# hila-chefer/Transformer-Explainability

Hardware: AMD Instinct MI355X
Metric: relevance maps/sec (ViT-B/16 224^2, batch 64 per GPU, generate_LRP transformer_attribution) (higher is better)
Workload: dtype f32 (3xbf16 split operands, 6 products, fp32 accumulate)

## Files before the change

### include/te_relprop.h

```cpp
#ifndef TE_RELPROP_H
#define TE_RELPROP_H

#include <stddef.h>
#include <stdint.h>

#ifdef __cplusplus
extern "C" {
#endif

typedef void* te_stream_t;
typedef uint16_t te_bf16_t;

enum {
  TE_OK = 0,
  TE_ERR_INVALID_ARG = -1,
  TE_ERR_WORKSPACE = -2,
  TE_ERR_UNSUPPORTED = -3,
  TE_ERR_NO_DEVICE = -4
};

enum { TE_VARIANT_OURS = 0, TE_VARIANT_LRP = 1, TE_IMPL_SIMPLE = 0x100 };

enum { TE_ROLLOUT_NORMALISE = 1, TE_ROLLOUT_CLS_FIXUP = 2, TE_ROLLOUT_ROW0 = 4 };

int te_version(void);
const char* te_status_string(int status);
int te_device_check(void);
const char* te_build_id(void);

size_t te_linear_relprop_workspace_bytes(int64_t T, int64_t in_f, int64_t out_f, int variant);
int te_linear_relprop_f32(const float* R, const float* X, const float* W, float* out,
                          int64_t T, int64_t in_f, int64_t out_f, float alpha, int variant,
                          void* ws, size_t ws_bytes, te_stream_t stream);

int te_linear_zpass_f32(const float* R, const float* X, const float* W, float* S,
                        int64_t T, int64_t in_f, int64_t out_f, te_stream_t stream);
int te_linear_cpass_f32(const float* S, const float* X, const float* W, float* out,
                        int64_t T, int64_t in_f, int64_t out_f, te_stream_t stream);

int te_linear_zpass_fwd_f32(const float* R, const float* X, const float* W, const float* Y, const float* bias,
                            float* S, int64_t T, int64_t in_f, int64_t out_f, te_stream_t stream);
int te_linear_relprop_fwd_f32(const float* R, const float* X, const float* W, const float* Y, const float* bias,
                              float* out, int64_t T, int64_t in_f, int64_t out_f,
                              void* ws, size_t ws_bytes, te_stream_t stream);

int te_linear_zpass_fwd_scaled_f32(const float* R, const float* r_scale, int64_t r_scale_stride,
                                   int64_t rows_per_sample, const float* X, const float* W, const float* Y,
                                   const float* bias, float* S, int64_t T, int64_t in_f, int64_t out_f,
                                   te_stream_t stream);
int te_linear_relprop_fwd_scaled_f32(const float* R, const float* r_scale, int64_t r_scale_stride,
                                     int64_t rows_per_sample, const float* X, const float* W, const float* Y,
                                     const float* bias, float* out, int64_t T, int64_t in_f, int64_t out_f,
                                     void* ws, size_t ws_bytes, te_stream_t stream);

size_t te_matmul_relprop_av_workspace_bytes(int64_t B, int64_t H, int64_t N, int64_t D);
int te_matmul_relprop_av_f32(const float* R, int64_t r_sb, int64_t r_sh, int64_t r_sn,
                             const float* attn,
                             const float* v, int64_t v_sb, int64_t v_sh, int64_t v_sn,
                             float* cam_attn,
                             float* cam_v, int64_t cv_sb, int64_t cv_sh, int64_t cv_sn,
                             int64_t B, int64_t H, int64_t N, int64_t D, float out_scale, int variant,
                             void* ws, size_t ws_bytes, te_stream_t stream);
size_t te_matmul_relprop_qk_workspace_bytes(int64_t B, int64_t H, int64_t N, int64_t D);
int te_matmul_relprop_av_fwd_f32(const float* R, int64_t r_sb, int64_t r_sh, int64_t r_sn,
                                 const float* attn,
                                 const float* v, int64_t v_sb, int64_t v_sh, int64_t v_sn,
                                 const float* Z,
                                 float* cam_attn,
                                 float* cam_v, int64_t cv_sb, int64_t cv_sh, int64_t cv_sn,
                                 int64_t B, int64_t H, int64_t N, int64_t D, float out_scale, int variant,
                                 void* ws, size_t ws_bytes, te_stream_t stream);
int te_matmul_relprop_av_fwdz_f32(const float* R, int64_t r_sb, int64_t r_sh, int64_t r_sn,
                                  const float* attn,
                                  const float* v, int64_t v_sb, int64_t v_sh, int64_t v_sn,
                                  const float* Z, int64_t z_sb, int64_t z_sh, int64_t z_sn,
                                  float* cam_attn,
                                  float* cam_v, int64_t cv_sb, int64_t cv_sh, int64_t cv_sn,
                                  int64_t B, int64_t H, int64_t N, int64_t D, float out_scale, int variant,
                                  void* ws, size_t ws_bytes, te_stream_t stream);
int te_matmul_relprop_qk_fwd_f32(const float* R_nn,
                                 const float* q, int64_t q_sb, int64_t q_sh, int64_t q_sn,
                                 const float* k, int64_t k_sb, int64_t k_sh, int64_t k_sn,
                                 const float* Z,
                                 float* cam_q, int64_t cq_sb, int64_t cq_sh, int64_t cq_sn,
                                 float* cam_k, int64_t ck_sb, int64_t ck_sh, int64_t ck_sn,
                                 int64_t B, int64_t H, int64_t N, int64_t D, float out_scale, int variant,
                                 void* ws, size_t ws_bytes, te_stream_t stream);
int te_matmul_relprop_qk_fwd_scaled_f32(const float* R_nn, const float* r_scale, int64_t r_scale_stride,
                                        const float* q, int64_t q_sb, int64_t q_sh, int64_t q_sn,
                                        const float* k, int64_t k_sb, int64_t k_sh, int64_t k_sn,
                                        const float* Z,
                                        float* cam_q, int64_t cq_sb, int64_t cq_sh, int64_t cq_sn,
                                        float* cam_k, int64_t ck_sb, int64_t ck_sh, int64_t ck_sn,
                                        int64_t B, int64_t H, int64_t N, int64_t D, float out_scale, int variant,
                                        void* ws, size_t ws_bytes, te_stream_t stream);
int te_matmul_relprop_qk_f32(const float* R_nn,
                             const float* q, int64_t q_sb, int64_t q_sh, int64_t q_sn,
                             const float* k, int64_t k_sb, int64_t k_sh, int64_t k_sn,
                             float* cam_q, int64_t cq_sb, int64_t cq_sh, int64_t cq_sn,
                             float* cam_k, int64_t ck_sb, int64_t ck_sh, int64_t ck_sn,
                             int64_t B, int64_t H, int64_t N, int64_t D, float out_scale, int variant,
                             void* ws, size_t ws_bytes, te_stream_t stream);

size_t te_add_relprop_workspace_bytes(int64_t B, int64_t n);
int te_add_relprop_f32(const float* R, const float* X0, const float* X1, float* out0, float* out1,
                       int64_t B, int64_t n, int64_t x1_batch_stride, int variant,
                       void* ws, size_t ws_bytes, te_stream_t stream);

size_t te_add_relprop_deferred_workspace_bytes(int64_t B, int64_t n);
int te_add_relprop_deferred_f32(const float* R, const float* X0, const float* X1, float* a, float* b, float* fac,
                                int64_t B, int64_t n, int64_t x1_batch_stride,
                                void* ws, size_t ws_bytes, te_stream_t stream);

size_t te_add_bcast_relprop_workspace_bytes(int64_t B, int64_t H, int64_t N);
int te_add_bcast_relprop_f32(const float* R, const float* X0, const float* mask, float* out0,
                             float* out1, int64_t B, int64_t H, int64_t N, int variant,
                             void* ws, size_t ws_bytes, te_stream_t stream);

int te_add_bcast_relprop_deferred_f32(const float* R, const float* X0, const float* mask, float* a, float* out1,
                                      float* fac, int64_t B, int64_t H, int64_t N,
                                      void* ws, size_t ws_bytes, te_stream_t stream);

int te_clone_relprop_f32(const float* R0, const float* R1, const float* R2, const float* X,
                         float* out, int64_t n, te_stream_t stream);

int te_clone_relprop_scaled_f32(const float* R0, const float* s0, int64_t s0_stride,
                                const float* R1, const float* s1, int64_t s1_stride,
                                const float* R2, const float* s2, int64_t s2_stride,
                                const float* X, float* out, int64_t B, int64_t n, te_stream_t stream);

int te_index_select_relprop_f32(const float* R, const float* X, float* out,
                                int64_t B, int64_t N, int64_t C, int64_t index, te_stream_t stream);

int te_gradcam_headmean_f32(const float* grad, const float* cam, float* out,
                            int64_t B, int64_t H, int64_t N, te_stream_t stream);

size_t te_rollout_workspace_bytes(int64_t L, int64_t B, int64_t N);
size_t te_rollout_row0_workspace_bytes(int64_t B, int64_t N);
int te_rollout_f32(const float* cams, int64_t L, int64_t start_layer, int64_t B, int64_t N,
                   int flags, float* joint, void* ws, size_t ws_bytes, te_stream_t stream);

#define TE_X6_TILE_AUTO 0
#define TE_X6_TILE_128 1
#define TE_X6_TILE_256 2
#define TE_X6_TILE_128x128 3
#define TE_X6_TEST_DROP_HANDOVER 0x200
#define TE_X6_WHOLE_TILES 0x10000
#define TE_X6_TEST_SMALL_GRID 0x4000
#define TE_X6_X_PLANES_SIGNED 0x20000
#define TE_X6_TILE_Z_SHIFT 10
#define TE_X6_TILE_C_SHIFT 12
#define TE_X6_PHASE_SPLIT 4
#define TE_X6_PHASE_Z 8
#define TE_X6_PHASE_C 16
#define TE_X6_PHASE_MASK 28
int te_linear_relprop_x6_supported(int64_t T, int64_t in_f, int64_t out_f);
size_t te_linear_relprop_x6_workspace_bytes(int64_t T, int64_t in_f, int64_t out_f);
size_t te_linear_x6_weight_planes_bytes(int64_t in_f, int64_t out_f);
size_t te_linear_x6_planes_bytes(int64_t rows, int64_t K);
int te_linear_x6_prepare_weights_f32(const float* W, int64_t in_f, int64_t out_f, void* planes, size_t planes_bytes,
                                     te_stream_t stream);
int te_linear_x6_split_abs_f32(const float* X, int64_t rows, int64_t K, void* planes, size_t planes_bytes,
                               te_stream_t stream);
int te_linear_relprop_x6_f32(const float* R, const float* r_scale, int64_t r_scale_stride, int64_t rows_per_sample,
                             const float* X, const float* W, const void* w_planes, const void* x_planes,
                             const float* Y, const float* bias, float* out,
                             int64_t T, int64_t in_f, int64_t out_f, int flags, unsigned* status, void* ws,
                             size_t ws_bytes, te_stream_t stream);
int te_linear_relprop_x6_check(const void* ws, int64_t T, int64_t in_f, int64_t out_f, te_stream_t stream);

int te_linear_relprop_x6_general_supported(int64_t T, int64_t in_f, int64_t out_f, int variant);
size_t te_linear_x6_weight_planes_lrp_bytes(int64_t in_f, int64_t out_f);
int te_linear_x6_prepare_weights_lrp_f32(const float* W, int64_t in_f, int64_t out_f, void* planes, size_t planes_bytes,
                                         te_stream_t stream);
size_t te_linear_relprop_x6_general_workspace_bytes(int64_t T, int64_t in_f, int64_t out_f, int variant);
int te_linear_relprop_x6_general_f32(const float* R, const float* r_scale, int64_t r_scale_stride, int64_t rows_per_sample,
                                     const float* X, const float* W, const void* w_planes, const void* w_planes_lrp,
                                     const void* x_abs_planes, const float* Y, const float* bias, float* out,
                                     int64_t T, int64_t in_f, int64_t out_f, float alpha, int variant, int flags,
                                     unsigned* status, void* ws, size_t ws_bytes, te_stream_t stream);

int te_gemm_x6_supported(int64_t T, int64_t K, int64_t M);
size_t te_gemm_x6_workspace_bytes(int64_t T, int64_t K, int64_t M);
int te_linear_x6_split_matrix_f32(const float* A, int64_t rows, int64_t K, int transposed, void* planes,
                                  size_t planes_bytes, te_stream_t stream);
int te_gemm_x6_f32(const float* X, const void* x_planes, const void* w_planes, const float* bias, float* out,
                   int64_t T, int64_t K, int64_t M, int flags, unsigned* status, void* ws, size_t ws_bytes,
                   te_stream_t stream);
int te_linear_x6_split_dual_f32(const float* A, int64_t rows, int64_t K, void* planes, void* planes_abs,
                                size_t planes_bytes, te_stream_t stream);
int te_gelu_backward_x6_planes_f32(const float* dy, const float* x, int64_t rows, int64_t K, void* planes,
                                   size_t planes_bytes, te_stream_t stream);
int te_gelu_forward_x6_planes_f32(const float* x, float* y, int64_t rows, int64_t K, void* planes, void* planes_abs,
                                  size_t planes_bytes, te_stream_t stream);

int te_attention_forward_supported(int64_t N, int64_t D);
int te_attention_forward_f32(const float* qkv, float* z_qk, float* attn, float* out,
                             int64_t B, int64_t H, int64_t N, int64_t D, float scale, te_stream_t stream);
int te_attention_forward_planes_f32(const float* qkv, float* z_qk, float* attn, float* out, void* out_planes,
                                    void* out_abs_planes, size_t planes_bytes, int64_t B, int64_t H, int64_t N, int64_t D,
                                    float scale, te_stream_t stream);
int te_attention_backward_f32(const float* d_out, const float* qkv, const float* attn, float* d_attn, float* d_qkv,
                              int64_t B, int64_t H, int64_t N, int64_t D, float scale, int need_qk, te_stream_t stream);
int te_attention_backward_out_f32(const float* d_out, const float* out, const float* qkv, const float* attn, float* d_attn,
                                  float* d_qkv, int64_t B, int64_t H, int64_t N, int64_t D, float scale, int need_qk,
                                  te_stream_t stream);

int te_attention_strided_supported(int64_t N, int64_t D);
size_t te_attention_backward_strided_workspace_bytes(int64_t B, int64_t H, int64_t N);
int te_attention_forward_strided_f32(const float* q, int64_t q_sb, int64_t q_sh, int64_t q_sn,
                                     const float* k, int64_t k_sb, int64_t k_sh, int64_t k_sn,
                                     const float* v, int64_t v_sb, int64_t v_sh, int64_t v_sn,
                                     const float* mask, float* z_qk, float* x_scaled, float* attn,
                                     float* out, int64_t o_sb, int64_t o_sh, int64_t o_sn,
                                     int64_t B, int64_t H, int64_t N, int64_t D, float scale, te_stream_t stream);
int te_attention_backward_strided_f32(const float* d_out, int64_t do_sb, int64_t do_sh, int64_t do_sn,
                                      const float* q, int64_t q_sb, int64_t q_sh, int64_t q_sn,
                                      const float* k, int64_t k_sb, int64_t k_sh, int64_t k_sn,
                                      const float* v, int64_t v_sb, int64_t v_sh, int64_t v_sn,
                                      const float* attn, float* d_attn,
                                      float* d_q, int64_t dq_sb, int64_t dq_sh, int64_t dq_sn,
                                      float* d_k, int64_t dk_sb, int64_t dk_sh, int64_t dk_sn,
                                      float* d_v, int64_t dv_sb, int64_t dv_sh, int64_t dv_sn,
                                      int64_t B, int64_t H, int64_t N, int64_t D, float scale, int need_qk,
                                      void* ws, size_t ws_bytes, te_stream_t stream);
int te_attention_backward_strided_out_f32(const float* d_out, int64_t do_sb, int64_t do_sh, int64_t do_sn,
                                          const float* out, int64_t o_sb, int64_t o_sh, int64_t o_sn,
                                          const float* q, int64_t q_sb, int64_t q_sh, int64_t q_sn,
                                          const float* k, int64_t k_sb, int64_t k_sh, int64_t k_sn,
                                          const float* v, int64_t v_sb, int64_t v_sh, int64_t v_sn,
                                          const float* attn, float* d_attn,
                                          float* d_q, int64_t dq_sb, int64_t dq_sh, int64_t dq_sn,
                                          float* d_k, int64_t dk_sb, int64_t dk_sh, int64_t dk_sn,
                                          float* d_v, int64_t dv_sb, int64_t dv_sh, int64_t dv_sn,
                                          int64_t B, int64_t H, int64_t N, int64_t D, float scale, int need_qk,
                                          void* ws, size_t ws_bytes, te_stream_t stream);

int te_layernorm_supported(int64_t C);
int te_layernorm_forward_f32(const float* x, const float* weight, const float* bias, float* y, float* mean, float* rstd,
                             int64_t T, int64_t C, float eps, te_stream_t stream);
int te_layernorm_backward_f32(const float* dy, const float* x, const float* weight, const float* mean, const float* rstd,
                              const float* add, float* dx, int64_t T, int64_t C, te_stream_t stream);
int te_gelu_forward_f32(const float* x, float* y, int64_t n, te_stream_t stream);
int te_gelu_backward_f32(const float* dy, const float* x, float* dx, int64_t n, te_stream_t stream);

int te_heatmap_f32(const float* maps, float* heat, float* fg_mask, int64_t B, int64_t g, int64_t scale,
                   int normalise, te_stream_t stream);

size_t te_seg_metrics_workspace_bytes(int64_t B, int64_t H, int64_t W);
int te_seg_metrics_f32(const float* heat, const float* fg_mask, const int64_t* labels, int64_t* counts, double* ap,
                       double* f1, int64_t B, int64_t H, int64_t W, void* ws, size_t ws_bytes, te_stream_t stream);

#define TE_MAPSIM_SSIM 1
size_t te_map_similarity_workspace_bytes(int64_t B, int64_t n);
int te_map_similarity_f32(const float* a, const float* b, int64_t* rank_sums, double* sim, int64_t B, int64_t n, int64_t H,
                          int64_t W, int flags, double data_range, void* ws, size_t ws_bytes, te_stream_t stream);

#define TE_RATIONALE_MAX_KS 16
#define TE_RATIONALE_CLAMP 1
size_t te_rationale_metrics_workspace_bytes(int64_t B, int64_t N, int64_t Wmax);
int te_rationale_metrics_f32(const float* scores, const int32_t* word_ids, const uint8_t* truth, float* word_scores,
                             int32_t* n_words, int32_t* order, int32_t* counts, double* soft, int64_t B, int64_t N,
                             int64_t Wmax, const int64_t* ks, int64_t n_ks, int flags, void* ws, size_t ws_bytes,
                             te_stream_t stream);

#define TE_TOKEN_ERASE_MAX_FRACTIONS 8
int te_token_erase(const int64_t* input_ids, const int64_t* attention_mask, const int32_t* word_ids,
                   const int32_t* order, const int32_t* n_words, int64_t* ids_out, int64_t* mask_out,
                   int32_t* n_rationale, int64_t B, int64_t N, int64_t Wmax, const double* fractions, int64_t n_t,
                   int64_t pad_id, te_stream_t stream);

size_t te_conv2d_zb_relprop_workspace_bytes(int64_t B, int64_t C, int64_t H, int64_t W, int64_t E, int64_t p);
int te_conv2d_zb_relprop_f32(const float* R, int64_t r_bs, const float* X, const float* W, const float* Y,
                             const float* bias, float* out, int64_t B, int64_t C, int64_t H, int64_t W_, int64_t E,
                             int64_t p, int flags, void* ws, size_t ws_bytes, te_stream_t stream);

#define TE_PERTURB_MAX_STEPS 16
#define TE_PERTURB_MAX_CHANNELS 4
size_t te_perturb_workspace_bytes(int64_t B, int64_t n_steps);
int te_perturb_f32(const float* vis, const float* data, float* out, int64_t B, int64_t C, int64_t HW,
                   const int64_t* ks, int64_t n_steps, const float* mean, const float* std_, void* ws,
                   size_t ws_bytes, te_stream_t stream);

#define TE_BLUR_MAX_TAPS 63
int te_blur_normalised_f32(const float* data, float* out, int64_t B, int64_t C, int64_t H, int64_t W, const float* taps,
                           int64_t klen, const float* mean, const float* std_, te_stream_t stream);
size_t te_pixel_rank_workspace_bytes(int64_t B, int64_t n);
int te_pixel_rank_f32(const float* vis, int32_t* rank, int64_t B, int64_t n, void* ws, size_t ws_bytes, te_stream_t stream);
int te_curve_inputs_f32(const float* data, const float* substrate, const float* fill, const int32_t* rank, float* out,
                        int64_t B, int64_t C, int64_t HW, int64_t step, int64_t s0, int64_t n_s, int insertion,
                        const float* mean, const float* std_, te_stream_t stream);
int te_curve_inputs_bf16(const float* data, const float* substrate, const float* fill, const int32_t* rank, te_bf16_t* out,
                         int64_t B, int64_t C, int64_t HW, int64_t step, int64_t s0, int64_t n_s, int insertion,
                         const float* mean, const float* std_, te_stream_t stream);
int te_curve_scores_f32(const float* logits, const int64_t* target, double* prob, int64_t B, int64_t K, int64_t s0,
                        int64_t n_s, te_stream_t stream);
int te_curve_scores_bf16(const te_bf16_t* logits, const int64_t* target, double* prob, int64_t B, int64_t K, int64_t s0,
                         int64_t n_s, te_stream_t stream);
int te_curve_auc_f64(const double* prob, double* auc, int64_t S1, int64_t B, te_stream_t stream);

size_t te_localisation_workspace_bytes(int64_t P, int64_t H, int64_t W);
int te_localisation_f32(const float* heat, const int64_t* labels, const int64_t* image_index, const int64_t* target_id,
                        const int64_t* boxes, int64_t M, int64_t* stats, double* energy, int64_t P, int64_t B, int64_t H,
                        int64_t W, void* ws, size_t ws_bytes, te_stream_t stream);

int te_noise_inputs_f32(const float* x, float* out, int64_t B, int64_t n, int64_t d0, int64_t n_d, float radius, int64_t seed,
                        int64_t id0, te_stream_t stream);
int te_noise_inputs_bf16(const float* x, te_bf16_t* out, int64_t B, int64_t n, int64_t d0, int64_t n_d, float radius,
                         int64_t seed, int64_t id0, te_stream_t stream);
int te_map_distance_f32(const float* a, const float* b, double* sums, int64_t B, int64_t D, int64_t n, te_stream_t stream);
int te_map_distance_bf16(const float* a, const te_bf16_t* b, double* sums, int64_t B, int64_t D, int64_t n,
                         te_stream_t stream);
size_t te_map_complexity_workspace_bytes(int64_t B, int64_t n);
int te_map_complexity_f32(const float* maps, double* out, int64_t* counts, int64_t B, int64_t n, double eps, void* ws,
                          size_t ws_bytes, te_stream_t stream);

#define TE_SUBSET_MAX_CELLS 4096
int te_subset_inputs_f32(const float* x, const float* substrate, const float* fill, const float* attr, float* out,
                         uint8_t* member, double* attr_sum, int64_t B, int64_t C, int64_t g_h, int64_t g_w, int64_t p,
                         int64_t k, int64_t d0, int64_t n_d, int64_t seed, int64_t id0, te_stream_t stream);
int te_subset_inputs_bf16(const float* x, const float* substrate, const float* fill, const float* attr, te_bf16_t* out,
                          uint8_t* member, double* attr_sum, int64_t B, int64_t C, int64_t g_h, int64_t g_w, int64_t p,
                          int64_t k, int64_t d0, int64_t n_d, int64_t seed, int64_t id0, te_stream_t stream);
int te_perturbation_dot_f32(const float* x, const float* y, const float* w, double* sums, int64_t B, int64_t D, int64_t n,
                            int64_t m, te_stream_t stream);
int te_perturbation_dot_bf16(const float* x, const te_bf16_t* y, const float* w, double* sums, int64_t B, int64_t D, int64_t n,
                             int64_t m, te_stream_t stream);

int te_linear_relprop_bf16_supported(int64_t T, int64_t in_f, int64_t out_f);
size_t te_linear_relprop_bf16_workspace_bytes(int64_t T, int64_t in_f, int64_t out_f);
size_t te_linear_bf16_weight_planes_bytes(int64_t in_f, int64_t out_f);
int te_linear_bf16_prepare_weights(const te_bf16_t* W, int64_t in_f, int64_t out_f, void* planes, size_t planes_bytes,
                                   te_stream_t stream);
int te_linear_relprop_bf16(const float* R, int64_t r_ld, const float* r_scale, int64_t r_scale_stride,
                           int64_t rows_per_scale, const te_bf16_t* X, int64_t x_ld, const void* w_planes, float* out,
                           int64_t T, int64_t in_f, int64_t out_f, void* ws, size_t ws_bytes, te_stream_t stream);
int te_matmul_relprop_bf16_supported(int64_t N, int64_t D);
size_t te_matmul_relprop_av_bf16_workspace_bytes(int64_t B, int64_t H, int64_t N, int64_t D);
size_t te_matmul_relprop_qk_bf16_workspace_bytes(int64_t B, int64_t H, int64_t N, int64_t D);
int te_matmul_relprop_av_bf16(const float* R, int64_t r_sb, int64_t r_sh, int64_t r_sn,
                              const te_bf16_t* attn,
                              const te_bf16_t* v, int64_t v_sb, int64_t v_sh, int64_t v_sn,
                              const te_bf16_t* Z, int64_t z_sb, int64_t z_sh, int64_t z_sn,
                              float* cam_attn,
                              float* cam_v, int64_t cv_sb, int64_t cv_sh, int64_t cv_sn,
                              int64_t B, int64_t H, int64_t N, int64_t D, float out_scale, int variant,
                              void* ws, size_t ws_bytes, te_stream_t stream);
int te_matmul_relprop_qk_bf16(const float* R_nn, const float* r_scale, int64_t r_scale_stride,
                              const te_bf16_t* q, int64_t q_sb, int64_t q_sh, int64_t q_sn,
                              const te_bf16_t* k, int64_t k_sb, int64_t k_sh, int64_t k_sn,
                              const te_bf16_t* Z,
                              float* cam_q, int64_t cq_sb, int64_t cq_sh, int64_t cq_sn,
                              float* cam_k, int64_t ck_sb, int64_t ck_sh, int64_t ck_sn,
                              int64_t B, int64_t H, int64_t N, int64_t D, float out_scale, int variant,
                              void* ws, size_t ws_bytes, te_stream_t stream);
int te_add_relprop_bf16(const float* R, const te_bf16_t* X0, const te_bf16_t* X1, float* out0, float* out1, int64_t B,
                        int64_t n, int64_t x1_batch_stride, int variant, void* ws, size_t ws_bytes, te_stream_t stream);
int te_add_relprop_deferred_bf16(const float* R, const te_bf16_t* X0, const te_bf16_t* X1, float* a, float* b,
                                 float* fac, int64_t B, int64_t n, int64_t x1_batch_stride, void* ws, size_t ws_bytes,
// ... 106 lines not shown
```

### transformer-explainability_amd/csrc/te_attn.hip

```cpp
#include "te_internal.h"

namespace {

constexpr int kThreads = 256;

__global__ __launch_bounds__(kThreads) void av_s_simple(
    const float* __restrict__ R, Strided rs, const float* __restrict__ attn, const float* __restrict__ v,
    Strided vs, float* __restrict__ S, int64_t B, int64_t H, int64_t N, int64_t D) {
  const int64_t idx = (int64_t)blockIdx.x * kThreads + threadIdx.x;
  if (idx >= B * H * N * D) return;
  const int64_t d = idx % D, i = (idx / D) % N, h = (idx / (D * N)) % H, b = idx / (D * N * H);
  const float* arow = attn + ((b * H + h) * N + i) * N;
  float z = 0.0f;
  for (int64_t j = 0; j < N; ++j) z = fmaf(arow[j], v[vs.at(b, h, j) + d], z);
  S[idx] = te_sd(R[rs.at(b, h, i) + d], z);
}

__global__ __launch_bounds__(kThreads) void av_s_from_z_simple(
    const float* __restrict__ R, Strided rs, const float* __restrict__ Z, float* __restrict__ S, int64_t B, int64_t H,
    int64_t N, int64_t D) {
  const int64_t idx = (int64_t)blockIdx.x * kThreads + threadIdx.x;
  if (idx >= B * H * N * D) return;
  const int64_t d = idx % D, i = (idx / D) % N, h = (idx / (D * N)) % H, b = idx / (D * N * H);
  S[idx] = te_sd(R[rs.at(b, h, i) + d], Z[idx]);
}
__global__ __launch_bounds__(kThreads) void qk_s_from_z_simple(const float* __restrict__ R, const float* __restrict__ Z,
                                                               float* __restrict__ S, int64_t n) {
  const int64_t idx = (int64_t)blockIdx.x * kThreads + threadIdx.x;
  if (idx < n) S[idx] = te_sd(R[idx], Z[idx]);
}

__global__ __launch_bounds__(kThreads) void av_cam_attn_simple(
    const float* __restrict__ S, const float* __restrict__ attn, const float* __restrict__ v, Strided vs,
    float* __restrict__ cam, int64_t B, int64_t H, int64_t N, int64_t D, float scale) {
  const int64_t idx = (int64_t)blockIdx.x * kThreads + threadIdx.x;
  if (idx >= B * H * N * N) return;
  const int64_t j = idx % N, i = (idx / N) % N, h = (idx / (N * N)) % H, b = idx / (N * N * H);
  const float* srow = S + ((b * H + h) * N + i) * D;
  const float* vrow = v + vs.at(b, h, j);
  float g = 0.0f;
  for (int64_t d = 0; d < D; ++d) g = fmaf(srow[d], vrow[d], g);
  cam[idx] = (attn[idx] * g) * scale;
}

__global__ __launch_bounds__(kThreads) void av_cam_v_simple(
    const float* __restrict__ S, const float* __restrict__ attn, const float* __restrict__ v, Strided vs,
    float* __restrict__ cam_v, Strided cs, int64_t B, int64_t H, int64_t N, int64_t D, float scale) {
  const int64_t idx = (int64_t)blockIdx.x * kThreads + threadIdx.x;
  if (idx >= B * H * N * D) return;
  const int64_t d = idx % D, j = (idx / D) % N, h = (idx / (D * N)) % H, b = idx / (D * N * H);
  const float* a = attn + (b * H + h) * N * N + j;
  const float* s = S + (b * H + h) * N * D + d;
  float u = 0.0f;
  for (int64_t i = 0; i < N; ++i) u = fmaf(a[i * N], s[i * D], u);
  cam_v[cs.at(b, h, j) + d] = (v[vs.at(b, h, j) + d] * u) * scale;
}

__global__ __launch_bounds__(kThreads) void qk_s_simple(
    const float* __restrict__ R, const float* __restrict__ q, Strided qs, const float* __restrict__ k,
    Strided ks, float* __restrict__ S, int64_t B, int64_t H, int64_t N, int64_t D) {
  const int64_t idx = (int64_t)blockIdx.x * kThreads + threadIdx.x;
  if (idx >= B * H * N * N) return;
  const int64_t j = idx % N, i = (idx / N) % N, h = (idx / (N * N)) % H, b = idx / (N * N * H);
  const float* qrow = q + qs.at(b, h, i);
  const float* krow = k + ks.at(b, h, j);
  float z = 0.0f;
  for (int64_t d = 0; d < D; ++d) z = fmaf(qrow[d], krow[d], z);
  S[idx] = te_sd(R[idx], z);
}

__global__ __launch_bounds__(kThreads) void qk_cam_q_simple(
    const float* __restrict__ S, const float* __restrict__ q, Strided qs, const float* __restrict__ k,
    Strided ks, float* __restrict__ cam_q, Strided cs, int64_t B, int64_t H, int64_t N, int64_t D, float scale) {
  const int64_t idx = (int64_t)blockIdx.x * kThreads + threadIdx.x;
  if (idx >= B * H * N * D) return;
  const int64_t d = idx % D, i = (idx / D) % N, h = (idx / (D * N)) % H, b = idx / (D * N * H);
  const float* srow = S + ((b * H + h) * N + i) * N;
  float u = 0.0f;
  for (int64_t j = 0; j < N; ++j) u = fmaf(srow[j], k[ks.at(b, h, j) + d], u);
  cam_q[cs.at(b, h, i) + d] = (q[qs.at(b, h, i) + d] * u) * scale;
}

__global__ __launch_bounds__(kThreads) void qk_cam_k_simple(
    const float* __restrict__ S, const float* __restrict__ q, Strided qs, const float* __restrict__ k,
    Strided ks, float* __restrict__ cam_k, Strided cs, int64_t B, int64_t H, int64_t N, int64_t D, float scale) {
  const int64_t idx = (int64_t)blockIdx.x * kThreads + threadIdx.x;
  if (idx >= B * H * N * D) return;
  const int64_t d = idx % D, j = (idx / D) % N, h = (idx / (D * N)) % H, b = idx / (D * N * H);
  const float* s = S + (b * H + h) * N * N + j;
  float u = 0.0f;
  for (int64_t i = 0; i < N; ++i) u = fmaf(s[i * N], q[qs.at(b, h, i) + d], u);
  cam_k[cs.at(b, h, j) + d] = (k[ks.at(b, h, j) + d] * u) * scale;
}

inline bool view_ok(Strided s) { return s.sb >= 0 && s.sh >= 0 && s.sn > 0; }

inline int finish(int rc) {
  if (rc != TE_OK) return rc;
  TE_RETURN_IF_LAUNCH_FAILED();
  return TE_OK;
}

}

extern "C" size_t te_matmul_relprop_av_workspace_bytes(int64_t B, int64_t H, int64_t N, int64_t D) {
  if (B <= 0 || H <= 0 || N <= 0 || D <= 0) return 0;
  return te_align_up((size_t)2 * B * H * N * D * sizeof(float), 256);
}

extern "C" int te_matmul_relprop_av_f32(const float* R, int64_t r_sb, int64_t r_sh, int64_t r_sn,
                                        const float* attn, const float* v, int64_t v_sb, int64_t v_sh,
                                        int64_t v_sn, float* cam_attn, float* cam_v, int64_t cv_sb,
                                        int64_t cv_sh, int64_t cv_sn, int64_t B, int64_t H, int64_t N,
                                        int64_t D, float out_scale, int variant, void* ws, size_t ws_bytes,
                                        te_stream_t stream_) {
  return te_matmul_relprop_av_fwd_f32(R, r_sb, r_sh, r_sn, attn, v, v_sb, v_sh, v_sn, nullptr, cam_attn, cam_v, cv_sb,
                                      cv_sh, cv_sn, B, H, N, D, out_scale, variant, ws, ws_bytes, stream_);
}

extern "C" int te_matmul_relprop_av_fwd_f32(const float* R, int64_t r_sb, int64_t r_sh, int64_t r_sn,
                                            const float* attn, const float* v, int64_t v_sb, int64_t v_sh,
                                            int64_t v_sn, const float* Z, float* cam_attn, float* cam_v,
                                            int64_t cv_sb, int64_t cv_sh, int64_t cv_sn, int64_t B, int64_t H,
                                            int64_t N, int64_t D, float out_scale, int variant, void* ws,
                                            size_t ws_bytes, te_stream_t stream_) {
  return te_matmul_relprop_av_fwdz_f32(R, r_sb, r_sh, r_sn, attn, v, v_sb, v_sh, v_sn, Z, H * N * D, N * D, D, cam_attn,
                                       cam_v, cv_sb, cv_sh, cv_sn, B, H, N, D, out_scale, variant, ws, ws_bytes, stream_);
}

extern "C" int te_matmul_relprop_av_fwdz_f32(const float* R, int64_t r_sb, int64_t r_sh, int64_t r_sn,
                                             const float* attn, const float* v, int64_t v_sb, int64_t v_sh,
                                             int64_t v_sn, const float* Z, int64_t z_sb, int64_t z_sh, int64_t z_sn,
                                             float* cam_attn, float* cam_v, int64_t cv_sb, int64_t cv_sh,
                                             int64_t cv_sn, int64_t B, int64_t H, int64_t N, int64_t D,
                                             float out_scale, int variant, void* ws, size_t ws_bytes,
                                             te_stream_t stream_) {
  if (!R || !attn || !v || !cam_attn || !cam_v || B <= 0 || H <= 0 || N <= 0 || D <= 0)
    return TE_ERR_INVALID_ARG;
  const Strided rs{r_sb, r_sh, r_sn}, vs{v_sb, v_sh, v_sn}, cs{cv_sb, cv_sh, cv_sn}, contig{H * N * D, N * D, D};
  if (!view_ok(rs) || !view_ok(vs) || !view_ok(cs)) return TE_ERR_INVALID_ARG;
  if (!ws || ws_bytes < te_matmul_relprop_av_workspace_bytes(B, H, N, D)) return TE_ERR_WORKSPACE;
  hipStream_t stream = (hipStream_t)stream_;
  float* S = (float*)ws;
  float* Zws = S + (size_t)(B * H) * N * D;
  Strided zs = Z ? Strided{z_sb, z_sh, z_sn} : contig;
  if ((variant & TE_IMPL_SIMPLE) || !te_attn_mfma::supported(N, D)) {
    if (zs.sn != contig.sn || zs.sh != contig.sh || zs.sb != contig.sb) return TE_ERR_UNSUPPORTED;
    const int64_t nd = B * H * N * D, nn = B * H * N * N;
    dim3 blk(kThreads);
    if (Z) av_s_from_z_simple<<<dim3((unsigned)te_ceil_div(nd, kThreads)), blk, 0, stream>>>(R, rs, Z, S, B, H, N, D);
    else av_s_simple<<<dim3((unsigned)te_ceil_div(nd, kThreads)), blk, 0, stream>>>(R, rs, attn, v, vs, S, B, H, N, D);
    av_cam_attn_simple<<<dim3((unsigned)te_ceil_div(nn, kThreads)), blk, 0, stream>>>(S, attn, v, vs, cam_attn, B,
                                                                                     H, N, D, out_scale);
    av_cam_v_simple<<<dim3((unsigned)te_ceil_div(nd, kThreads)), blk, 0, stream>>>(S, attn, v, vs, cam_v, cs, B, H,
                                                                                  N, D, out_scale);
    TE_RETURN_IF_LAUNCH_FAILED();
    return TE_OK;
  }
  if (!Z) {
    const int rc = te_attn_mfma::z_av_launch(attn, v, vs, Zws, B, H, N, stream);
    if (rc != TE_OK) return rc;
    Z = Zws;
  }
  if (te_attn_kb::supported(B, H, N, D))
    return finish(te_attn_kb::av_launch(TE_ATTN_RULE, R, rs, attn, v, vs, Z, zs, cam_attn, cam_v, cs, B, H, N, out_scale, stream));
  return finish(te_attn_mfma::av_launch(R, rs, attn, v, vs, Z, zs, cam_attn, cam_v, cs, B, H, N, out_scale, S, stream));
}

extern "C" size_t te_matmul_relprop_qk_workspace_bytes(int64_t B, int64_t H, int64_t N, int64_t D) {
  if (B <= 0 || H <= 0 || N <= 0 || D <= 0) return 0;
  return te_align_up((size_t)2 * B * H * N * N * sizeof(float), 256);
}

extern "C" int te_matmul_relprop_qk_f32(const float* R_nn, const float* q, int64_t q_sb, int64_t q_sh,
                                        int64_t q_sn, const float* k, int64_t k_sb, int64_t k_sh, int64_t k_sn,
                                        float* cam_q, int64_t cq_sb, int64_t cq_sh, int64_t cq_sn, float* cam_k,
                                        int64_t ck_sb, int64_t ck_sh, int64_t ck_sn, int64_t B, int64_t H,
                                        int64_t N, int64_t D, float out_scale, int variant, void* ws,
                                        size_t ws_bytes, te_stream_t stream_) {
  return te_matmul_relprop_qk_fwd_f32(R_nn, q, q_sb, q_sh, q_sn, k, k_sb, k_sh, k_sn, nullptr, cam_q, cq_sb, cq_sh,
                                      cq_sn, cam_k, ck_sb, ck_sh, ck_sn, B, H, N, D, out_scale, variant, ws, ws_bytes,
                                      stream_);
}

extern "C" int te_matmul_relprop_qk_fwd_f32(const float* R_nn, const float* q, int64_t q_sb, int64_t q_sh,
                                            int64_t q_sn, const float* k, int64_t k_sb, int64_t k_sh,
                                            int64_t k_sn, const float* Z, float* cam_q, int64_t cq_sb,
                                            int64_t cq_sh, int64_t cq_sn, float* cam_k, int64_t ck_sb,
                                            int64_t ck_sh, int64_t ck_sn, int64_t B, int64_t H, int64_t N,
                                            int64_t D, float out_scale, int variant, void* ws, size_t ws_bytes,
                                            te_stream_t stream_) {
  return te_matmul_relprop_qk_fwd_scaled_f32(R_nn, nullptr, 0, q, q_sb, q_sh, q_sn, k, k_sb, k_sh, k_sn, Z, cam_q, cq_sb,
                                             cq_sh, cq_sn, cam_k, ck_sb, ck_sh, ck_sn, B, H, N, D, out_scale, variant, ws,
                                             ws_bytes, stream_);
}

extern "C" int te_matmul_relprop_qk_fwd_scaled_f32(const float* R_nn, const float* r_scale, int64_t r_scale_stride,
                                                   const float* q, int64_t q_sb, int64_t q_sh, int64_t q_sn,
                                                   const float* k, int64_t k_sb, int64_t k_sh, int64_t k_sn,
                                                   const float* Z, float* cam_q, int64_t cq_sb, int64_t cq_sh,
                                                   int64_t cq_sn, float* cam_k, int64_t ck_sb, int64_t ck_sh,
                                                   int64_t ck_sn, int64_t B, int64_t H, int64_t N, int64_t D,
                                                   float out_scale, int variant, void* ws, size_t ws_bytes,
                                                   te_stream_t stream_) {
  if (!R_nn || !q || !k || !cam_q || !cam_k || B <= 0 || H <= 0 || N <= 0 || D <= 0) return TE_ERR_INVALID_ARG;
  const Strided qs{q_sb, q_sh, q_sn}, ks{k_sb, k_sh, k_sn}, cqs{cq_sb, cq_sh, cq_sn}, cks{ck_sb, ck_sh, ck_sn};
  if (!view_ok(qs) || !view_ok(ks) || !view_ok(cqs) || !view_ok(cks)) return TE_ERR_INVALID_ARG;
  if (!ws || ws_bytes < te_matmul_relprop_qk_workspace_bytes(B, H, N, D)) return TE_ERR_WORKSPACE;
  hipStream_t stream = (hipStream_t)stream_;
  float* S = (float*)ws;
  float* Zws = S + (size_t)(B * H) * N * N;
  if ((variant & TE_IMPL_SIMPLE) || !te_attn_mfma::supported(N, D)) {
    if (r_scale) return TE_ERR_UNSUPPORTED;
    const int64_t nd = B * H * N * D, nn = B * H * N * N;
    dim3 blk(kThreads);
    if (Z) qk_s_from_z_simple<<<dim3((unsigned)te_ceil_div(nn, kThreads)), blk, 0, stream>>>(R_nn, Z, S, nn);
    else qk_s_simple<<<dim3((unsigned)te_ceil_div(nn, kThreads)), blk, 0, stream>>>(R_nn, q, qs, k, ks, S, B, H, N, D);
    qk_cam_q_simple<<<dim3((unsigned)te_ceil_div(nd, kThreads)), blk, 0, stream>>>(S, q, qs, k, ks, cam_q, cqs, B, H,
                                                                                  N, D, out_scale);
    qk_cam_k_simple<<<dim3((unsigned)te_ceil_div(nd, kThreads)), blk, 0, stream>>>(S, q, qs, k, ks, cam_k, cks, B, H,
                                                                                  N, D, out_scale);
    TE_RETURN_IF_LAUNCH_FAILED();
    return TE_OK;
  }
  if (!Z) {
    const int rc = te_attn_mfma::z_qk_launch(q, qs, k, ks, Zws, B, H, N, stream);
    if (rc != TE_OK) return rc;
    Z = Zws;
  }
  if (te_attn_rules::supported(B, H, N, D) && q_sn > 65536) return TE_ERR_UNSUPPORTED;
  if (te_attn_rc::supported(B, H, N, D))
    return finish(te_attn_rc::qk_launch(TE_ATTN_RULE, R_nn, q, qs, k, ks, Z, cam_q, cqs, cam_k, cks, B, H, N, out_scale, r_scale, r_scale_stride,
                                        stream));
  if (te_attn_rules::supported(B, H, N, D))
    return finish(te_attn_rules::qk_launch(TE_ATTN_RULE, R_nn, q, qs, k, ks, Z, cam_q, cqs, cam_k, cks, B, H, N, out_scale, S, r_scale,
                                           r_scale_stride, stream));
  if (r_scale) return TE_ERR_UNSUPPORTED;
  return finish(te_attn_mfma::qk_launch(R_nn, q, qs, k, ks, Z, cam_q, cqs, cam_k, cks, B, H, N, out_scale, S, stream));
}

extern "C" int te_attention_forward_supported(int64_t N, int64_t D) { return te_attn_fwd6::supported(1, 1, N, D) ? 1 : 0; }

extern "C" int te_attention_forward_f32(const float* qkv, float* z_qk, float* attn, float* out, int64_t B, int64_t H,
                                        int64_t N, int64_t D, float scale, te_stream_t stream_) {
  if (!qkv || !z_qk || !attn || !out || B <= 0 || H <= 0 || N <= 0) return TE_ERR_INVALID_ARG;
  if (!te_attn_fwd6::supported(B, H, N, D)) return TE_ERR_UNSUPPORTED;
  return finish(te_attn_fwd6::launch(qkv, z_qk, attn, out, B, H, N, scale, (hipStream_t)stream_));
}

extern "C" int te_attention_forward_planes_f32(const float* qkv, float* z_qk, float* attn, float* out, void* out_planes,
                                               void* out_abs_planes, size_t planes_bytes, int64_t B, int64_t H, int64_t N,
                                               int64_t D, float scale, te_stream_t stream_) {
  if (!qkv || !z_qk || !attn || !out || !out_planes || B <= 0 || H <= 0 || N <= 0) return TE_ERR_INVALID_ARG;
  if (!te_attn_fwd6::supported(B, H, N, D)) return TE_ERR_UNSUPPORTED;
  const size_t need = te_linear_x6_planes_bytes(B * N, H * D);
  if (need == 0) return TE_ERR_UNSUPPORTED;
  if (planes_bytes < need || !te_aligned16(out_planes) || (out_abs_planes && !te_aligned16(out_abs_planes))) return TE_ERR_WORKSPACE;
  return finish(te_attn_fwd6::launch(qkv, z_qk, attn, out, B, H, N, scale, (hipStream_t)stream_, out_planes, out_abs_planes));
}

static int attention_backward(const float* d_out, const float* out, const float* qkv, const float* attn, float* d_attn, float* d_qkv,
                              int64_t B, int64_t H, int64_t N, int64_t D, float scale, int need_qk, te_stream_t stream_) {
  if (!d_out || !qkv || !attn || !d_attn || !d_qkv || B <= 0 || H <= 0 || N <= 0) return TE_ERR_INVALID_ARG;
  if (!te_attn_fwd6::supported(B, H, N, D)) return TE_ERR_UNSUPPORTED;
  hipStream_t stream = (hipStream_t)stream_;
  const int64_t C = H * 64;
  const Strided heads{N * C, 64, C};
  const Strided fused{N * 3 * C, 64, 3 * C};
  const float *q = qkv, *k = qkv + C, *v = qkv + 2 * C;
  float *d_q = d_qkv, *d_k = d_qkv + C, *d_v = d_qkv + 2 * C;
  const int rc = te_attn_kb::av_launch(TE_ATTN_BWD, d_out, heads, attn, v, fused, nullptr, Strided(), d_attn, d_v, fused, B, H, N, 1.0f, stream);
  if (rc != TE_OK || !need_qk) return finish(rc);
  if ((N <= 160 || out) && te_attn_rc::supported(B, H, N, D))
    return finish(te_attn_rc::qk_launch(TE_ATTN_BWD, d_attn, q, fused, k, fused, attn, d_q, fused, d_k, fused, B, H, N, scale, nullptr, 0, stream,
                                        out ? d_out : nullptr, out, heads));
  return finish(te_attn_rules::qk_launch(TE_ATTN_BWD, d_attn, q, fused, k, fused, attn, d_q, fused, d_k, fused, B, H, N, scale, nullptr, nullptr, 0,
                                         stream));
}

extern "C" int te_attention_backward_f32(const float* d_out, const float* qkv, const float* attn, float* d_attn,
                                         float* d_qkv, int64_t B, int64_t H, int64_t N, int64_t D, float scale,
                                         int need_qk, te_stream_t stream_) {
  return attention_backward(d_out, nullptr, qkv, attn, d_attn, d_qkv, B, H, N, D, scale, need_qk, stream_);
}

extern "C" int te_attention_backward_out_f32(const float* d_out, const float* out, const float* qkv, const float* attn,
                                             float* d_attn, float* d_qkv, int64_t B, int64_t H, int64_t N, int64_t D,
                                             float scale, int need_qk, te_stream_t stream_) {
  if (!out) return TE_ERR_INVALID_ARG;
  return attention_backward(d_out, out, qkv, attn, d_attn, d_qkv, B, H, N, D, scale, need_qk, stream_);
}

extern "C" int te_attention_strided_supported(int64_t N, int64_t D) { return te_attn_long::supported(1, 1, N, D) ? 1 : 0; }

extern "C" size_t te_attention_backward_strided_workspace_bytes(int64_t B, int64_t H, int64_t N) {
  return te_align_up((size_t)(B * H * N) * sizeof(float), 256);
}

extern "C" int te_attention_forward_strided_f32(const float* q, int64_t q_sb, int64_t q_sh, int64_t q_sn, const float* k,
                                                int64_t k_sb, int64_t k_sh, int64_t k_sn, const float* v, int64_t v_sb,
                                                int64_t v_sh, int64_t v_sn, const float* mask, float* z_qk,
                                                float* x_scaled, float* attn, float* out, int64_t o_sb, int64_t o_sh,
                                                int64_t o_sn, int64_t B, int64_t H, int64_t N, int64_t D, float scale,
                                                te_stream_t stream_) {
  using te_attn_long::strides_ok;
  if (!q || !k || !v || !attn || !out || B <= 0 || H <= 0 || N <= 0) return TE_ERR_INVALID_ARG;
  const Strided qs{q_sb, q_sh, q_sn}, ks{k_sb, k_sh, k_sn}, vs{v_sb, v_sh, v_sn}, os{o_sb, o_sh, o_sn};
  if (!te_attn_long::supported(B, H, N, D)) return TE_ERR_UNSUPPORTED;
  if (!strides_ok(qs) || !strides_ok(ks) || !strides_ok(vs) || !strides_ok(os)) return TE_ERR_UNSUPPORTED;
  hipStream_t stream = (hipStream_t)stream_;
  if (te_attn_fwd6l::supported(B, H, N, D))
    return finish(te_attn_fwd6l::launch(q, qs, k, ks, v, vs, mask, z_qk, x_scaled, attn, out, os, B, H, N, scale, stream));
  return finish(te_attn_long::fwd_launch(q, qs, k, ks, v, vs, mask, z_qk, x_scaled, attn, out, os, B, H, N, scale, stream));
}

static int backward_strided(const float* d_out, Strided dos, const float* out, Strided os, const float* q, Strided qs, const float* k,
                            Strided ks, const float* v, Strided vs, const float* attn, float* d_attn, float* d_q, Strided dqs, float* d_k,
                            Strided dks, float* d_v, Strided dvs, int64_t B, int64_t H, int64_t N, int64_t D, float scale, int need_qk,
                            void* ws, size_t ws_bytes, te_stream_t stream_) {
  using te_attn_long::strides_ok;
  if (!d_out || !k || !v || !attn || !d_attn || !d_v || B <= 0 || H <= 0 || N <= 0) return TE_ERR_INVALID_ARG;
  if (need_qk && (!q || !d_q || !d_k)) return TE_ERR_INVALID_ARG;
  if (!te_attn_long::supported(B, H, N, D)) return TE_ERR_UNSUPPORTED;
  if (!strides_ok(dos) || !strides_ok(ks) || !strides_ok(vs) || !strides_ok(dvs) || (out && !strides_ok(os))) return TE_ERR_UNSUPPORTED;
  if (need_qk && (!strides_ok(qs) || !strides_ok(dqs) || !strides_ok(dks))) return TE_ERR_UNSUPPORTED;
  if (!ws || ws_bytes < te_attention_backward_strided_workspace_bytes(B, H, N)) return TE_ERR_WORKSPACE;
  hipStream_t stream = (hipStream_t)stream_;
  float* rowdot = (float*)ws;
  need_qk = need_qk ? 1 : 0;
  const bool l6 = te_attn_bwd6l::supported(B, H, N, D);
  int rc;
  if ((out || !need_qk) && l6)
    rc = te_attn_bwd6l::launch_rows(d_out, dos, out, os, k, ks, v, vs, attn, d_attn, rowdot, d_q, dqs, B, H, N, scale, need_qk, stream);
  else
    rc = te_attn_long::bwd_rows_launch(d_out, dos, k, ks, v, vs, attn, d_attn, rowdot, d_q, dqs, B, H, N, scale, need_qk, stream);
  if (rc != TE_OK) return rc;
  if (l6) return finish(te_attn_bwd6l::launch_cols(attn, d_attn, rowdot, d_out, dos, q, qs, d_v, dvs, d_k, dks, B, H, N, scale, need_qk, stream));
  return finish(te_attn_long::bwd_cols_launch(attn, d_attn, rowdot, d_out, dos, q, qs, d_v, dvs, d_k, dks, B, H, N, scale, need_qk, stream));
}

extern "C" int te_attention_backward_strided_f32(const float* d_out, int64_t do_sb, int64_t do_sh, int64_t do_sn,
                                                 const float* q, int64_t q_sb, int64_t q_sh, int64_t q_sn, const float* k,
                                                 int64_t k_sb, int64_t k_sh, int64_t k_sn, const float* v, int64_t v_sb,
                                                 int64_t v_sh, int64_t v_sn, const float* attn, float* d_attn, float* d_q,
                                                 int64_t dq_sb, int64_t dq_sh, int64_t dq_sn, float* d_k, int64_t dk_sb,
                                                 int64_t dk_sh, int64_t dk_sn, float* d_v, int64_t dv_sb, int64_t dv_sh,
                                                 int64_t dv_sn, int64_t B, int64_t H, int64_t N, int64_t D, float scale,
                                                 int need_qk, void* ws, size_t ws_bytes, te_stream_t stream_) {
  return backward_strided(d_out, {do_sb, do_sh, do_sn}, nullptr, Strided(), q, {q_sb, q_sh, q_sn}, k, {k_sb, k_sh, k_sn}, v, {v_sb, v_sh, v_sn},
                          attn, d_attn, d_q, {dq_sb, dq_sh, dq_sn}, d_k, {dk_sb, dk_sh, dk_sn}, d_v, {dv_sb, dv_sh, dv_sn}, B, H, N, D, scale,
                          need_qk, ws, ws_bytes, stream_);
}

extern "C" int te_attention_backward_strided_out_f32(const float* d_out, int64_t do_sb, int64_t do_sh, int64_t do_sn,
                                                     const float* out, int64_t o_sb, int64_t o_sh, int64_t o_sn, const float* q,
                                                     int64_t q_sb, int64_t q_sh, int64_t q_sn, const float* k, int64_t k_sb,
                                                     int64_t k_sh, int64_t k_sn, const float* v, int64_t v_sb, int64_t v_sh,
                                                     int64_t v_sn, const float* attn, float* d_attn, float* d_q, int64_t dq_sb,
                                                     int64_t dq_sh, int64_t dq_sn, float* d_k, int64_t dk_sb, int64_t dk_sh,
                                                     int64_t dk_sn, float* d_v, int64_t dv_sb, int64_t dv_sh, int64_t dv_sn,
                                                     int64_t B, int64_t H, int64_t N, int64_t D, float scale, int need_qk, void* ws,
                                                     size_t ws_bytes, te_stream_t stream_) {
  if (!out) return TE_ERR_INVALID_ARG;
  return backward_strided(d_out, {do_sb, do_sh, do_sn}, out, {o_sb, o_sh, o_sn}, q, {q_sb, q_sh, q_sn}, k, {k_sb, k_sh, k_sn}, v,
                          {v_sb, v_sh, v_sn}, attn, d_attn, d_q, {dq_sb, dq_sh, dq_sn}, d_k, {dk_sb, dk_sh, dk_sn}, d_v, {dv_sb, dv_sh, dv_sn}, B,
                          H, N, D, scale, need_qk, ws, ws_bytes, stream_);
}
```

### transformer-explainability_amd/csrc/te_attn_kb.hip

```cpp
#include <type_traits>

#include "te_buffer.h"
#include "te_internal.h"
#include "te_x6.h"

namespace te_attn_kb {

namespace {

constexpr int TI = 32;
constexpr int kT = 512;
constexpr int kWaves = kT / 64;
constexpr int XLD = 36;

enum { RULE = 0, BWD = 1 };



constexpr int kRLD = 144;
constexpr int kTLD = 80;
constexpr int kPlR = TI * kRLD;
constexpr int kPlT = 64 * kTLD;
constexpr int kSBuf = 3 * kPlR + 3 * kPlT;

template <int MODE>
__global__ __launch_bounds__(kT) void av6_kb_kernel(
    const float* __restrict__ R, Strided rs, const float* __restrict__ Z, Strided zs, const float* __restrict__ attn,
    const float* __restrict__ v, Strided vs, float* __restrict__ cam_attn, float* __restrict__ cam_v, Strided cs, int H,
    int N, int BH, int KBG, float scale) {
  __shared__ __attribute__((aligned(16))) unsigned char Sb[3][kSBuf];
  __shared__ __attribute__((aligned(16))) float Xw[kWaves][TI * XLD];
  __shared__ unsigned arrived;
  if (threadIdx.x == 0) arrived = 0;
  __syncthreads();
  const int bh = blockIdx.x % BH, g = blockIdx.x / BH;
  const int b = bh / H, h = bh - b * H;
  const int wave = __builtin_amdgcn_readfirstlane(threadIdx.x >> 6), lane = threadIdx.x & 63, lr = lane & 31, kh = lane >> 5;
  const int nkb = (N + 31) >> 5, kb = g * KBG + wave;
  const bool has_blk = wave < KBG && kb < nkb;
  const int j = kb * 32 + lr;
  const int ntiles = (N + TI - 1) / TI;
  const int srow = threadIdx.x >> 4, sc = threadIdx.x & 15;
  const int spos = (srow & 0x13) | ((srow & 4) << 1) | ((srow & 8) >> 1);

  const unsigned nn_bytes = (unsigned)N * (unsigned)N * 4u;
  const Rsrc a_rs = make_rsrc(attn + (int64_t)bh * N * N, nn_bytes);
  const Rsrc ca_rs = make_rsrc(cam_attn + (int64_t)bh * N * N, nn_bytes);
  const Rsrc r_rs = make_rsrc(R + (int64_t)b * rs.sb + (int64_t)h * rs.sh, view_bytes(N, rs.sn));
  const Rsrc z_rs = make_rsrc(MODE == RULE ? Z + (int64_t)b * zs.sb + (int64_t)h * zs.sh : R, MODE == RULE ? view_bytes(N, zs.sn) : 0u);
  const Rsrc v_rs = make_rsrc(v + (int64_t)b * vs.sb + (int64_t)h * vs.sh, view_bytes(N, vs.sn));
  const Rsrc cv_rs = make_rsrc(cam_v + (int64_t)b * cs.sb + (int64_t)h * cs.sh, view_bytes(N, cs.sn));
  const unsigned row_bytes = (unsigned)N * 4u;

  f32x4 rr = {0.f, 0.f, 0.f, 0.f}, zz = {0.f, 0.f, 0.f, 0.f};
  const unsigned r_off = ((unsigned)srow * (unsigned)rs.sn + 4u * sc) * 4u, z_off = ((unsigned)srow * (unsigned)zs.sn + 4u * sc) * 4u;
  const unsigned r_tile = (unsigned)TI * (unsigned)rs.sn * 4u, z_tile = (unsigned)TI * (unsigned)zs.sn * 4u;
  auto fetch_rz = [&](int it) __attribute__((always_inline)) {
    ld128_hidden(rr, r_rs, r_off + (unsigned)it * r_tile);
    if constexpr (MODE == RULE) ld128_hidden(zz, z_rs, z_off + (unsigned)it * z_tile);
  };
  constexpr int kRz = (MODE == RULE) ? 2 : 1;
  auto pin_rz = [&]() __attribute__((always_inline)) {
    TE_PIN(rr);
    if constexpr (MODE == RULE) TE_PIN(zz);
  };
  auto put_s = [&](int it) __attribute__((always_inline)) {
    f32x4 s = rr;
    if constexpr (MODE == RULE) {
#pragma unroll
      for (int e = 0; e < 4; ++e) s[e] = te_sd(rr[e], zz[e]);
    }
    unsigned p01[3], p23[3];
    split3_pk(s[0], s[1], p01);
    split3_pk(s[2], s[3], p23);
    unsigned char* base = Sb[it % 3];
#pragma unroll
    for (int q = 0; q < 3; ++q) {
      *reinterpret_cast<u32x2*>(base + q * kPlR + srow * kRLD + sc * 8) = u32x2{p01[q], p23[q]};
      unsigned char* t = base + 3 * kPlR + q * kPlT + (4 * sc) * kTLD + spos * 2;
      *reinterpret_cast<unsigned short*>(t) = (unsigned short)(p01[q] & 0xffffu);
      *reinterpret_cast<unsigned short*>(t + kTLD) = (unsigned short)(p01[q] >> 16);
      *reinterpret_cast<unsigned short*>(t + 2 * kTLD) = (unsigned short)(p23[q] & 0xffffu);
      *reinterpret_cast<unsigned short*>(t + 3 * kTLD) = (unsigned short)(p23[q] >> 16);
    }
    asm volatile("s_waitcnt lgkmcnt(0)" ::: "memory");
    if (lane == 0) __hip_atomic_fetch_add(&arrived, 1u, __ATOMIC_RELAXED, __HIP_MEMORY_SCOPE_WORKGROUP);
  };
  auto wait_s = [&](int it) __attribute__((always_inline)) {
    const unsigned target = (unsigned)kWaves * (unsigned)(it + 1);
    while (__builtin_amdgcn_readfirstlane(__hip_atomic_load(&arrived, __ATOMIC_RELAXED, __HIP_MEMORY_SCOPE_WORKGROUP)) < target)
      __builtin_amdgcn_s_sleep(1);
    asm volatile("" ::: "memory");
  };

  if (!has_blk) {
    fetch_rz(0);
    TE_VM_WAIT(0);
    pin_rz();
    put_s(0);
    fetch_rz(1);
    for (int it = 0; it < ntiles; ++it) {
      wait_s(it);
      TE_VM_WAIT(0);
      pin_rz();
      put_s(it + 1);
      fetch_rz(it + 2);
    }
    TE_VM_WAIT(0);
    return;
  }

  bf16x8 vpl[4][3];
  {
    const unsigned off = ((unsigned)j * (unsigned)vs.sn + 8u * kh) * 4u;
#pragma unroll
    for (int s4 = 0; s4 < 4; ++s4) {
      const f32x4 lo = ld128(v_rs, off + 64u * s4), hi = ld128(v_rs, off + 64u * s4 + 16u);
      const float x[8] = {lo[0], lo[1], lo[2], lo[3], hi[0], hi[1], hi[2], hi[3]};
      planes_of8(x, vpl[s4]);
    }
  }
  float* const Xb = Xw[wave];
  const int xr = lane >> 3, xc = (lane & 7) << 2;
  const unsigned lane_x4 = ((unsigned)xr * (unsigned)N + (unsigned)(kb * 32 + xc)) * 4u;
  const unsigned lane_nn = ((unsigned)(4 * kh) * (unsigned)N + (unsigned)j) * 4u;
  const bool key_ok = j < N;
  const bool blk_full = kb * 32 + 32 <= N;
  auto fetch_attn = [&](int it, f32x4 (&dst)[4]) __attribute__((always_inline)) {
    const unsigned base = (unsigned)(it * TI) * row_bytes;
#pragma unroll
    for (int p = 0; p < 4; ++p) ld128_hidden(dst[p], a_rs, lane_x4 + (base + (unsigned)(8 * p) * row_bytes));
  };
  auto to_acc = [&](const f32x4 (&src)[4], float (&dst)[16]) __attribute__((always_inline)) {
#pragma unroll
    for (int p = 0; p < 4; ++p) *reinterpret_cast<f32x4*>(Xb + (8 * p + xr) * XLD + xc) = src[p];
#pragma unroll
    for (int e = 0; e < 16; ++e) dst[e] = Xb[crow(e, kh) * XLD + lr];
  };

  float ac[16];
  f32x4 an[4], an2[4];
  fetch_rz(0);
  fetch_attn(0, an2);
  TE_VM_WAIT(0);
  pin_rz();
#pragma unroll
  for (int s4 = 0; s4 < 4; ++s4)
#pragma unroll
    for (int q = 0; q < 3; ++q) TE_PIN(vpl[s4][q]);
#pragma unroll
  for (int p = 0; p < 4; ++p) TE_PIN(an2[p]);
  put_s(0);
  fetch_rz(1);
  fetch_attn(1, an);
  to_acc(an2, ac);

  f32x16 accv[2];
  zero16(accv[0]);
  zero16(accv[1]);
  auto tile = [&](int it, f32x4 (&ax)[4], f32x4 (&ay)[4]) __attribute__((always_inline)) {
    const unsigned char* Sc = Sb[it % 3];
    wait_s(it);
    TE_VM_WAIT(4);
    pin_rz();
    put_s(it + 1);
    fetch_rz(it + 2);
    fetch_attn(it + 2, ax);
    __builtin_amdgcn_sched_barrier(0);
    if (it < ntiles) {
      f32x16 gacc;
      zero16(gacc);
      {
        const unsigned char* Ab = Sc + lr * kRLD + 16 * kh;
#pragma unroll
        for (int s4 = 0; s4 < 4; ++s4) {
          bf16x8 a[3];
#pragma unroll
          for (int q = 0; q < 3; ++q) a[q] = *reinterpret_cast<const bf16x8*>(Ab + q * kPlR + 32 * s4);
          mfma_x6(gacc, a, vpl[s4]);
        }
      }
      float gp[16];
#pragma unroll
      for (int e = 0; e < 16; ++e) gp[e] = (MODE == RULE) ? (ac[e] * gacc[e]) * scale : gacc[e];
      const unsigned base = (unsigned)(it * TI) * row_bytes;
      if (blk_full) {
#pragma unroll
        for (int e = 0; e < 16; ++e) Xb[crow(e, kh) * XLD + lr] = gp[e];
#pragma unroll
        for (int p = 0; p < 4; ++p) {
          const f32x4 t = *reinterpret_cast<const f32x4*>(Xb + (8 * p + xr) * XLD + xc);
          st128_hidden(t, ca_rs, lane_x4 + (base + (unsigned)(8 * p) * row_bytes));
        }
      } else if (key_ok) {
#pragma unroll
        for (int e = 0; e < 16; ++e) st32_hidden(gp[e], ca_rs, lane_nn + (base + (unsigned)((e & 3) + 8 * (e >> 2)) * row_bytes));
      }
      bf16x8 apl[2][3];
#pragma unroll
      for (int s2 = 0; s2 < 2; ++s2) {
        const float x[8] = {ac[8 * s2], ac[8 * s2 + 1], ac[8 * s2 + 2], ac[8 * s2 + 3],
                            ac[8 * s2 + 4], ac[8 * s2 + 5], ac[8 * s2 + 6], ac[8 * s2 + 7]};
        planes_of8(x, apl[s2]);
      }
#pragma unroll
      for (int db = 0; db < 2; ++db) {
        const unsigned char* Bb = Sc + 3 * kPlR + (db * 32 + lr) * kTLD + 16 * kh;
#pragma unroll
        for (int s2 = 0; s2 < 2; ++s2) {
          bf16x8 bq[3];
#pragma unroll
          for (int q = 0; q < 3; ++q) bq[q] = *reinterpret_cast<const bf16x8*>(Bb + q * kPlT + 32 * s2);
          mfma_x6(accv[db], apl[s2], bq);
        }
      }
    }
    if constexpr (kRz == 2) TE_VM_WAIT(6);
    else TE_VM_WAIT(5);
#pragma unroll
    for (int p = 0; p < 4; ++p) TE_PIN(ay[p]);
    to_acc(ay, ac);
  };
#pragma unroll 1
  for (int it = 0; it < ntiles; it += 2) {
    tile(it, an2, an);
    tile(it + 1, an, an2);
  }
  TE_VM_WAIT(0);

#pragma unroll
  for (int db = 0; db < 2; ++db) {
    const unsigned d4 = (unsigned)(db * 32 + lr) * 4u;
    float x[16];
    if constexpr (MODE == RULE) {
      const unsigned xoff = (unsigned)(kb * 32 + 4 * kh) * (unsigned)vs.sn * 4u + d4;
#pragma unroll
      for (int e = 0; e < 16; ++e) x[e] = ld32(v_rs, xoff + (unsigned)((e & 3) + 8 * (e >> 2)) * (unsigned)vs.sn * 4u);
    }
    const unsigned ooff = (unsigned)(kb * 32 + 4 * kh) * (unsigned)cs.sn * 4u + d4;
#pragma unroll
    for (int e = 0; e < 16; ++e) {
      float val = accv[db][e];
      if constexpr (MODE == RULE) val = (x[e] * val) * scale;
      st32(val, cv_rs, ooff + (unsigned)((e & 3) + 8 * (e >> 2)) * (unsigned)cs.sn * 4u);
    }
  }
}

inline void groups_for(int64_t N, int& ng, int& kbg) {
  const int nkb = (int)((N + 31) / 32);
  ng = (nkb + kWaves - 1) / kWaves;
  kbg = (nkb + ng - 1) / ng;
}

}

bool supported(int64_t B, int64_t H, int64_t N, int64_t D) {
  int ng, kbg;
  groups_for(N, ng, kbg);
  return D == 64 && N >= 1 && N <= 4096 && B * H * ng <= 0x7fffffff;
}

int av_launch(int mode, const float* R, Strided rs, const float* attn, const float* v, Strided vs, const float* Z, Strided zs,
              float* cam_attn, float* cam_v, Strided cs, int64_t B, int64_t H, int64_t N, float scale, hipStream_t stream) {
  int ng, kbg;
  groups_for(N, ng, kbg);
  const int BH = (int)(B * H);
  auto stride_ok = [](int64_t sn) { return sn >= 64 && sn <= 65536; };
  if (!stride_ok(rs.sn) || !stride_ok(vs.sn) || !stride_ok(cs.sn) || (mode == 0 && !stride_ok(zs.sn))) return TE_ERR_UNSUPPORTED;
  const dim3 grid((unsigned)(BH * ng)), blk(kT);
  if (mode == 0)
    av6_kb_kernel<RULE><<<grid, blk, 0, stream>>>(R, rs, Z, zs, attn, v, vs, cam_attn, cam_v, cs, (int)H, (int)N, BH, kbg, scale);
  else
    av6_kb_kernel<BWD><<<grid, blk, 0, stream>>>(R, rs, nullptr, Strided{0, 0, 0}, attn, v, vs, cam_attn, cam_v, cs, (int)H,
                                                 (int)N, BH, kbg, 1.0f);
  return TE_OK;
}

}
```

### transformer-explainability_amd/csrc/te_attn_rc.hip

```cpp
#include <stdlib.h>
#include <string.h>

#include <type_traits>

#include "te_buffer.h"
#include "te_internal.h"
#include "te_x6.h"

namespace te_attn_rc {

namespace {

constexpr int kT = 512;
constexpr int kMaxN = 224;
constexpr int kMaxSteps = kMaxN / 16;

enum { RULE = 0, BWD = 1 };
enum { ROWS = 0, COLS = 1 };


template <bool PERM>
__device__ __forceinline__ void stage_planes(unsigned char* __restrict__ Pl, const float* __restrict__ M, int64_t sn, int N,
                                             int NS) {
  for (int item = threadIdx.x; item < NS * 2 * 16; item += kT) {
// ... 159 lines not shown
    float rdr[8];
    if constexpr (MODE == BWD) {
      const float* rp = rdv + 32 * blk + 16 * (s & 1) + 8 * kh;
      const f32x4 a0 = *reinterpret_cast<const f32x4*>(rp), a1 = *reinterpret_cast<const f32x4*>(rp + 4);
#pragma unroll
      for (int e = 0; e < 4; ++e) rdr[e] = a0[e], rdr[4 + e] = a1[e];
    }
#pragma unroll
    for (int t2 = 0; t2 < 4; ++t2) {
      f32x2 r = {rc[set][2 * t2], rc[set][2 * t2 + 1]}, z = {zc[set][2 * t2], zc[set][2 * t2 + 1]};
      if constexpr (MODE == RULE) {
        if (has_f) r = r * f32x2{f, f};
        sv[t2] = sd2(r, z);
      } else {
        sv[t2] = (z * (r - f32x2{rdr[2 * t2], rdr[2 * t2 + 1]})) * f32x2{scale, scale};
      }
    }
    if (32 * (s >> 1) + 32 > N) {
      const bool ok = 32 * (s >> 1) + n < N;
#pragma unroll
      for (int t2 = 0; t2 < 4; ++t2) sv[t2][0] = ok ? sv[t2][0] : 0.0f, sv[t2][1] = ok ? sv[t2][1] : 0.0f;
    }
    unsigned pk[4][3];
#pragma unroll
    for (int t2 = 0; t2 < 4; ++t2) split3_pk(sv[t2][0], sv[t2][1], pk[t2]);
#pragma unroll
    for (int q = 0; q < 3; ++q) b[q] = __builtin_bit_cast(bf16x8, u32x4{pk[0][q], pk[1][q], pk[2][q], pk[3][q]});
  };
  bf16x8 E[2];
#pragma unroll
  for (int sp = 0; sp < 2; ++sp) {
    const int tt = n - 16 * sp - 8 * kh;
    u32x4 w;
#pragma unroll
    for (int u = 0; u < 4; ++u) w[u] = (tt == 2 * u) ? 0x00003f80u : (tt == 2 * u + 1) ? 0x3f800000u : 0u;
    E[sp] = __builtin_bit_cast(bf16x8, w);
  }
  const unsigned char* const frag = Pk + lane * 16;
  issue(0, 0);
  issue(1, 1);
  issue(2, 2);
  static_for<0, kMaxSteps / 2>([&](auto ri) __attribute__((always_inline)) {
    constexpr int r = decltype(ri)::value, s0 = 2 * r, s1 = 2 * r + 1;
    bf16x8 P0[3], P1[3];
    vm_wait<(((s0 + 2 < kMaxSteps - 1) ? s0 + 2 : kMaxSteps - 1) - s0) * LPS>();
    if (r < NB) {
      pin(s0 % RING);
      make_planes(s0, s0 % RING, P0);
    }
    if constexpr (s0 + RING < kMaxSteps) issue(s0 + RING, s0 % RING);
    vm_wait<(((s1 + 2 < kMaxSteps - 1) ? s1 + 2 : kMaxSteps - 1) - s1) * LPS>();
    if (r < NB) {
      pin(s1 % RING);
      make_planes(s1, s1 % RING, P1);
    }
    if constexpr (s1 + RING < kMaxSteps) issue(s1 + RING, s1 % RING);
    if (r < NB) {
      bf16x8 Ba[3], Bb[3];
#pragma unroll
      for (int q = 0; q < 3; ++q) {
        f32x16 T;
#pragma unroll
        for (int e = 0; e < 16; ++e) T[e] = 0.0f;
        T = TE_MFMA_BF16(P0[q], E[0], T);
        T = TE_MFMA_BF16(P1[q], E[1], T);
        u32x4 wa, wb;
#pragma unroll
        for (int u = 0; u < 4; ++u) {
          wa[u] = __builtin_bit_cast(unsigned, __builtin_convertvector(f32x2{T[2 * u], T[2 * u + 1]}, bf16x2));
          wb[u] = __builtin_bit_cast(unsigned, __builtin_convertvector(f32x2{T[8 + 2 * u], T[8 + 2 * u + 1]}, bf16x2));
        }
        Ba[q] = __builtin_bit_cast(bf16x8, wa);
        Bb[q] = __builtin_bit_cast(bf16x8, wb);
      }
#pragma unroll
      for (int half = 0; half < 2; ++half) {
        bf16x8 a[2][3];
#pragma unroll
        for (int mb = 0; mb < 2; ++mb)
#pragma unroll
          for (int q = 0; q < 3; ++q)
            a[mb][q] = *reinterpret_cast<const bf16x8*>(frag + q * plane + (size_t)((s0 + half) * 2 + mb) * kFrag);
#pragma unroll
        for (int p6 = 0; p6 < 6; ++p6)
#pragma unroll
          for (int mb = 0; mb < 2; ++mb)
            acc[mb] = TE_MFMA_BF16(a[mb][PA[p6]], half ? Bb[PB[p6]] : Ba[PB[p6]], acc[mb]);
      }
    }
  });
  vm_wait<0>();
  pin(0);
  pin(1);
  pin(2);
}

__device__ __forceinline__ void row_dots(float* __restrict__ rdv, Rsrc r_rs, Rsrc z_rs, int N, int NB, int blk) {
  const int lane = threadIdx.x & 63, lr = lane >> 3, lc = lane & 7;
  constexpr int RING = 3, LPS = 8;
  f32x4 rv[RING][4], zv[RING][4];
  const unsigned row_bytes = (unsigned)N * 4u;
  const unsigned base = ((unsigned)(blk * 32 + lr) * (unsigned)N + 4u * lc) * 4u;
  auto issue = [&](int u, int set) __attribute__((always_inline)) {
#pragma unroll
    for (int p = 0; p < 4; ++p) {
      const unsigned off = base + (unsigned)(8 * p) * row_bytes + 128u * (unsigned)u;
      ld128_hidden(rv[set][p], r_rs, off);
      ld128_hidden(zv[set][p], z_rs, off);
    }
  };
  auto pin = [&](int set) __attribute__((always_inline)) {
#pragma unroll
    for (int p = 0; p < 4; ++p) { TE_PIN(rv[set][p]); TE_PIN(zv[set][p]); }
  };
  float part[4] = {0.0f, 0.0f, 0.0f, 0.0f};
  issue(0, 0);
  issue(1, 1);
  issue(2, 2);
  static_for<0, kMaxSteps / 2>([&](auto ui) __attribute__((always_inline)) {
    constexpr int u = decltype(ui)::value, NU = kMaxSteps / 2;
    vm_wait<(((u + 2 < NU - 1) ? u + 2 : NU - 1) - u) * LPS>();
    if (u < NB) {
      pin(u % RING);
#pragma unroll
      for (int p = 0; p < 4; ++p)
#pragma unroll
        for (int e = 0; e < 4; ++e) {
          const float v = rv[u % RING][p][e] * zv[u % RING][p][e];
          part[p] = part[p] + ((32 * u + 4 * lc + e < N) ? v : 0.0f);
        }
    }
    if constexpr (u + RING < NU) issue(u + RING, u % RING);
  });
  vm_wait<0>();
  pin(0);
  pin(1);
  pin(2);
#pragma unroll
  for (int p = 0; p < 4; ++p) {
    float v = part[p];
    v = v + __shfl_xor(v, 1, 64);
    v = v + __shfl_xor(v, 2, 64);
    v = v + __shfl_xor(v, 4, 64);
    if (lc == 0) rdv[32 * blk + 8 * p + lr] = v;
  }
}

template <int MODE>
__global__ __launch_bounds__(kT) void qk_rc_kernel(const float* __restrict__ Rnn, const float* __restrict__ Z,
                                                   const float* __restrict__ q, Strided qs, const float* __restrict__ k,
                                                   Strided ks, float* __restrict__ cam_q, Strided cqs,
                                                   float* __restrict__ cam_k, Strided cks, int H, int N, float scale,
                                                   const float* __restrict__ r_scale, int64_t r_scale_stride, int both,
                                                   const float* __restrict__ dO, const float* __restrict__ O, Strided os) {
  extern __shared__ __attribute__((aligned(16))) unsigned char smem[];
  const int NS = (N + 15) >> 4, NB = (N + 31) >> 5;
  const size_t plane = (size_t)NS * 2 * kFrag;
  unsigned char* const Pk = smem;
  unsigned char* const Pq = both ? smem + 3 * plane : smem;
  float* const rdv = reinterpret_cast<float*>(smem + (both ? 6 : 3) * plane);
  const int bh = blockIdx.x, b = bh / H, h = bh - b * H;
  const int wave = __builtin_amdgcn_readfirstlane(threadIdx.x >> 6), lane = threadIdx.x & 63, n = lane & 31, hh = lane >> 5;
  const unsigned nn_bytes = (unsigned)N * (unsigned)N * 4u;
  const Rsrc r_rs = make_rsrc(Rnn + (int64_t)bh * N * N, nn_bytes), z_rs = make_rsrc(Z + (int64_t)bh * N * N, nn_bytes);
  const float* q_bh = q + (int64_t)b * qs.sb + (int64_t)h * qs.sh;
  const float* k_bh = k + (int64_t)b * ks.sb + (int64_t)h * ks.sh;
  const bool has_f = (MODE == RULE) && r_scale != nullptr;
  const float f = has_f ? r_scale[(int64_t)b * r_scale_stride] : 1.0f;
  const bool owner = wave < NB;

  stage_planes<true>(Pk, k_bh, ks.sn, N, NS);
  if (both) stage_planes<false>(Pq, q_bh, qs.sn, N, NS);
  float rd_own = 0.0f;
  if constexpr (MODE == BWD) {
    if (dO != nullptr) {
      const float* dO_bh = dO + (int64_t)b * os.sb + (int64_t)h * os.sh;
      const float* O_bh = O + (int64_t)b * os.sb + (int64_t)h * os.sh;
      for (int r0 = 0; r0 < 32 * NB; r0 += kT / 4) {
        const int i = r0 + (threadIdx.x >> 2), c = threadIdx.x & 3;
        float part = 0.0f;
        if (i < N) {
          const float* a = dO_bh + (int64_t)i * os.sn + 16 * c;
          const float* o = O_bh + (int64_t)i * os.sn + 16 * c;
          f32x4 av[4], ov[4];
#pragma unroll
          for (int u = 0; u < 4; ++u) av[u] = *reinterpret_cast<const f32x4_u*>(a + 4 * u), ov[u] = *reinterpret_cast<const f32x4_u*>(o + 4 * u);
#pragma unroll
          for (int u = 0; u < 4; ++u)
#pragma unroll
            for (int e = 0; e < 4; ++e) part = part + av[u][e] * ov[u][e];
        }
        part = part + __shfl_xor(part, 1, 64);
        part = part + __shfl_xor(part, 2, 64);
        if (c == 0 && i < 32 * NB) rdv[i] = part;
      }
    } else if (owner) {
      row_dots(rdv, r_rs, z_rs, N, NB, wave);
    }
  }
  __syncthreads();

  if (owner) {
    f32x16 acc[2];
#pragma unroll
    for (int mb = 0; mb < 2; ++mb)
#pragma unroll
      for (int e = 0; e < 16; ++e) acc[mb][e] = 0.0f;
    phase_rows<MODE>(acc, Pk, plane, r_rs, z_rs, N, NB, wave, f, has_f, scale, rdv);
    const int i = wave * 32 + n;
    if (i < N) {
      const float* qrow = q_bh + (int64_t)i * qs.sn + 4 * hh;
      float* orow = cam_q + (int64_t)b * cqs.sb + (int64_t)h * cqs.sh + (int64_t)i * cqs.sn + 4 * hh;
      f32x4 x4[2][4];
      if constexpr (MODE == RULE) {
#pragma unroll
        for (int mb = 0; mb < 2; ++mb)
#pragma unroll
          for (int g = 0; g < 4; ++g) x4[mb][g] = *reinterpret_cast<const f32x4_u*>(qrow + 32 * mb + 8 * g);
      }
#pragma unroll
      for (int mb = 0; mb < 2; ++mb)
#pragma unroll
        for (int g = 0; g < 4; ++g) {
          f32x4 o;
#pragma unroll
          for (int c = 0; c < 4; ++c) {
            const float v = acc[mb][4 * g + c];
            o[c] = (MODE == RULE) ? (x4[mb][g][c] * v) * scale : v;
          }
          *reinterpret_cast<f32x4_u*>(orow + 32 * mb + 8 * g) = o;
        }
    }
  }
  if (!both) {
    __syncthreads();
    stage_planes<false>(Pq, q_bh, qs.sn, N, NS);
    __syncthreads();
  }

  if (owner) {
    f32x16 acc[2];
#pragma unroll
    for (int mb = 0; mb < 2; ++mb)
#pragma unroll
      for (int e = 0; e < 16; ++e) acc[mb][e] = 0.0f;
    phase<MODE, COLS>(acc, Pq, plane, r_rs, z_rs, N, NS, wave, f, has_f, scale, rd_own, rdv);
    const int j = wave * 32 + n;
    if (j < N) {
      const float* krow = k_bh + (int64_t)j * ks.sn + 4 * hh;
      float* orow = cam_k + (int64_t)b * cks.sb + (int64_t)h * cks.sh + (int64_t)j * cks.sn + 4 * hh;
      f32x4 x4[2][4];
      if constexpr (MODE == RULE) {
#pragma unroll
        for (int mb = 0; mb < 2; ++mb)
#pragma unroll
          for (int g = 0; g < 4; ++g) x4[mb][g] = *reinterpret_cast<const f32x4_u*>(krow + 32 * mb + 8 * g);
      }
#pragma unroll
      for (int mb = 0; mb < 2; ++mb)
#pragma unroll
        for (int g = 0; g < 4; ++g) {
          f32x4 o;
#pragma unroll
          for (int c = 0; c < 4; ++c) {
            const float v = acc[mb][4 * g + c];
            o[c] = (MODE == RULE) ? (x4[mb][g][c] * v) * scale : v;
          }
          *reinterpret_cast<f32x4_u*>(orow + 32 * mb + 8 * g) = o;
        }
    }
  }
}

inline size_t lds_bytes(int64_t N, bool both) {
  const int64_t NS = (N + 15) >> 4;
  return (size_t)((both ? 6 : 3) * NS * 2 * kFrag) + (size_t)(NS * 16 + 16) * sizeof(float);
}
constexpr size_t kLdsMax = 160 * 1024;

}

bool supported(int64_t B, int64_t H, int64_t N, int64_t D) {
  return D == 64 && N >= 1 && N <= kMaxN && B * H >= 1 && B * H <= 0x7fffffff;
}

int qk_launch(int mode, const float* Rnn, const float* q, Strided qs, const float* k, Strided ks, const float* Z, float* cam_q,
              Strided cqs, float* cam_k, Strided cks, int64_t B, int64_t H, int64_t N, float scale, const float* r_scale,
              int64_t r_scale_stride, hipStream_t stream, const float* d_out, const float* out, Strided os) {
  if (!supported(B, H, N, 64)) return TE_ERR_UNSUPPORTED;
  const int both = lds_bytes(N, true) <= kLdsMax ? 1 : 0;
  const size_t lds = lds_bytes(N, both != 0);
  const dim3 grid((unsigned)(B * H));
  if (mode == RULE) {
    (void)hipFuncSetAttribute(reinterpret_cast<const void*>(qk_rc_kernel<RULE>), hipFuncAttributeMaxDynamicSharedMemorySize, (int)kLdsMax);
    qk_rc_kernel<RULE><<<grid, dim3(kT), lds, stream>>>(Rnn, Z, q, qs, k, ks, cam_q, cqs, cam_k, cks, (int)H, (int)N, scale, r_scale,
                                                       r_scale_stride, both, nullptr, nullptr, Strided{0, 0, 0});
  } else {
    (void)hipFuncSetAttribute(reinterpret_cast<const void*>(qk_rc_kernel<BWD>), hipFuncAttributeMaxDynamicSharedMemorySize, (int)kLdsMax);
    const bool from_out = d_out != nullptr && out != nullptr;
    qk_rc_kernel<BWD><<<grid, dim3(kT), lds, stream>>>(Rnn, Z, q, qs, k, ks, cam_q, cqs, cam_k, cks, (int)H, (int)N, scale, nullptr, 0,
                                                      both, from_out ? d_out : nullptr, from_out ? out : nullptr, os);
  }
  return TE_OK;
}

}
```

### transformer-explainability_amd/csrc/te_internal.h

```cpp
#pragma once

#include "te_common.h"

bool te_internal_zb_cpass_tiled(const float* S, const float* W, const float* X, float* out, int64_t T, int64_t in_f,
                                int64_t out_f, const TeZbGeom& zb, hipStream_t stream);

enum { TE_ATTN_RULE = 0, TE_ATTN_BWD = 1 };

namespace te_attn_mfma {
bool supported(int64_t N, int64_t D);
int z_av_launch(const float* attn, const float* v, Strided vs, float* Z, int64_t B, int64_t H, int64_t N, hipStream_t stream);
int z_qk_launch(const float* q, Strided qs, const float* k, Strided ks, float* Z, int64_t B, int64_t H, int64_t N, hipStream_t stream);
int av_launch(const float* R, Strided rs, const float* attn, const float* v, Strided vs, const float* Z, Strided zs, float* cam_attn,
              float* cam_v, Strided cs, int64_t B, int64_t H, int64_t N, float scale, float* S, hipStream_t stream);
int qk_launch(const float* Rnn, const float* q, Strided qs, const float* k, Strided ks, const float* Z, float* cam_q, Strided cqs,
              float* cam_k, Strided cks, int64_t B, int64_t H, int64_t N, float scale, float* S, hipStream_t stream);
int rollout_bmm_launch(const float* A, const float* Bm, float* C, int64_t B, int64_t N, hipStream_t stream);
}

namespace te_attn_rules {
bool supported(int64_t B, int64_t H, int64_t N, int64_t D);
int qk_launch(int mode, const float* Rnn, const float* q, Strided qs, const float* k, Strided ks, const float* Z, float* cam_q,
              Strided cqs, float* cam_k, Strided cks, int64_t B, int64_t H, int64_t N, float scale, float* qpart, const float* r_scale,
              int64_t r_scale_stride, hipStream_t stream);
}

namespace te_attn_kb {
bool supported(int64_t B, int64_t H, int64_t N, int64_t D);
int av_launch(int mode, const float* R, Strided rs, const float* attn, const float* v, Strided vs, const float* Z, Strided zs,
              float* cam_attn, float* cam_v, Strided cs, int64_t B, int64_t H, int64_t N, float scale, hipStream_t stream);
}

namespace te_attn_rc {
bool supported(int64_t B, int64_t H, int64_t N, int64_t D);
int qk_launch(int mode, const float* Rnn, const float* q, Strided qs, const float* k, Strided ks, const float* Z, float* cam_q,
              Strided cqs, float* cam_k, Strided cks, int64_t B, int64_t H, int64_t N, float scale, const float* r_scale,
              int64_t r_scale_stride, hipStream_t stream, const float* d_out = nullptr, const float* out = nullptr, Strided os = Strided());
}

namespace te_attn_fwd6 {
bool supported(int64_t B, int64_t H, int64_t N, int64_t D);
int launch(const float* qkv, float* z_qk, float* attn, float* out, int64_t B, int64_t H, int64_t N, float scale, hipStream_t stream,
           void* out_planes = nullptr, void* out_abs_planes = nullptr);
}

namespace te_attn_fwd6l {
bool supported(int64_t B, int64_t H, int64_t N, int64_t D);
int launch(const float* q, Strided qs, const float* k, Strided ks, const float* v, Strided vs, const float* mask, float* z_qk,
           float* x_scaled, float* attn, float* out, Strided os, int64_t B, int64_t H, int64_t N, float scale, hipStream_t stream);
}

namespace te_attn_bwd6l {
bool supported(int64_t B, int64_t H, int64_t N, int64_t D);
int launch_rows(const float* d_out, Strided dos, const float* out, Strided os, const float* k, Strided ks, const float* v, Strided vs,
                const float* attn, float* d_attn, float* rowdot, float* d_q, Strided dqs, int64_t B, int64_t H, int64_t N, float scale,
                int need_qk, hipStream_t stream);
int launch_cols(const float* attn, const float* d_attn, const float* rowdot, const float* d_out, Strided dos, const float* q, Strided qs,
                float* d_v, Strided dvs, float* d_k, Strided dks, int64_t B, int64_t H, int64_t N, float scale, int need_qk,
                hipStream_t stream);
}

namespace te_attn_long {
bool supported(int64_t B, int64_t H, int64_t N, int64_t D);
bool strides_ok(Strided s);
int fwd_launch(const float* q, Strided qs, const float* k, Strided ks, const float* v, Strided vs, const float* mask, float* z_qk,
               float* x_scaled, float* attn, float* out, Strided os, int64_t B, int64_t H, int64_t N, float scale, hipStream_t stream);
int bwd_rows_launch(const float* d_out, Strided dos, const float* k, Strided ks, const float* v, Strided vs, const float* attn, float* d_attn,
                    float* rowdot, float* d_q, Strided dqs, int64_t B, int64_t H, int64_t N, float scale, int need_qk, hipStream_t stream);
int bwd_cols_launch(const float* attn, const float* d_attn, const float* rowdot, const float* d_out, Strided dos, const float* q, Strided qs,
                    float* d_v, Strided dvs, float* d_k, Strided dks, int64_t B, int64_t H, int64_t N, float scale, int need_qk,
                    hipStream_t stream);
}
```

### transformer-explainability_amd/generators.py

```python
from __future__ import annotations

import contextlib
from typing import NamedTuple, Optional

import numpy as np
import torch

from . import methods as M
from . import ops
from .rules import StopRelprop, stop_after_attn_cam
from .vit import relprop_tail


def _one_hot(output: torch.Tensor, index) -> torch.Tensor:
    B, K = output.shape
    if index is None:
        idx = output.detach().argmax(dim=-1)
    else:
        idx = torch.as_tensor(np.asarray(index) if not torch.is_tensor(index) else index, device=output.device)
        idx = idx.reshape(-1).long()
        if idx.numel() == 1 and B > 1:
            idx = idx.expand(B)
    dtype = torch.float32 if output.dtype == torch.bfloat16 else output.dtype
    one_hot = torch.zeros((B, K), dtype=dtype, device=output.device)
    one_hot.scatter_(1, idx.view(B, 1), 1.0)
    return one_hot


def _headmean_stack(attns):
    if ops._is_bf16(attns[0]):
        B, _, N, _ = attns[0].shape
        stack = torch.empty((len(attns), B, N, N), dtype=torch.float32, device=attns[0].device)
        for i, a in enumerate(attns):
            ops.attn_headmean(a, out=stack[i])
        return stack
    return torch.stack([a.mean(dim=1) for a in attns], 0)


def _attention_gradients(loss, attn_modules, retain_graph=False):
    anchors = [getattr(m, "_fused_anchor", None) for m in attn_modules]
    if anchors and all(a is not None for a in anchors):
        lowest = attn_modules[0]
        lowest._fused_stop_backward = True
        try:
            torch.autograd.grad(loss, [anchors[0]], retain_graph=retain_graph, allow_unused=True)
        finally:
            lowest._fused_stop_backward = False
        return
    if any(a is not None for a in anchors):
        raise ops._lib.TeError("attention gradients: some of the listed blocks ran on the producer kernels and some on "
                               "stock PyTorch (a frozen qkv layer, or a block in train mode?); the gradient driver "
                               "handles one kind per pass -- set ops.USE_FUSED_PRODUCERS = False for this model")
    attns = [m.get_attn() for m in attn_modules]
    grads = torch.autograd.grad(loss, attns, retain_graph=retain_graph, allow_unused=False)
    for m, g in zip(attn_modules, grads):
        m.save_attn_gradients(g)


def cam_attn_tail(model):
    last = model.blocks[-1].attn
    grad = last.get_attn_gradients()
    B, H, N, _ = grad.shape
    side = int(round((N - 1) ** 0.5))
    cam = last.get_attention_map().detach()[:, :, 0, 1:].float().reshape(B, H, side, side)
    g = grad[:, :, 0, 1:].float().reshape(B, H, side, side).mean(dim=[2, 3], keepdim=True)
    cam = (cam * g).mean(1).clamp(min=0)
    lo = cam.amin(dim=(1, 2), keepdim=True)
    hi = cam.amax(dim=(1, 2), keepdim=True)
    cam = (cam - lo) / (hi - lo)
    return cam[0] if B == 1 else cam


def attn_rollout_tail(model, start_layer=0):
    stack = _headmean_stack([blk.attn.get_attention_map().detach() for blk in model.blocks])
    joint = ops.rollout(stack, start_layer=start_layer, normalise=True)
    return joint[:, 0, 1:]


def _masked(head_mask) -> dict:
    return {} if head_mask is None else {"head_mask": head_mask}


def _head_relevance_chain(attn_modules, chain):
    for m in attn_modules:
        m.save_head_relevance, m.head_relevance = True, None
    try:
        chain()
    finally:
        for m in attn_modules:
            m.save_head_relevance = False
    return torch.stack([m.head_relevance for m in attn_modules], 1)


def _refuse_before_forward(input, wanted):
    if "full" in wanted and ops._is_f64(input):
        raise ops._lib.TeError(f"{ops.DTYPES_MSG}; method='full' (the z^B patch rule) is not implemented for a "
                               "torch.float64 model: run it on a float32 or bfloat16 model")


@contextlib.contextmanager
def _x6_bracket(t):
    if t.is_cuda:
        ops.x6_poll(t.device)
    yield
    if t.is_cuda:
        ops.x6_post(t.device)


@contextlib.contextmanager
def _prune_flag(model, value):
    user_flag = model.prune_below_start_layer
    model.prune_below_start_layer = value
    try:
        yield
    finally:
        model.prune_below_start_layer = user_flag


class ClassMaps(NamedTuple):
    classes: Optional[torch.Tensor]
    scores: torch.Tensor
    maps: dict


def _num_classes(model):
    for name in ("num_classes", "num_labels"):
        n = getattr(model, name, None)
        if isinstance(n, int) and n > 0:
            return n
    return None


class TopAnd:

    def __init__(self, classes, top_first=True):
        self.classes, self.top_first = classes, bool(top_first)


class _ClassRequest:

    def __init__(self, classes, topk, seeds):
        if sum(a is not None for a in (classes, topk, seeds)) != 1:
            raise ValueError("generate_classes: give exactly one of classes / topk / seeds")
        self.classes, self.topk, self.seeds = classes, topk, seeds

    def check(self, B, C, rel_dtype, device):
        if self.topk is not None:
            k = self.topk
            if isinstance(k, bool) or int(k) != k or k < 1 or (C is not None and k > C):
                raise ValueError(f"topk must be an integer in [1, {C if C is not None else 'num_classes'}], got {self.topk!r}")
        elif isinstance(self.classes, TopAnd):
            given = self.classes.classes
            given = given.reshape(B, -1) if torch.is_tensor(given) else np.asarray(given).reshape(B, -1)
            if C is not None:
                self.classes = TopAnd(ops.host_classes(given, B, C, device), self.classes.top_first)
        elif self.classes is not None:
            if C is not None:
                self.classes = ops.host_classes(self.classes, B, C, device)
        else:
            t = self.seeds
            if not torch.is_tensor(t):
                raise ValueError("seeds must be a tensor of shape [B,C] or [B,K,C]")
            if t.dtype != rel_dtype:
                raise ops._lib.TeError(f"{ops.DTYPES_MSG}; the seeds of this model are {rel_dtype} (its relevance dtype), "
                                       f"got {t.dtype}")
            if t.dim() not in (2, 3) or t.shape[0] != B or t.numel() == 0 or (C is not None and t.shape[-1] != C):
                raise ValueError(f"seeds must have shape [B,C] or [B,K,C] = [{B},{'K,' if t.dim() == 3 else ''}"
                                 f"{C if C is not None else 'num_classes'}], got {tuple(t.shape)}")

    def targets(self, output):
        B, C = output.shape
        logits = output.detach()
        rel = ops.relevance_dtype(logits.dtype)
        self.check(B, C, rel, logits.device)
        if isinstance(self.classes, TopAnd):
            top = ops.class_targets(logits, topk=1, with_seeds=False)[0]
            cols = [top, self.classes.classes] if self.classes.top_first else [self.classes.classes, top]
            return ops.class_targets(logits, classes=torch.cat(cols, 1))
        if self.seeds is None:
            return ops.class_targets(logits, classes=self.classes, topk=self.topk)
        seeds = self.seeds.to(logits.device).reshape(B, -1, C).permute(1, 0, 2).contiguous()
        scores = (seeds * logits.to(rel)).sum(dim=-1).t().contiguous()
        return None, scores, seeds


def _stack_classes(per_class, names):
    return {m: torch.stack([d[m] for d in per_class], 1) for m in names}


class _PassDriver:

    def __init__(self, model, overlap_backward, prune):
        self.model = model
        self.model.eval()
        self.overlap_backward = bool(overlap_backward)
        self._relprop_stream = None
        self.prune = bool(prune)

    def check(self):
        ops.x6_raise_if_failed(next(self.model.parameters()).device)

    def _class_pass(self, output, seeds, attn_modules, chain_of, tails, tail_owner=None):
        K = seeds.shape[0]
        caches = [m.__dict__["_te_cache"] for m in self.model.modules() if m.__dict__.get("_te_cache") is not None]
        per_class = []
        with ops.x_abs_planes_kept(caches) as kept:
            for k in range(K):
                kept.last = k == K - 1
                seed = seeds[k]
                loss = torch.sum(seed * output)
                out = self._gradients_and_chain(loss, attn_modules, chain_of(seed), tail_owner=tail_owner,
                                                retain_graph=not kept.last)
                per_class.append(tails(out))
        return per_class

    def _gradients_and_chain(self, loss, attn_modules, chain, tail_owner=None, retain_graph=False):
        if chain is None or not (self.overlap_backward and loss.is_cuda):
            if attn_modules:
                _attention_gradients(loss, attn_modules, retain_graph)
            return None if chain is None else chain()
        dev = loss.device
        main = torch.cuda.current_stream(dev)
        if self._relprop_stream is None:
            self._relprop_stream = torch.cuda.Stream(device=dev)
        side = self._relprop_stream
        side.wait_stream(main)
        if attn_modules:
            _attention_gradients(loss, attn_modules, retain_graph)
        if tail_owner is not None:
            grads_ready = main.record_event()
            tail_owner._before_tail = lambda: torch.cuda.current_stream(dev).wait_event(grads_ready)
        try:
            with torch.cuda.stream(side):
                out = chain()
        finally:
            if tail_owner is not None:
                tail_owner._before_tail = None
            main.wait_stream(side)
        if not torch.cuda.is_current_stream_capturing():
            for t in (out.values() if isinstance(out, dict) else (out,)):
                if t is not None:
                    t.record_stream(main)
        return out


class LRP(_PassDriver):

    _SINGLE_CALL_NEED = M.Needs(all_grads=True, relprop=True)

    def __init__(self, model, overlap_backward=False, prune=False):
        super().__init__(model, overlap_backward, prune)

    def generate_LRP(self, input, index=None, method="transformer_attribution", is_ablation=False, start_layer=0,
                     head_mask=None):
        with _x6_bracket(input):
            return self._single(input, index, method, is_ablation, start_layer, head_mask)

    def _single(self, input, index, method="transformer_attribution", is_ablation=False, start_layer=0, head_mask=None):
        _refuse_before_forward(input, (method,))
        pruned = bool((self.prune or self.model.prune_below_start_layer) and method in M.SINGLE_CALL_PRUNED)
        name = self.model.default_method if method is None else method
        return self._pass(input, (name,), index, is_ablation, start_layer, head_mask, self._SINGLE_CALL_NEED, pruned)[name]

    def generate_all(self, input, methods, index=None, is_ablation=False, start_layer=0, head_mask=None):
        wanted = M.check(methods, M.LRP_NEEDS)
        _refuse_before_forward(input, wanted)
        if input.dtype == torch.float16:
            raise ops._lib.TeError(f"{ops.DTYPES_MSG}; got {input.dtype} here")
        need = M.needs(wanted, M.LRP_NEEDS, is_ablation, M.LRP_ABLATION_NEEDS)
        pruned = bool((self.prune or self.model.prune_below_start_layer) and need.relprop
                      and M.prunable(wanted, M.LRP_NEEDS))
        ours = tuple(m for m in wanted if m not in M.BASELINE_METHODS)
        with _x6_bracket(input):
            maps = self._pass(input, ours, index, is_ablation, start_layer, head_mask, need, pruned)
            if "attn_rollout" in wanted:
                maps["attn_rollout"] = attn_rollout_tail(self.model, start_layer)
            if "attn_gradcam" in wanted:
                maps["attn_gradcam"] = cam_attn_tail(self.model)
            return {m: maps[m] for m in wanted}

    def generate_classes(self, input, classes=None, topk=None, seeds=None, methods=("transformer_attribution",),
                         is_ablation=False, start_layer=0, head_mask=None) -> ClassMaps:
        wanted = M.check(methods, M.LRP_NEEDS)
        _refuse_before_forward(input, wanted)
        if input.dtype == torch.float16:
            raise ops._lib.TeError(f"{ops.DTYPES_MSG}; got {input.dtype} here")
        request = _ClassRequest(classes, topk, seeds)
        request.check(input.shape[0], _num_classes(self.model), ops.relevance_dtype(input.dtype), input.device)
        model = self.model

        def row(m):
            return M.needs((m,), M.LRP_NEEDS, is_ablation, M.LRP_ABLATION_NEEDS)
        once = tuple(m for m in wanted if row(m).forward_only)
        per_class = tuple(m for m in wanted if m not in once)
        need = M.needs(per_class, M.LRP_NEEDS, is_ablation, M.LRP_ABLATION_NEEDS)
        pruned = bool((self.prune or model.prune_below_start_layer) and need.relprop and M.prunable(wanted, M.LRP_NEEDS))
        ours = tuple(m for m in per_class if m not in M.BASELINE_METHODS)
        with _x6_bracket(input):
            with ops.gelu_backward_plane_handoff():
                output = model(input, **_masked(head_mask))
            cls, scores, seed_stack = request.targets(output)
            B, K = scores.shape
            shared = {m: attn_rollout_tail(model, start_layer) if m == "attn_rollout"
                      else relprop_tail(model, m, None, is_ablation, start_layer) for m in once}
            blocks = list(model.blocks)
            grad_blocks = blocks[start_layer if pruned else 0:] if need.all_grads else blocks[-1:] if need.last_grad else []

            def chain_of(seed):
                if not need.relprop:
                    return None
                return lambda: model.relprop(seed, method=ours, is_ablation=is_ablation, start_layer=start_layer, alpha=1)

            def tails(maps):
                maps = dict(maps or {})
                if "attn_gradcam" in per_class:
                    cam = cam_attn_tail(model)
                    maps["attn_gradcam"] = cam.unsqueeze(0) if B == 1 else cam
                return maps
            stacked = {}
            if per_class:
                with _prune_flag(model, pruned):
                    stacked = _stack_classes(self._class_pass(output, seed_stack, [blk.attn for blk in grad_blocks],
                                                              chain_of, tails, tail_owner=model), per_class)
            for m, t in shared.items():
                stacked[m] = t.unsqueeze(1).expand(-1, K, *t.shape[1:])
            return ClassMaps(cls, scores, {m: stacked[m] for m in wanted})

    def _pass(self, input, wanted, index, is_ablation, start_layer, head_mask, need, pruned):
        model = self.model
        with ops.gelu_backward_plane_handoff():
            output = model(input, **_masked(head_mask))
        maps = {}
        if not need.forward_only:
            one_hot = _one_hot(output, index)
            loss = torch.sum(one_hot * output)
            blocks = list(model.blocks)
            grad_blocks = blocks[start_layer if pruned else 0:] if need.all_grads else blocks[-1:] if need.last_grad else []

            def chain():
                return model.relprop(one_hot, method=wanted, is_ablation=is_ablation, start_layer=start_layer, alpha=1)
            with _prune_flag(model, pruned):
                maps = self._gradients_and_chain(loss, [blk.attn for blk in grad_blocks],
                                                 chain if need.relprop else None, tail_owner=model) or {}
        if not need.relprop:
            maps = {m: relprop_tail(model, m, None, is_ablation, start_layer) for m in wanted}
        return maps

    def generate_head_relevance(self, input, index=None, head_mask=None):
        model = self.model
        with torch.no_grad():
            output = model(input, **_masked(head_mask))
        one_hot = _one_hot(output, index)
        with _prune_flag(model, False):
            return _head_relevance_chain([blk.attn for blk in model.blocks],
                                         lambda: model.relprop(one_hot, method=(), alpha=1))


class Baselines:

    def __init__(self, model):
        self.model = model
        self.model.eval()

    def generate_cam_attn(self, input, index=None):
        with ops.gelu_backward_plane_handoff():
            output = self.model(input, register_hook=True)
        one_hot = _one_hot(output, index)
        _attention_gradients(torch.sum(one_hot * output), [self.model.blocks[-1].attn])
        return cam_attn_tail(self.model)

    def generate_rollout(self, input, start_layer=0):
        self.model(input)
        return attn_rollout_tail(self.model, start_layer)


def _jet_bgr(mask01: np.ndarray) -> np.ndarray:
    x = np.floor(255.0 * mask01) / 255.0
    r = np.clip(1.5 - np.abs(4.0 * x - 3.0), 0.0, 1.0)
    g = np.clip(1.5 - np.abs(4.0 * x - 2.0), 0.0, 1.0)
    b = np.clip(1.5 - np.abs(4.0 * x - 1.0), 0.0, 1.0)
    return np.stack([b, g, r], axis=-1).astype(np.float32)
# ... 258 lines not shown
```

### transformer-explainability_amd/ops.py

```python
from __future__ import annotations

import contextlib
import os
from typing import Optional, Sequence, Tuple

import torch

from . import _lib
from ._lib import (TE_HEADMEAN_CLAMP, TE_HEADMEAN_ROW0, TE_IMPL_SIMPLE, TE_RATIONALE_CLAMP, TE_ROLLOUT_CLS_FIXUP,
                   TE_ROLLOUT_NORMALISE, TE_ROLLOUT_ROW0, TE_VARIANT_LRP, TE_VARIANT_OURS)
from ._lib import (TE_X6_PHASE_C, TE_X6_PHASE_SPLIT, TE_X6_PHASE_Z, TE_X6_TEST_DROP_HANDOVER,
                   TE_X6_TEST_SMALL_GRID, TE_X6_TILE_C_SHIFT, TE_X6_TILE_Z_SHIFT, TE_X6_WHOLE_TILES, TE_X6_X_PLANES_SIGNED)

Tensor = torch.Tensor
_VARIANTS = {"ours": TE_VARIANT_OURS, "lrp": TE_VARIANT_LRP}

FORCE_SIMPLE = False
KERNEL_TIMER = None
_NULL = contextlib.nullcontext()


def _timed(name: str, flops: float = 0.0, nbytes: float = 0.0):
    return _NULL if KERNEL_TIMER is None else KERNEL_TIMER(name, float(flops), float(nbytes))

# ... 395 lines not shown
                               "te_linear_x6_split_matrix_f32")
                    post_x_abs_planes(keep_abs, X, T, K, xs)
                else:
                    xs, xa = _ws(nb, Xc), _ws(nb, Xc)
                    _lib.check(lib.te_linear_x6_split_dual_f32(_ptr(Xc), T, K, _ptr(xs), _ptr(xa), nb, _stream(Xc)),
                               "te_linear_x6_split_dual_f32")
                    post_x_abs_planes(keep_abs, X, T, K, xa)
            _lib.check(lib.te_gemm_x6_f32(_ptr(Xc) if Xc is not None else None, _ptr(xs), _ptr(w_planes), _ptr(bc), _ptr(out),
                                          T, K, M, (X6_TILE | X6_FLAGS) & ~0x3c00, _ptr(x6_status(X.device)), _ptr(ws),
                                          ws.numel(), _stream(like)), "te_gemm_x6_f32")
    return out.reshape(*lead, M)


def linear_relprop(R: Tensor, X: Tensor, W: Tensor, alpha: float = 1.0, variant="ours",
                   Y: Optional[Tensor] = None, bias: Optional[Tensor] = None, cache: Optional[dict] = None) -> Tensor:
    if _any_f64(R, X, W):
        return linear_relprop_f64(R, X, W, alpha=alpha, variant=variant)
    if _is_bf16(X) or _is_bf16(W):
        return linear_relprop_bf16(R, X, W, alpha=alpha, variant=variant, cache=cache)
    out_f, in_f = W.shape
    lead = X.shape[:-1]
    R, r_scale = _split_deferred(R)
    Rc, Xc, Wc = _c(R).reshape(-1, out_f), _c(X).reshape(-1, in_f), _c(W)
    T = Xc.shape[0]
    if Rc.shape[0] != T:
        raise _lib.TeError(f"Linear.relprop: R has {Rc.shape[0]} rows, X has {T}")
    out = torch.empty((T, in_f), dtype=torch.float32, device=X.device)
    var = _variant(variant)
    fast_ok = (var == TE_VARIANT_OURS and alpha == 1 and in_f % 4 == 0 and out_f % 4 == 0 and
               all(t.data_ptr() % 16 == 0 for t in (Rc, Xc, Wc)))
    fwd = fast_ok and USE_FORWARD_OUTPUT and Y is not None
    if r_scale is not None and not fwd:
        Rc = _c(Deferred(R, r_scale).materialise()).reshape(-1, out_f)
        r_scale = None
    rs_ptr, rs_stride, rps = None, 0, 1
    if r_scale is not None:
        rs_ptr, rs_stride, rps = r_scale.data_ptr(), r_scale.stride(0), T // r_scale.shape[0]
    var_code = var & 0xff
    general = (USE_LINEAR_X6 and not (var & TE_IMPL_SIMPLE) and not (var_code == TE_VARIANT_OURS and alpha == 1)
               and all(t.data_ptr() % 16 == 0 for t in (Rc, Xc, Wc))
               and (var_code == TE_VARIANT_LRP or (USE_FORWARD_OUTPUT and Y is not None))
               and bool(_lib.load().te_linear_relprop_x6_general_supported(T, in_f, out_f, var_code)))
    if general:
        Yg = bg = None
        if var_code == TE_VARIANT_OURS:
            Yg = _c(Y.detach()).reshape(-1, out_f)
            bg = None if bias is None else _c(bias.detach())
            general = Yg.shape[0] == T and Yg.data_ptr() % 16 == 0 and (bg is None or bg.data_ptr() % 16 == 0)
    if general:
        wp = x6_weight_planes(W, cache) if var_code == TE_VARIANT_OURS else None
        wpl = x6_weight_planes_lrp(W, cache) if var_code == TE_VARIANT_LRP else None
        xa = take_x_abs_planes(cache, X, T, in_f) if cache is not None and var_code == TE_VARIANT_OURS else None
        if planes_are_signed(xa):
            xa = None
        gemm = 2.0 * T * in_f * out_f
        halves = 2 if alpha != 1 else 1
        units = (18.0 if var_code == TE_VARIANT_OURS else 24.0) * halves
        with _on_device(Xc) as lib, _timed("linear_x6_general", units * gemm,
                                           halves * (6.0 * (2 * T * in_f + 3 * in_f * out_f + 2 * T * out_f) + 16.0 * T * in_f)):
            ws = _ws(lib.te_linear_relprop_x6_general_workspace_bytes(T, in_f, out_f, var_code), Xc)
            _lib.check(lib.te_linear_relprop_x6_general_f32(_ptr(Rc), rs_ptr, rs_stride, rps, _ptr(Xc), _ptr(Wc), _ptr(wp),
                                                            _ptr(wpl), _ptr(xa), _ptr(Yg), _ptr(bg), _ptr(out), T, in_f,
                                                            out_f, float(alpha), var_code, (X6_TILE | X6_FLAGS) & ~0x3c00,
                                                            _ptr(x6_status(Xc.device)), _ptr(ws), ws.numel(), _stream(Xc)),
                       "te_linear_relprop_x6_general_f32")
            if X6_CHECK:
                x6_raise_if_failed(Xc.device)
        return out.reshape(*lead, in_f)
    if fwd:
        Yc = _c(Y.detach()).reshape(-1, out_f)
        bc = None if bias is None else _c(bias.detach())
        if Yc.shape[0] != T:
            raise _lib.TeError(f"Linear.relprop: Y has {Yc.shape[0]} rows, X has {T}")
    if (fwd and USE_LINEAR_X6 and Yc.data_ptr() % 16 == 0 and (bc is None or bc.data_ptr() % 16 == 0)
            and _lib.load().te_linear_relprop_x6_supported(T, in_f, out_f)):
        planes = x6_weight_planes(W, cache)
        xa = take_x_abs_planes(cache, X, T, in_f) if cache is not None else None
        x_signed = TE_X6_X_PLANES_SIGNED if planes_are_signed(xa) else 0
        with _on_device(Xc) as lib:
            ws = _ws(lib.te_linear_relprop_x6_workspace_bytes(T, in_f, out_f), Xc)
            status = x6_status(Xc.device)

            def call(flags):
                _lib.check(lib.te_linear_relprop_x6_f32(_ptr(Rc), rs_ptr, rs_stride, rps, _ptr(Xc), _ptr(Wc), _ptr(planes),
                                                        _ptr(xa), _ptr(Yc), _ptr(bc), _ptr(out), T, in_f, out_f,
                                                        X6_TILE | X6_FLAGS | x_signed | flags, _ptr(status), _ptr(ws), ws.numel(),
                                                        _stream(Xc)),
                           "te_linear_relprop_x6_f32")
            if KERNEL_TIMER is None:
                call(0)
            else:
                gemm = 2.0 * T * in_f * out_f
                if xa is None:
                    with _timed("linear_x6_split", 0.0, 10.0 * T * in_f):
                        call(TE_X6_PHASE_SPLIT)
                else:
                    call(TE_X6_PHASE_SPLIT)
                with _timed("linear_x6_zpass", 6.0 * gemm, 6.0 * (T * in_f + in_f * out_f + T * out_f) + 8.0 * T * out_f):
                    call(TE_X6_PHASE_Z)
                with _timed("linear_x6_cpass", 12.0 * gemm, 6.0 * (T * out_f + 2 * in_f * out_f) + 8.0 * T * in_f):
                    call(TE_X6_PHASE_C)
            if X6_CHECK:
                rc = lib.te_linear_relprop_x6_check(_ptr(ws), T, in_f, out_f, _stream(Xc))
                if rc != 0:
                    status.zero_()
                    raise _lib.TeError(f"te_linear_relprop_x6_f32({T},{in_f},{out_f}): a workgroup waited in vain for the "
                                       f"accumulators of a shared tile (status {rc}); the result is invalid")
                x6_raise_if_failed(Xc.device)
        return out.reshape(*lead, in_f)
    if KERNEL_TIMER is not None and fast_ok:
        with _on_device(Xc) as lib:
            S = torch.empty((T, out_f), dtype=torch.float32, device=X.device)
            st = _stream(Xc)
            if fwd:
                with _timed("linear_zpass_fwd", 2.0 * T * in_f * out_f, 4.0 * (T * in_f + 3 * T * out_f + in_f * out_f)):
                    _lib.check(lib.te_linear_zpass_fwd_scaled_f32(_ptr(Rc), rs_ptr, rs_stride, rps, _ptr(Xc), _ptr(Wc),
                                                                  _ptr(Yc), _ptr(bc), _ptr(S), T, in_f, out_f, st),
                               "te_linear_zpass_fwd_scaled_f32")
            else:
                with _timed("linear_zpass", 2.0 * T * (2 * in_f) * out_f, 4.0 * (T * in_f + 2 * T * out_f + in_f * out_f)):
                    _lib.check(lib.te_linear_zpass_f32(_ptr(Rc), _ptr(Xc), _ptr(Wc), _ptr(S), T, in_f, out_f, st),
                               "te_linear_zpass_f32")
            with _timed("linear_cpass", 2.0 * T * (2 * in_f) * out_f, 4.0 * (T * out_f + 2 * T * in_f + in_f * out_f)):
                _lib.check(lib.te_linear_cpass_f32(_ptr(S), _ptr(Xc), _ptr(Wc), _ptr(out), T, in_f, out_f, st),
                           "te_linear_cpass_f32")
        return out.reshape(*lead, in_f)
    with _on_device(Xc) as lib:
        ws = _ws(lib.te_linear_relprop_workspace_bytes(T, in_f, out_f, var), Xc)
        if fwd:
            _lib.check(lib.te_linear_relprop_fwd_scaled_f32(_ptr(Rc), rs_ptr, rs_stride, rps, _ptr(Xc), _ptr(Wc),
                                                            _ptr(Yc), _ptr(bc), _ptr(out), T, in_f, out_f, _ptr(ws),
                                                            ws.numel(), _stream(Xc)),
                       "te_linear_relprop_fwd_scaled_f32")
        else:
            _lib.check(lib.te_linear_relprop_f32(_ptr(Rc), _ptr(Xc), _ptr(Wc), _ptr(out), T, in_f, out_f, float(alpha),
                                                 var, _ptr(ws), ws.numel(), _stream(Xc)), "te_linear_relprop_f32")
    return out.reshape(*lead, in_f)


def _bhnd(t: Tensor) -> Tuple[Tensor, int, int, int]:
    t = _prep(t)
    if t.stride(-1) != 1 or min(t.stride()[:3]) < 0:
        t = t.contiguous()
    sb, sh, sn, _ = t.stride()
    return t, sb, sh, sn


def _cached_z(z: Optional[Tensor], shape) -> Optional[Tensor]:
    if z is None or not USE_FORWARD_PRODUCTS or tuple(z.shape) != tuple(shape):
        return None
    return _c(z.detach())


def matmul_relprop_av(R: Tensor, attn: Tensor, v: Tensor, out_scale: float = 1.0,
                      cam_v_out: Optional[Tensor] = None, variant="ours", z: Optional[Tensor] = None
                      ) -> Tuple[Tensor, Tensor]:
    if _any_f64(R, attn, v):
        return matmul_relprop_av_f64(R, attn, v, out_scale, cam_v_out, variant, z)
    if _is_bf16(attn) or _is_bf16(v):
        return matmul_relprop_av_bf16(R, attn, v, out_scale, cam_v_out, variant, z)
    B, H, N, D = v.shape
    zc = None
    z_str = (H * N * D, N * D, D)
    if z is not None and USE_FORWARD_PRODUCTS and tuple(z.shape) == (B, H, N, D):
        zd = _prep(z.detach())
        if zd.stride(-1) == 1 and min(zd.stride()[:3]) > 0:
            zc, z_str = zd, tuple(zd.stride()[:3])
        else:
            zc = zd.contiguous()
    R, r_sb, r_sh, r_sn = _bhnd(R)
    v, v_sb, v_sh, v_sn = _bhnd(v)
    attn = _c(attn)
    cam_attn = torch.empty((B, H, N, N), dtype=torch.float32, device=attn.device)
    cam_v = cam_v_out if cam_v_out is not None else torch.empty((B, H, N, D), dtype=torch.float32, device=attn.device)
    if cam_v.stride(-1) != 1:
        raise _lib.TeError("cam_v_out must have a contiguous last dim")
    cv_sb, cv_sh, cv_sn, _ = cam_v.stride()
    with _on_device(attn) as lib, _timed("attention_av_rule", 4.0 * B * H * N * N * D,
                                         4.0 * B * H * (2 * N * N + 5 * N * D)):
        ws = _ws(lib.te_matmul_relprop_av_workspace_bytes(B, H, N, D), attn)
        args = (_ptr(cam_attn), _ptr(cam_v), cv_sb, cv_sh, cv_sn, B, H, N, D, float(out_scale), _variant(variant),
                _ptr(ws), ws.numel(), _stream(attn))
        rc = lib.te_matmul_relprop_av_fwdz_f32(_ptr(R), r_sb, r_sh, r_sn, _ptr(attn), _ptr(v), v_sb, v_sh, v_sn,
                                               _ptr(zc), z_str[0], z_str[1], z_str[2], *args)
        if rc == _lib.TE_ERR_UNSUPPORTED and zc is not None and not zc.is_contiguous():
            zc = zc.contiguous()
            rc = lib.te_matmul_relprop_av_fwd_f32(_ptr(R), r_sb, r_sh, r_sn, _ptr(attn), _ptr(v), v_sb, v_sh, v_sn,
                                                  _ptr(zc), *args)
        _lib.check(rc, "te_matmul_relprop_av_fwdz_f32")
    return cam_attn, cam_v


def matmul_relprop_qk(R: Tensor, q: Tensor, k: Tensor, out_scale: float = 1.0,
                      cam_q_out: Optional[Tensor] = None, cam_k_out: Optional[Tensor] = None,
                      variant="ours", z: Optional[Tensor] = None) -> Tuple[Tensor, Tensor]:
    if _any_f64(R, q, k):
        return matmul_relprop_qk_f64(R, q, k, out_scale, cam_q_out, cam_k_out, variant, z)
    if _is_bf16(q) or _is_bf16(k):
        return matmul_relprop_qk_bf16(R, q, k, out_scale, cam_q_out, cam_k_out, variant, z)
    B, H, N, D = q.shape
    zc = _cached_z(z, (B, H, N, N))
    q, q_sb, q_sh, q_sn = _bhnd(q)
    k, k_sb, k_sh, k_sn = _bhnd(k)
    R, r_scale = _split_deferred(R)
    R = _c(R)
    dev = R.device
    cam_q = cam_q_out if cam_q_out is not None else torch.empty((B, H, N, D), dtype=torch.float32, device=dev)
    cam_k = cam_k_out if cam_k_out is not None else torch.empty((B, H, N, D), dtype=torch.float32, device=dev)
    if cam_q.stride(-1) != 1 or cam_k.stride(-1) != 1:
        raise _lib.TeError("cam_q_out / cam_k_out must have a contiguous last dim")
    cq, ck = cam_q.stride(), cam_k.stride()
    with _on_device(R) as lib, _timed("attention_qk_rule", 4.0 * B * H * N * N * D,
                                      4.0 * B * H * (2 * N * N + 4 * N * D)):
        ws = _ws(lib.te_matmul_relprop_qk_workspace_bytes(B, H, N, D), R)
        tail = (_ptr(q), q_sb, q_sh, q_sn, _ptr(k), k_sb, k_sh, k_sn, _ptr(zc), _ptr(cam_q), cq[0], cq[1], cq[2],
                _ptr(cam_k), ck[0], ck[1], ck[2], B, H, N, D, float(out_scale), _variant(variant), _ptr(ws), ws.numel(),
                _stream(R))
        rc = lib.te_matmul_relprop_qk_fwd_scaled_f32(_ptr(R), _ptr(r_scale), 0 if r_scale is None else r_scale.stride(0),
                                                     *tail)
        if rc == _lib.TE_ERR_UNSUPPORTED and r_scale is not None:
            R = _c(Deferred(R, r_scale).materialise())
            rc = lib.te_matmul_relprop_qk_fwd_scaled_f32(_ptr(R), None, 0, *tail)
        _lib.check(rc, "te_matmul_relprop_qk_fwd_scaled_f32")
    return cam_q, cam_k


USE_FUSED_PRODUCERS = False


class stock_forward:

    def __enter__(self):
        global USE_FUSED_PRODUCERS
        self.was, USE_FUSED_PRODUCERS = USE_FUSED_PRODUCERS, False

    def __exit__(self, *exc):
        global USE_FUSED_PRODUCERS
        USE_FUSED_PRODUCERS = self.was


def attention_forward_supported(N: int, D: int) -> bool:
    lib = _lib.load()
    return bool(lib.te_attention_forward_supported(int(N), int(D)) or lib.te_attention_strided_supported(int(N), int(D)))


def attention_forward_bf16_supported(N: int, D: int) -> bool:
    return bool(_lib.load().te_attention_bf16_supported(int(N), int(D)))


def _heads(t: Tensor, H: int):
    sb, sn, sc = t.stride()
    if sc != 1:
        raise _lib.TeError("attention producers need a contiguous feature dimension")
    return t, sb, 64, sn


def attention_forward_qkv(q: Tensor, k: Tensor, v: Tensor, num_heads: int, scale: float,
                          mask: Optional[Tensor] = None, want_z: bool = True, want_x: bool = False):
    if _is_bf16(q) or _is_bf16(k) or _is_bf16(v):
        return attention_forward_qkv_bf16(q, k, v, num_heads, scale, mask, want_z, want_x)
    B, N, C = q.shape
    H, D = num_heads, C // num_heads
    dev = q.device
    out = torch.empty((B, N, C), dtype=torch.float32, device=dev)
    attn = torch.empty((B, H, N, N), dtype=torch.float32, device=dev)
    zqk = torch.empty((B, H, N, N), dtype=torch.float32, device=dev) if want_z else None
    xsc = torch.empty((B, H, N, N), dtype=torch.float32, device=dev) if want_x else None
    mk = None if mask is None else _c(mask.reshape(B, N))
    (q, qb, qh, qn), (k, kb, kh, kn), (v, vb, vh, vn) = _heads(_prep(q), H), _heads(_prep(k), H), _heads(_prep(v), H)
    with _on_device(q) as lib, _timed("attention_forward", 4.0 * B * H * N * N * D,
                                      4.0 * B * ((2 + bool(want_x)) * H * N * N + 4 * N * C)):
        _lib.check(lib.te_attention_forward_strided_f32(_ptr(q), qb, qh, qn, _ptr(k), kb, kh, kn, _ptr(v), vb, vh, vn,
                                                        _ptr(mk), _ptr(zqk), _ptr(xsc), _ptr(attn), _ptr(out), N * C, 64, C,
                                                        B, H, N, D, float(scale), _stream(q)),
                   "te_attention_forward_strided_f32")
    return out, attn, zqk, xsc


def attention_forward_qkv_bf16(q: Tensor, k: Tensor, v: Tensor, num_heads: int, scale: float,
                               mask: Optional[Tensor] = None, want_z: bool = True, want_x: bool = False):
    q, k, v = _prep_bf16(q), _prep_bf16(k), _prep_bf16(v)
    B, N, C = q.shape
    H, D = num_heads, C // num_heads
    dev = q.device
    new = lambda *shape: torch.empty(shape, dtype=torch.bfloat16, device=dev)
    out, attn = new(B, N, C), new(B, H, N, N)
    zqk = new(B, H, N, N) if want_z else None
    xsc = new(B, H, N, N) if want_x else None
    mk = None if mask is None else _c16(mask.reshape(B, N))
    (q, qb, qh, qn), (k, kb, kh, kn), (v, vb, vh, vn) = _heads(q, H), _heads(k, H), _heads(v, H)
    with _on_device(q) as lib, _timed("attention_forward", 4.0 * B * H * N * N * D,
                                      2.0 * B * ((2 + bool(want_x)) * H * N * N + 4 * N * C)):
        _lib.check(lib.te_attention_forward_strided_bf16(_ptr(q), qb, qh, qn, _ptr(k), kb, kh, kn, _ptr(v), vb, vh, vn,
                                                         _ptr(mk), _ptr(zqk), _ptr(xsc), _ptr(attn), _ptr(out), N * C, 64, C,
                                                         B, H, N, D, float(scale), _stream(q)),
                   "te_attention_forward_strided_bf16")
    return out, attn, zqk, xsc


def attention_backward_qkv_bf16(d_out: Tensor, q: Optional[Tensor], k: Optional[Tensor], v: Tensor, attn: Tensor,
                                num_heads: int, scale: float, d_q: Optional[Tensor], d_k: Optional[Tensor], d_v: Tensor,
                                need_qk: bool = True) -> Tensor:
    B, N, C = d_out.shape
    H, D = num_heads, C // num_heads
    d_out, attn = _c16(d_out), _c16(attn)
    d_attn = torch.empty_like(attn)
    hd = lambda t: (None, 0, 0, 0) if t is None else _heads(_prep_bf16(t), H)
    (q, qb, qh, qn), (k, kb, kh, kn), (v, vb, vh, vn) = hd(q), hd(k), hd(v)
    (dq, dqb, dqh, dqn), (dk, dkb, dkh, dkn), (dv, dvb, dvh, dvn) = hd(d_q), hd(d_k), hd(d_v)
    with _on_device(d_out) as lib, _timed("attention_backward", (8.0 if need_qk else 4.0) * B * H * N * N * D,
                                          2.0 * B * ((5 if need_qk else 2) * H * N * N + 8 * N * C)):
        ws = _ws(lib.te_attention_backward_strided_bf16_workspace_bytes(B, H, N), d_out)
        _lib.check(lib.te_attention_backward_strided_bf16(_ptr(d_out), N * C, 64, C, _ptr(q), qb, qh, qn, _ptr(k), kb, kh, kn,
                                                          _ptr(v), vb, vh, vn, _ptr(attn), _ptr(d_attn), _ptr(dq), dqb, dqh,
                                                          dqn, _ptr(dk), dkb, dkh, dkn, _ptr(dv), dvb, dvh, dvn, B, H, N, D,
                                                          float(scale), int(bool(need_qk)), _ptr(ws), ws.numel(),
                                                          _stream(d_out)), "te_attention_backward_strided_bf16")
    return d_attn


def attention_backward_qkv(d_out: Tensor, q: Tensor, k: Tensor, v: Tensor, attn: Tensor, num_heads: int, scale: float,
                           d_q: Optional[Tensor], d_k: Optional[Tensor], d_v: Tensor, need_qk: bool = True,
                           out: Optional[Tensor] = None) -> Tensor:
    if any(_is_bf16(t) for t in (d_out, q, k, v, attn)):
        return attention_backward_qkv_bf16(d_out, q, k, v, attn, num_heads, scale, d_q, d_k, d_v, need_qk=need_qk)
    B, N, C = d_out.shape
    H, D = num_heads, C // num_heads
    d_out, attn = _c(d_out), _c(attn)
    d_attn = torch.empty_like(attn)
    hd = lambda t: (None, 0, 0, 0) if t is None else _heads(_prep(t), H)
    (q, qb, qh, qn), (k, kb, kh, kn), (v, vb, vh, vn) = hd(q), hd(k), hd(v)
    (dq, dqb, dqh, dqn), (dk, dkb, dkh, dkn), (dv, dvb, dvh, dvn) = hd(d_q), hd(d_k), hd(d_v)
    with _on_device(d_out) as lib, _timed("attention_backward", (8.0 if need_qk else 4.0) * B * H * N * N * D,
                                          4.0 * B * ((4 if need_qk else 2) * H * N * N + 8 * N * C)):
        ws = _ws(lib.te_attention_backward_strided_workspace_bytes(B, H, N), d_out)
        if out is not None and tuple(out.shape) == (B, N, C) and out.dtype == d_out.dtype and out.stride(-1) == 1:
            (o, ob, oh, on) = _heads(_prep(out), H)
            _lib.check(lib.te_attention_backward_strided_out_f32(_ptr(d_out), N * C, 64, C, _ptr(o), ob, oh, on, _ptr(q), qb, qh, qn,
                                                                 _ptr(k), kb, kh, kn, _ptr(v), vb, vh, vn, _ptr(attn), _ptr(d_attn),
                                                                 _ptr(dq), dqb, dqh, dqn, _ptr(dk), dkb, dkh, dkn, _ptr(dv), dvb, dvh,
                                                                 dvn, B, H, N, D, float(scale), int(bool(need_qk)), _ptr(ws),
                                                                 ws.numel(), _stream(d_out)), "te_attention_backward_strided_out_f32")
            return d_attn
        _lib.check(lib.te_attention_backward_strided_f32(_ptr(d_out), N * C, 64, C, _ptr(q), qb, qh, qn, _ptr(k), kb, kh, kn,
                                                         _ptr(v), vb, vh, vn, _ptr(attn), _ptr(d_attn), _ptr(dq), dqb, dqh,
                                                         dqn, _ptr(dk), dkb, dkh, dkn, _ptr(dv), dvb, dvh, dvn, B, H, N, D,
                                                         float(scale), int(bool(need_qk)), _ptr(ws), ws.numel(),
                                                         _stream(d_out)), "te_attention_backward_strided_f32")
    return d_attn


def attention_forward_planes_supported(qkv: Tensor, num_heads: int) -> bool:
    B, N, C3 = qkv.shape
    C = C3 // 3
    return (qkv.is_cuda and qkv.dtype == torch.float32 and C % num_heads == 0 and C // num_heads == 64 and N <= 224
            and bool(_lib.load().te_attention_forward_supported(N, 64)))


def attention_forward(qkv: Tensor, num_heads: int, scale: float, planes: bool = False, planes_abs: bool = True):
    if _is_bf16(qkv):
        if planes:
            raise _lib.TeError("attention_forward(planes=True): operand planes are emitted from float32 activations only")
        qkv = _c16(qkv)
        C = qkv.shape[-1] // 3
        out, attn, zqk, _ = attention_forward_qkv_bf16(qkv[..., :C], qkv[..., C:2 * C], qkv[..., 2 * C:], num_heads, scale)
        return out, attn, zqk
    qkv = _c(qkv)
    B, N, C3 = qkv.shape
    C = C3 // 3
    H, D = num_heads, C // num_heads
    if not _lib.load().te_attention_forward_supported(N, D):
        if planes:
            raise _lib.TeError("attention_forward(planes=True): shape not served by te_attention_forward_planes_f32")
        out, attn, zqk, _ = attention_forward_qkv(qkv[..., :C], qkv[..., C:2 * C], qkv[..., 2 * C:], num_heads, scale)
        return out, attn, zqk
    out = torch.empty((B, N, C), dtype=torch.float32, device=qkv.device)
    attn = torch.empty((B, H, N, N), dtype=torch.float32, device=qkv.device)
    zqk = torch.empty((B, H, N, N), dtype=torch.float32, device=qkv.device)
    extra = (12.0 if planes_abs else 6.0) * B * N * C if planes else 0.0
    with _on_device(qkv) as lib, _timed("attention_forward", 4.0 * B * H * N * N * D, 4.0 * B * (2 * H * N * N + 4 * N * C) + extra):
        if planes:
            nb = lib.te_linear_x6_planes_bytes(B * N, C)
            xs, xa = _ws(nb, qkv), _ws(nb, qkv) if planes_abs else None
            _lib.check(lib.te_attention_forward_planes_f32(_ptr(qkv), _ptr(zqk), _ptr(attn), _ptr(out), _ptr(xs), _ptr(xa), nb,
                                                           B, H, N, D, float(scale), _stream(qkv)),
                       "te_attention_forward_planes_f32")
            return out, attn, zqk, xs, xa
        _lib.check(lib.te_attention_forward_f32(_ptr(qkv), _ptr(zqk), _ptr(attn), _ptr(out), B, H, N, D, float(scale),
                                                _stream(qkv)), "te_attention_forward_f32")
    return out, attn, zqk


def attention_backward(d_out: Tensor, qkv: Tensor, attn: Tensor, num_heads: int, scale: float,
                       need_qk: bool = True, out: Optional[Tensor] = None) -> Tuple[Tensor, Optional[Tensor]]:
    if _is_bf16(d_out) or _is_bf16(qkv) or _is_bf16(attn):
        qkv = _c16(qkv)
        C = qkv.shape[-1] // 3
        d_qkv = torch.empty_like(qkv)
        th = lambda t, i: t[..., i * C:(i + 1) * C]
        d_attn = attention_backward_qkv_bf16(d_out, th(qkv, 0), th(qkv, 1), th(qkv, 2), attn, num_heads, scale,
                                             th(d_qkv, 0), th(d_qkv, 1), th(d_qkv, 2), need_qk=need_qk)
        return d_attn, d_qkv
    d_out, qkv, attn = _c(d_out), _c(qkv), _c(attn)
    B, N, C3 = qkv.shape
    C = C3 // 3
    H, D = num_heads, C // num_heads
    d_qkv = torch.empty_like(qkv)
    if not _lib.load().te_attention_forward_supported(N, D):
        th = lambda t, i: t[..., i * C:(i + 1) * C]
        d_attn = attention_backward_qkv(d_out, th(qkv, 0), th(qkv, 1), th(qkv, 2), attn, num_heads, scale,
                                        th(d_qkv, 0), th(d_qkv, 1), th(d_qkv, 2), need_qk=need_qk, out=out)
        return d_attn, d_qkv
    d_attn = torch.empty_like(attn)
    with _on_device(qkv) as lib, _timed("attention_backward", (8.0 if need_qk else 4.0) * B * H * N * N * D,
                                        4.0 * B * ((4 if need_qk else 2) * H * N * N + 8 * N * C)):
        if out is not None and need_qk and tuple(out.shape) == tuple(d_out.shape) and out.is_contiguous() and out.dtype == d_out.dtype:
            _lib.check(lib.te_attention_backward_out_f32(_ptr(d_out), _ptr(out), _ptr(qkv), _ptr(attn), _ptr(d_attn), _ptr(d_qkv),
                                                         B, H, N, D, float(scale), 1, _stream(qkv)),
                       "te_attention_backward_out_f32")
        else:
            _lib.check(lib.te_attention_backward_f32(_ptr(d_out), _ptr(qkv), _ptr(attn), _ptr(d_attn), _ptr(d_qkv), B, H, N,
                                                     D, float(scale), int(bool(need_qk)), _stream(qkv)),
                       "te_attention_backward_f32")
    return d_attn, d_qkv


def layernorm_supported(x: Tensor) -> bool:
    return (x.is_cuda and x.dtype == torch.float32 and x.dim() >= 2
            and bool(_lib.load().te_layernorm_supported(int(x.shape[-1]))))


def layernorm_forward(x: Tensor, weight: Tensor, bias: Optional[Tensor], eps: float) -> Tuple[Tensor, Tensor, Tensor]:
    x = _c(x)
    C = x.shape[-1]
    T = x.numel() // C
    y = torch.empty_like(x)
    mean = torch.empty((T,), dtype=torch.float32, device=x.device)
    rstd = torch.empty((T,), dtype=torch.float32, device=x.device)
    with _on_device(x) as lib, _timed("layernorm_forward", 0.0, 4.0 * 2 * T * C):
        _lib.check(lib.te_layernorm_forward_f32(_ptr(x), _ptr(_c(weight)), _ptr(_c(bias)) if bias is not None else None,
                                                _ptr(y), _ptr(mean), _ptr(rstd), T, C, float(eps), _stream(x)),
                   "te_layernorm_forward_f32")
    return y, mean, rstd


def layernorm_backward(dy: Tensor, x: Tensor, weight: Tensor, mean: Tensor, rstd: Tensor,
                       add: Optional[Tensor] = None) -> Tensor:
    dy, x = _c(dy), _c(x)
    C = x.shape[-1]
    T = x.numel() // C
    dx = torch.empty_like(x)
    with _on_device(x) as lib, _timed("layernorm_backward", 0.0, 4.0 * (3 + (add is not None)) * T * C):
        _lib.check(lib.te_layernorm_backward_f32(_ptr(dy), _ptr(x), _ptr(_c(weight)), _ptr(mean), _ptr(rstd),
                                                 _ptr(_c(add)) if add is not None else None, _ptr(dx), T, C, _stream(x)),
                   "te_layernorm_backward_f32")
    return dx


def gelu_forward(x: Tensor) -> Tensor:
    x = _c(x)
    y = torch.empty_like(x)
    with _on_device(x) as lib, _timed("gelu_forward", 0.0, 4.0 * 2 * x.numel()):
        _lib.check(lib.te_gelu_forward_f32(_ptr(x), _ptr(y), x.numel(), _stream(x)), "te_gelu_forward_f32")
    return y


X6_FUSE_GELU = os.environ.get("TE_X6_FUSE_GELU", "1") not in ("", "0")


_GELU_BWD_HANDOFF = 0


class gelu_backward_plane_handoff:

    def __enter__(self):
        global _GELU_BWD_HANDOFF
        _GELU_BWD_HANDOFF += 1
        return self

    def __exit__(self, *exc):
        global _GELU_BWD_HANDOFF
        _GELU_BWD_HANDOFF -= 1


def gelu_backward_handoff_active() -> bool:
    return _GELU_BWD_HANDOFF > 0


def gelu_planes_supported(x: Tensor) -> bool:
    return bool(X6_FUSE_GELU and x.dim() >= 2 and x.shape[-1] >= 16 and x.shape[-1] % 16 == 0)


def gelu_forward_planes(x: Tensor, planes_abs: bool = True):
    x = _c(x)
    K = x.shape[-1]
    T = x.numel() // K
    y = torch.empty_like(x)
    with _on_device(x) as lib, _timed("gelu_forward", 0.0, (4.0 * 2 + (12.0 if planes_abs else 6.0)) * x.numel()):
        nb = lib.te_linear_x6_planes_bytes(T, K)
        xs, xa = _ws(nb, x), _ws(nb, x) if planes_abs else None
        _lib.check(lib.te_gelu_forward_x6_planes_f32(_ptr(x), _ptr(y), T, K, _ptr(xs), _ptr(xa), nb, _stream(x)),
                   "te_gelu_forward_x6_planes_f32")
    return y, xs, xa


def gelu_backward_planes(dy: Tensor, x: Tensor) -> Tensor:
    dy, x = _c(dy), _c(x)
    K = x.shape[-1]
    T = x.numel() // K
    with _on_device(x) as lib, _timed("gelu_backward", 0.0, (4.0 * 2 + 6.0) * x.numel()):
        nb = lib.te_linear_x6_planes_bytes(T, K)
        planes = _ws(nb, x)
        _lib.check(lib.te_gelu_backward_x6_planes_f32(_ptr(dy), _ptr(x), T, K, _ptr(planes), nb, _stream(x)),
                   "te_gelu_backward_x6_planes_f32")
    return planes


def gelu_backward(dy: Tensor, x: Tensor) -> Tensor:
    dy, x = _c(dy), _c(x)
    dx = torch.empty_like(x)
    with _on_device(x) as lib, _timed("gelu_backward", 0.0, 4.0 * 3 * x.numel()):
        _lib.check(lib.te_gelu_backward_f32(_ptr(dy), _ptr(x), _ptr(dx), x.numel(), _stream(x)), "te_gelu_backward_f32")
    return dx


USE_DEFERRED_ADD = True


def _is_bcast_mask(X0: Tensor, X1: Tensor) -> bool:
    return X1.dim() == 4 and X0.dim() == 4 and X1.shape[1] == 1 and X1.shape[2] == 1 and X0.shape[1] * X0.shape[2] != 1


def add_relprop(R: Tensor, X0: Tensor, X1: Tensor, variant="ours", deferred: bool = False):
    if _any_f64(R, X0, X1):
        return add_relprop_f64(R, X0, X1, variant, deferred)
    if _is_bf16(X0) or _is_bf16(X1):
        return add_relprop_bf16(R, X0, X1, variant, deferred)
    B = X0.shape[0]
    R, X0 = _c(R), _c(X0)
    n = X0[0].numel()
    if _is_bcast_mask(X0, X1):
        H, N = X0.shape[1], X0.shape[3]
        mask = _c(X1).reshape(X1.shape[0], N)
        if mask.shape[0] == 1 and B > 1:
            mask = mask.expand(B, N).contiguous()
        out0 = torch.empty_like(X0)
        out1 = torch.empty((B, 1, 1, N), dtype=torch.float32, device=X0.device)
        if deferred and _variant(variant) == TE_VARIANT_OURS:
            fac = torch.empty((B, 2), dtype=torch.float32, device=X0.device)
            with _on_device(X0) as lib, _timed("add_bcast_mask_deferred", 0.0, 4.0 * B * (3 * H * N * N + 2 * N)):
                ws = _ws(lib.te_add_bcast_relprop_workspace_bytes(B, H, N), X0)
                _lib.check(lib.te_add_bcast_relprop_deferred_f32(_ptr(R), _ptr(X0), _ptr(mask), _ptr(out0), _ptr(out1),
                                                                 _ptr(fac), B, H, N, _ptr(ws), ws.numel(), _stream(X0)),
                           "te_add_bcast_relprop_deferred_f32")
            return Deferred(out0, fac[:, 0]), out1
        with _on_device(X0) as lib, _timed("add_bcast_mask", 0.0, 4.0 * B * (3 * H * N * N + 2 * N)):
            ws = _ws(lib.te_add_bcast_relprop_workspace_bytes(B, H, N), X0)
            _lib.check(lib.te_add_bcast_relprop_f32(_ptr(R), _ptr(X0), _ptr(mask), _ptr(out0), _ptr(out1), B, H, N,
                                                    _variant(variant), _ptr(ws), ws.numel(), _stream(X0)),
                       "te_add_bcast_relprop_f32")
        return out0, out1
    X1 = _c(X1)
    if X1.shape == X0.shape:
        x1_bs = n
    elif X1.shape[0] == 1 and X1.shape[1:] == X0.shape[1:]:
        x1_bs = 0
    else:
        raise _lib.TeError(f"Add.relprop: unsupported operand shapes {tuple(X0.shape)} + {tuple(X1.shape)}")
    out0, out1 = torch.empty_like(X0), torch.empty_like(X0)
# ... 1257 lines not shown
```

### transformer-explainability_amd/producers.py

```python
from __future__ import annotations

import torch

from . import ops


def usable(x: torch.Tensor) -> bool:
    return ops.USE_FUSED_PRODUCERS and torch.is_tensor(x) and ops.layernorm_supported(x)


def gelu_usable(x: torch.Tensor) -> bool:
    return (ops.USE_FUSED_PRODUCERS and torch.is_tensor(x) and x.is_cuda and x.dtype == torch.float32
            and x.numel() > 0 and x.numel() % 4 == 0)


def norm_usable(x: torch.Tensor, norm) -> bool:
    return (usable(x) and not norm.training and getattr(norm, "weight", None) is not None
            and tuple(norm.normalized_shape) == (x.shape[-1],))


class _LayerNorm(torch.autograd.Function):
    @staticmethod
    def forward(ctx, x, weight, bias, eps):
        y, mean, rstd = ops.layernorm_forward(x, weight, bias, eps)
        ctx.save_for_backward(x, weight, mean, rstd)
        return y

    @staticmethod
    def backward(ctx, dy):
        x, weight, mean, rstd = ctx.saved_tensors
        return ops.layernorm_backward(dy, x, weight, mean, rstd), None, None, None


class _ResidualLayerNorm(torch.autograd.Function):

    @staticmethod
    def forward(ctx, x, weight, bias, eps):
        y, mean, rstd = ops.layernorm_forward(x, weight, bias, eps)
        ctx.save_for_backward(x, weight, mean, rstd)
        return x.view_as(x), y

    @staticmethod
    def backward(ctx, d_bypass, dy):
        x, weight, mean, rstd = ctx.saved_tensors
        if dy is None:
            return d_bypass, None, None, None
        return ops.layernorm_backward(dy, x, weight, mean, rstd, add=d_bypass), None, None, None


class _Gelu(torch.autograd.Function):

    @staticmethod
    def forward(ctx, x, feeds, source):
        ctx.save_for_backward(x)
        ctx.source = source
        if feeds is not None:
            y, xs, xa = ops.gelu_forward_planes(x, not ops.X6_SIGNED_PLANES)
            ops.post_x_planes(feeds, y, xs, xa)
            return y
        return ops.gelu_forward(x)

    @staticmethod
    def backward(ctx, dy):
        (x,) = ctx.saved_tensors
        if ctx.source is not None:
            return ops.post_dy_planes(ctx.source, ops.gelu_backward_planes(dy, x), x), None, None
        return ops.gelu_backward(dy, x), None, None


class _Linear(torch.autograd.Function):

    @staticmethod
    def forward(ctx, x, weight, bias, cache, fwd_x6, bwd_x6):
        ctx.weight, ctx.cache, ctx.bwd_x6 = weight, cache, bwd_x6
        if fwd_x6:
            return ops.gemm_x6(x, ops.x6_matrix_planes(weight, False, cache), bias, weight.shape[0], "linear_forward_x6",
                               keep_abs=cache)
        return torch.nn.functional.linear(x, weight, bias)

    @staticmethod
    def backward(ctx, dy):
        w = ctx.weight
        if ctx.bwd_x6:
            dx = ops.gemm_x6(dy, ops.x6_matrix_planes(w, True, ctx.cache), None, w.shape[1], "linear_backward_x6",
                             x_planes=ops.take_dy_planes(ctx.cache, dy))
        else:
            dx = torch.matmul(dy, w)
        return dx, None, None, None, None, None


def linear_plan(x: torch.Tensor, lin):
    if not (ops.USE_FUSED_PRODUCERS and ops.X6_GEMM != "off" and torch.is_tensor(x) and x.is_cuda
            and x.dtype == torch.float32 and not lin.training and x.dim() >= 2):
        return False, False
    out_f, in_f = lin.weight.shape
    T = x.numel() // in_f
    return ops.gemm_x6_wanted(T, in_f, out_f), ops.gemm_x6_wanted(T, out_f, in_f)


def takes_producer_planes(lin, T: int, K: int) -> bool:
    out_f, in_f = lin.weight.shape
    return bool(K == in_f and ops.USE_FUSED_PRODUCERS and ops.X6_GEMM != "off" and not lin.training
                and ops.gemm_x6_wanted(T, in_f, out_f) and ops.rule_takes_abs_planes(T, in_f, out_f))


def _d(t):
    return None if t is None else t.detach()


def linear(x, lin, cache, plan):
    out = _Linear.apply(x, _d(lin.weight), _d(lin.bias), cache, plan[0], plan[1])
    if plan[1]:
        out._te_bwd_x6_cache = cache
    return out


def layer_norm(x, norm):
    return _LayerNorm.apply(x, _d(norm.weight), _d(norm.bias), norm.eps)


def residual_layer_norm(x, norm):
    return _ResidualLayerNorm.apply(x, _d(norm.weight), _d(norm.bias), norm.eps)


def gelu(x, consumer=None, consumer_cache=None):
    feeds = source = None
    if ops.gelu_planes_supported(x):
        K = x.shape[-1]
        if consumer is not None and takes_producer_planes(consumer, x.numel() // K, K):
            feeds = consumer_cache
        if ops.gelu_backward_handoff_active():
            source = getattr(x, "_te_bwd_x6_cache", None)
    if feeds is None and consumer_cache is not None:
        ops.drop_x_planes(consumer_cache)
    return _Gelu.apply(x, feeds, source)
```

### transformer-explainability_amd/vit.py

```python
from __future__ import annotations

import torch
import torch.nn as nn

from . import methods, ops, producers
from . import rules as R_ours

__all__ = ["VisionTransformer", "vit_base_patch16_224", "vit_large_patch16_224", "deit_base_patch16_224",
           "compute_rollout_attention", "make_vit_module"]


def compute_rollout_attention(all_layer_matrices, start_layer=0):
    return ops.rollout(torch.stack(list(all_layer_matrices), 0), start_layer=start_layer, normalise=False)


def tail_full(model, cam, **kwargs):
    cam, _ = model.add.relprop(cam, **kwargs)
    cam = model.patch_embed.relprop(cam[:, 1:], **kwargs)
    return cam.sum(dim=1)


def tail_rollout(model, start_layer=0):
    mats = [blk.attn.get_attn_cam().clamp(min=0).mean(dim=1) for blk in model.blocks]
    return compute_rollout_attention(mats, start_layer=start_layer)[:, 0, 1:]


def tail_attribution(model, start_layer=0, pruned=False):
    first = model.blocks[-1].attn.get_attn_cam()
    Bn, _, N, _ = first.shape
    stack = torch.empty((len(model.blocks), Bn, N, N), dtype=first.dtype, device=first.device)
    for i, blk in enumerate(model.blocks):
        if i >= start_layer or not pruned:
            ops.gradcam_headmean(blk.attn.get_attn_gradients(), blk.attn.get_attn_cam(), out=stack[i])
    return ops.rollout(stack, start_layer=start_layer, normalise=False, row0_only=True)[:, 1:]


def tail_layer(model, method, is_ablation=False):
    blk = model.blocks[-1] if method == "last_layer" else model.blocks[1]
    c = blk.attn.get_attn_cam()
    if is_ablation:
        c = blk.attn.get_attn_gradients() * c
    return c.clamp(min=0).mean(dim=1)[:, 0, 1:]


def tail_last_layer_attn(model):
    attn = model.blocks[-1].attn.get_attn()
    if ops._is_bf16(attn):
        return ops.attn_headmean(attn.detach(), clamp=True, row0=True)[:, 1:]
    return attn.clamp(min=0).mean(dim=1)[:, 0, 1:]


def relprop_tail(model, method, cam=None, is_ablation=False, start_layer=0, pruned=False, **kwargs):
    if method == "full":
        return tail_full(model, cam, **kwargs)
    if method == "rollout":
        return tail_rollout(model, start_layer)
    if method in ("transformer_attribution", "grad"):
        return tail_attribution(model, start_layer, pruned)
    if method in ("last_layer", "second_layer"):
        return tail_layer(model, method, is_ablation)
    if method == "last_layer_attn":
        return tail_last_layer_attn(model)
    return None


def _trunc_normal_(t, std=.02):
    with torch.no_grad():
        return nn.init.trunc_normal_(t, mean=0., std=std, a=-2., b=2.)


class _SplitQKV(torch.autograd.Function):

    @staticmethod
    def forward(ctx, qkv, num_heads):
        B, N, C3 = qkv.shape
        parts = qkv.view(B, N, 3, num_heads, C3 // (3 * num_heads)).permute(2, 0, 3, 1, 4)
        return parts[0].contiguous(), parts[1].contiguous(), parts[2].contiguous()

    @staticmethod
    def backward(ctx, dq, dk, dv):
        ref = next(g for g in (dq, dk, dv) if g is not None)
        B, H, N, D = ref.shape
        grad = torch.empty((B, N, 3, H, D), dtype=ref.dtype, device=ref.device)
        slots = grad.permute(2, 0, 3, 1, 4)
        for slot, g in zip(slots, (dq, dk, dv)):
            if g is None:
                slot.zero_()
            else:
                slot.copy_(g)
        return grad.view(B, N, 3 * H * D), None


def split_qkv(qkv, num_heads):
    return _SplitQKV.apply(qkv, num_heads)


class _FusedAttention(torch.autograd.Function):

    @staticmethod
    def forward(ctx, qkv, num_heads, scale, module, feeds=None):
        if feeds is not None:
            out, attn, zqk, xs, xa = ops.attention_forward(qkv, num_heads, scale, planes=True, planes_abs=not ops.X6_SIGNED_PLANES)
            ops.post_x_planes(feeds, out, xs, xa)
        else:
            out, attn, zqk = ops.attention_forward(qkv, num_heads, scale)
        ctx.save_for_backward(qkv, attn, out)
        ctx.num_heads, ctx.scale, ctx.module = num_heads, scale, module
        ctx.mark_non_differentiable(attn, zqk)
        ctx.set_materialize_grads(False)
        return out, attn, zqk

    @staticmethod
    def backward(ctx, d_out, _d_attn_unused, _d_zqk_unused):
        qkv, attn, out = ctx.saved_tensors
        if d_out is None:
            return None, None, None, None, None
        stop = bool(getattr(ctx.module, "_fused_stop_backward", False))
        d_attn, d_qkv = ops.attention_backward(d_out, qkv, attn, ctx.num_heads, ctx.scale, need_qk=not stop, out=out)
        ctx.module.save_attn_gradients(d_attn)
        return (None if stop else d_qkv), None, None, None, None


PRETRAINED_URLS = {
    "vit_base_patch16_224": "https://github.com/rwightman/pytorch-image-models/releases/download/v0.1-vitjx/"
                            "jx_vit_base_p16_224-80ecf9dd.pth",
    "vit_large_patch16_224": "https://github.com/rwightman/pytorch-image-models/releases/download/v0.1-vitjx/"
                             "jx_vit_large_p16_224-4ee7a4dc.pth",
    "deit_base_patch16_224": "https://dl.fbaipublicfiles.com/deit/deit_base_patch16_224-b5f2ef4d.pth",
}


def load_pretrained_weights(model, url, patch_size=16, key=None):
    import os
    name = os.path.basename(url)
    try:
        state = torch.hub.load_state_dict_from_url(url, map_location="cpu", progress=False)
    except Exception as exc:
        where = os.path.join(torch.hub.get_dir(), "checkpoints", name)
        raise RuntimeError(f"pretrained=True: {name} is not in the torch hub cache and could not be downloaded "
                           f"({type(exc).__name__}: {exc}); place the checkpoint at {where}") from exc
    if key is not None:
        state = state[key]
    state = dict(state)
    w = state.get("patch_embed.proj.weight")
    if w is not None and w.dim() == 2:
        state["patch_embed.proj.weight"] = w.reshape(w.shape[0], 3, patch_size, patch_size)
    strict = True
    if "head.weight" in state and state["head.weight"].shape[0] != model.head.weight.shape[0]:
        del state["head.weight"], state["head.bias"]
        strict = False
    model.load_state_dict(state, strict=strict)
    return model


def make_vit_module(L):

    class Mlp(nn.Module):
        def __init__(self, in_features, hidden_features=None, out_features=None, drop=0.):
            super().__init__()
            out_features = out_features or in_features
            hidden_features = hidden_features or in_features
            self.fc1 = L.Linear(in_features, hidden_features)
            self.act = L.GELU()
            self.fc2 = L.Linear(hidden_features, out_features)
            self.drop = L.Dropout(drop)
            if hasattr(self.act, "feeds"):
                self.act.feeds(self.fc2)

        def forward(self, x):
            return self.drop(self.fc2(self.drop(self.act(self.fc1(x)))))

        def relprop(self, cam, **kwargs):
            cam = self.fc2.relprop(cam, **kwargs)
            return self.fc1.relprop(cam, **kwargs)

    class Attention(nn.Module):
        def __init__(self, dim, num_heads=8, qkv_bias=False, attn_drop=0., proj_drop=0.):
            super().__init__()
            self.num_heads = num_heads
            self.scale = (dim // num_heads) ** -0.5
            self.matmul1 = L.einsum('bhid,bhjd->bhij')
            self.matmul2 = L.einsum('bhij,bhjd->bhid')
            self.qkv = L.Linear(dim, dim * 3, bias=qkv_bias)
            self.attn_drop = L.Dropout(attn_drop)
            self.proj = L.Linear(dim, dim)
            self.proj_drop = L.Dropout(proj_drop)
            self.softmax = L.Softmax(dim=-1)
            self.mul = L.Mul()
            self.attn_cam = self.attn = self.v = self.v_cam = self.attn_gradients = None
            self.head_mask = None
            self.save_head_relevance = False
            self.head_relevance = None

        def get_attn(self): return self.attn
        def save_attn(self, attn): self.attn = attn
        def get_attention_map(self): return self.attn
        def save_attention_map(self, attn): self.attn = attn
        def save_attn_cam(self, cam): self.attn_cam = cam
        def get_attn_cam(self): return self.attn_cam
        def get_v(self): return self.v
        def save_v(self, v): self.v = v
        def save_v_cam(self, cam): self.v_cam = cam
        def get_v_cam(self): return self.v_cam
        def save_attn_gradients(self, g): self.attn_gradients = g
        def get_attn_gradients(self): return self.attn_gradients

        def forward(self, x, head_mask=None):
            B, N, C = x.shape
            H = self.num_heads
            self._fused_anchor = None
            self.head_mask = head_mask
            if head_mask is None and ops.USE_FUSED_PRODUCERS and x.is_cuda and not self.training and (
                    (x.dtype == torch.float32 and ops.attention_forward_supported(N, C // H))
                    or (x.dtype == torch.bfloat16 and ops.attention_forward_bf16_supported(N, C // H))):
                return self._forward_fused(x)
            q, k, v = split_qkv(self.qkv(x), H)
            self.save_v(v)
            attn = self.attn_drop(self.softmax(self.matmul1([q, k]) * self.scale))
            self.save_attn(attn)
            if attn.requires_grad:
                attn.register_hook(self.save_attn_gradients)
            if head_mask is not None:
                attn = self.mul([attn, head_mask])
            out = self.matmul2([attn, v]).permute(0, 2, 1, 3).reshape(B, N, C)
            return self.proj_drop(self.proj(out))

        def _forward_fused(self, x):
            B, N, C = x.shape
            H, D = self.num_heads, C // self.num_heads
            qkv = self.qkv(x)
            feeds = None
            if (isinstance(self.proj, L.Linear) and ops.attention_forward_planes_supported(qkv, H)
                    and producers.takes_producer_planes(self.proj, B * N, C)):
                feeds = R_ours.x6_cache(self.proj)
            out, attn, zqk = _FusedAttention.apply(qkv, H, self.scale, self, feeds)
            self._fused_anchor = qkv if qkv.requires_grad else None
            q, k, v = qkv.detach().view(B, N, 3, H, D).permute(2, 0, 3, 1, 4)
            self.save_v(v)
            self.save_attn(attn)
            zav = out.detach().view(B, N, H, D).permute(0, 2, 1, 3)
            for mod, X, Y in ((self.matmul1, [q, k], zqk), (self.matmul2, [attn, v], zav)):
                mod.X, mod.Y = X, Y
                mod._y_version, mod._w_version = Y._version, (None, None)
            return self.proj_drop(self.proj(out))

        def relprop(self, cam, **kwargs):
            return self.relprop_after_proj(self.proj.relprop(cam, **kwargs), **kwargs)

        def relprop_after_proj(self, cam, **kwargs):
            B, N, C = cam.shape
            H = self.num_heads
            D = C // H
            r_heads = cam.view(B, N, H, D).permute(0, 2, 1, 3)
            if self.save_head_relevance:
                self.head_relevance = ops.head_relevance(r_heads)
            attn, v = self.matmul2.X
            q, k = self.matmul1.X
            cam_qkv = torch.empty((B, N, 3 * C), dtype=cam.dtype, device=cam.device)
            slots = cam_qkv.view(B, N, 3, H, D).permute(2, 0, 3, 1, 4)
            var = self.matmul2.variant
            cam1, cam_v = ops.matmul_relprop_av(r_heads, attn, v, out_scale=0.5, cam_v_out=slots[2], variant=var,
                                                z=R_ours._cached_y(self.matmul2))
            self.save_v_cam(cam_v)
            if self.head_mask is not None:
                cam1, _ = self.mul.relprop(cam1, **kwargs)
            self.save_attn_cam(cam1)
            if getattr(self, "_stop_after_attn_cam", False):
                raise L.StopRelprop()
            ops.matmul_relprop_qk(cam1, q, k, out_scale=0.5, cam_q_out=slots[0], cam_k_out=slots[1], variant=var,
                                  z=R_ours._cached_y(self.matmul1))
            return self.qkv.relprop(cam_qkv, **kwargs)

    class Block(nn.Module):
        def __init__(self, dim, num_heads, mlp_ratio=4., qkv_bias=False, drop=0., attn_drop=0., norm_eps=1e-6):
            super().__init__()
            self.norm1 = L.LayerNorm(dim, eps=norm_eps)
            self.attn = Attention(dim, num_heads=num_heads, qkv_bias=qkv_bias, attn_drop=attn_drop, proj_drop=drop)
            self.norm2 = L.LayerNorm(dim, eps=norm_eps)
            self.mlp = Mlp(in_features=dim, hidden_features=int(dim * mlp_ratio), drop=drop)
            self.add1 = L.Add()
            self.add2 = L.Add()
            self.clone1 = L.Clone()
            self.clone2 = L.Clone()

        def forward(self, x, head_mask=None):
            x1, n = self._clone_norm(self.clone1, self.norm1, x)
            x = self.add1([x1, self.attn(n) if head_mask is None else self.attn(n, head_mask)])
            x1, n = self._clone_norm(self.clone2, self.norm2, x)
            return self.add2([x1, self.mlp(n)])

        @staticmethod
        def _clone_norm(clone, norm, x):
            if producers.norm_usable(x, norm):
                x1, n = producers.residual_layer_norm(x, norm)
                clone.X, clone.num = x.detach(), 2
                norm.X, norm.Y = clone.X, n
                return x1, n
            x1, x2 = clone(x, 2)
            return x1, norm(x2)

        def relprop(self, cam, **kwargs):
            cam1, cam2 = self.add2.relprop(cam, deferred=True, **kwargs)
            cam2 = self.mlp.relprop(cam2, **kwargs)
            cam = self.clone2.relprop((cam1, cam2), **kwargs)
            cam1, cam2 = self.add1.relprop(cam, deferred=True, **kwargs)
            cam2 = self.attn.relprop(cam2, **kwargs)
            return self.clone1.relprop((cam1, cam2), **kwargs)

        def relprop_cls_only(self, cam_cls, **kwargs):
            alpha = kwargs.get("alpha", 1)
            var = self.add2.variant
            cls = lambda t: t[:, :1]
            dfr = ops.USE_DEFERRED_ADD
            c1, c2 = ops.add_relprop(cam_cls, cls(self.add2.X[0]), cls(self.add2.X[1]), variant=var, deferred=dfr)
            c2 = R_ours.linear_rule(self.mlp.fc2, c2, alpha, cls, var)
            c2 = R_ours.linear_rule(self.mlp.fc1, c2, alpha, cls, var)
            cam = ops.clone_relprop((c1, c2), cls(self.clone2.X))
            c1, c2 = ops.add_relprop(cam, cls(self.add1.X[0]), cls(self.add1.X[1]), variant=var, deferred=dfr)
            c2 = R_ours.linear_rule(self.attn.proj, c2, alpha, cls, var)
            if isinstance(c1, ops.Deferred):
                c1 = c1.materialise()
            B, N, C = self.clone1.X.shape
            dense = torch.zeros((2, B, N, C), dtype=c2.dtype, device=c2.device)
            dense[0, :, 0] = c1[:, 0]
            dense[1, :, 0] = c2[:, 0]
            cam2 = self.attn.relprop_after_proj(dense[1], **kwargs)
            return self.clone1.relprop((dense[0], cam2), **kwargs)

    class PatchEmbed(nn.Module):
        def __init__(self, img_size=224, patch_size=16, in_chans=3, embed_dim=768):
            super().__init__()
            img_size = (img_size, img_size) if isinstance(img_size, int) else tuple(img_size)
            patch_size = (patch_size, patch_size) if isinstance(patch_size, int) else tuple(patch_size)
            self.img_size, self.patch_size = img_size, patch_size
            self.num_patches = (img_size[1] // patch_size[1]) * (img_size[0] // patch_size[0])
            self.proj = L.Conv2d(in_chans, embed_dim, kernel_size=patch_size, stride=patch_size)

        def forward(self, x):
            B, C, Hh, Ww = x.shape
            assert Hh == self.img_size[0] and Ww == self.img_size[1], \
                f"Input image size ({Hh}*{Ww}) doesn't match model ({self.img_size[0]}*{self.img_size[1]})."
            return self.proj(x).flatten(2).transpose(1, 2)

        def relprop(self, cam, **kwargs):
            cam = cam.unflatten(1, (self.img_size[0] // self.patch_size[0], self.img_size[1] // self.patch_size[1]))
            return self.proj.relprop(cam.permute(0, 3, 1, 2), **kwargs)

    class VisionTransformer(nn.Module):
        default_method = "transformer_attribution" if L.RelProp.variant == "ours" else "grad"

        def __init__(self, img_size=224, patch_size=16, in_chans=3, num_classes=1000, embed_dim=768, depth=12,
                     num_heads=12, mlp_ratio=4., qkv_bias=False, mlp_head=False, drop_rate=0., attn_drop_rate=0.,
                     block_norm_eps=1e-6, final_norm_eps=1e-5):
            super().__init__()
            self.num_classes = num_classes
            self.num_features = self.embed_dim = embed_dim
            self.patch_embed = PatchEmbed(img_size=img_size, patch_size=patch_size, in_chans=in_chans,
                                          embed_dim=embed_dim)
            num_patches = self.patch_embed.num_patches
            self.pos_embed = nn.Parameter(torch.zeros(1, num_patches + 1, embed_dim))
            self.cls_token = nn.Parameter(torch.zeros(1, 1, embed_dim))
            self.blocks = nn.ModuleList([
                Block(dim=embed_dim, num_heads=num_heads, mlp_ratio=mlp_ratio, qkv_bias=qkv_bias, drop=drop_rate,
                      attn_drop=attn_drop_rate, norm_eps=block_norm_eps) for _ in range(depth)])
            self.norm = L.LayerNorm(embed_dim, eps=final_norm_eps)
            self.head = Mlp(embed_dim, int(embed_dim * mlp_ratio), num_classes) if mlp_head \
                else L.Linear(embed_dim, num_classes)
            _trunc_normal_(self.pos_embed, std=.02)
            _trunc_normal_(self.cls_token, std=.02)
            self.apply(self._init_weights)
            self.pool = L.IndexSelect()
            self.add = L.Add()
            self.inp_grad = None
            self.exploit_cls_sparsity = True
            self.prune_below_start_layer = False
            self.register_buffer("_cls_index", torch.zeros((), dtype=torch.long), persistent=False)

        def save_inp_grad(self, grad): self.inp_grad = grad
        def get_inp_grad(self): return self.inp_grad

        def _init_weights(self, m):
            if isinstance(m, nn.Linear):
                _trunc_normal_(m.weight, std=.02)
                if m.bias is not None:
                    nn.init.constant_(m.bias, 0)
            elif isinstance(m, nn.LayerNorm):
                nn.init.constant_(m.bias, 0)
                nn.init.constant_(m.weight, 1.0)

        @property
        def no_weight_decay(self):
            return {'pos_embed', 'cls_token'}

        def get_head_mask(self, head_mask, batch_size=None):
            return R_ours.expand_head_mask(head_mask, len(self.blocks), self.blocks[0].attn.num_heads, self.pos_embed.dtype,
                                           batch_size, self.pos_embed.device)

        def forward(self, x, register_hook=False, head_mask=None):
            B = x.shape[0]
            head_mask = self.get_head_mask(head_mask, B)
            with (ops.stock_forward() if torch.is_tensor(head_mask) else ops._NULL):
                x = self.patch_embed(x)
                x = torch.cat((self.cls_token.expand(B, -1, -1), x), dim=1)
                x = self.add([x, self.pos_embed])
                if x.requires_grad:
                    x.register_hook(self.save_inp_grad)
                for blk, hm in zip(self.blocks, head_mask):
                    x = blk(x) if hm is None else blk(x, hm)
                x = self.norm(x)
                x = self.pool(x, dim=1, indices=self._cls_index).squeeze(1)
                return self.head(x)

        def relprop(self, cam=None, method=None, is_ablation=False, start_layer=0, **kwargs):
            if method is None:
                method = self.default_method
            several = not isinstance(method, str)
            wanted = tuple(method) if several else (method,)
            if "full" in wanted and ops._is_f64(cam):
                raise ops._lib.TeError(f"{ops.DTYPES_MSG}; method='full' (the z^B patch rule) is not implemented for "
                                       "torch.float64 relevance: run it on a float32 or bfloat16 model")
            if several:
                prune = self.prune_below_start_layer and methods.prunable(wanted, methods.LRP_NEEDS)
            else:
                prune = self.prune_below_start_layer and method in methods.SINGLE_CALL_PRUNED
            try:
                with L.stop_after_attn_cam(self.blocks[start_layer].attn if prune else None):
                    cam = self.head.relprop(cam, **kwargs)
                    if self.exploit_cls_sparsity and isinstance(self.head, nn.Linear):
                        cam = ops.index_select_relprop(cam.unsqueeze(1), self.pool.X[:, :1], 0)
                        cam = self.blocks[-1].relprop_cls_only(cam, **kwargs)
                        rest = list(self.blocks)[:-1]
                    else:
                        cam = self.pool.relprop(cam.unsqueeze(1), **kwargs)
                        rest = list(self.blocks)
                    for blk in reversed(rest):
                        cam = blk.relprop(cam, **kwargs)
            except L.StopRelprop:
                cam = None

            hook = getattr(self, "_before_tail", None)
            if hook is not None:
                hook()

            maps = {m: relprop_tail(self, m, cam, is_ablation, start_layer, prune, **kwargs) for m in wanted}
            return maps if several else maps[method]

    def vit_base_patch16_224(pretrained=False, **kwargs):
        model = VisionTransformer(patch_size=16, embed_dim=768, depth=12, num_heads=12, mlp_ratio=4, qkv_bias=True,
                                  **kwargs)
        if pretrained:
            load_pretrained_weights(model, PRETRAINED_URLS["vit_base_patch16_224"], patch_size=16)
        return model

    def vit_large_patch16_224(pretrained=False, **kwargs):
        model = VisionTransformer(patch_size=16, embed_dim=1024, depth=24, num_heads=16, mlp_ratio=4, qkv_bias=True,
                                  **kwargs)
        if pretrained:
            load_pretrained_weights(model, PRETRAINED_URLS["vit_large_patch16_224"], patch_size=16)
        return model

    def deit_base_patch16_224(pretrained=False, **kwargs):
        model = VisionTransformer(patch_size=16, embed_dim=768, depth=12, num_heads=12, mlp_ratio=4, qkv_bias=True,
                                  **kwargs)
        if pretrained:
            load_pretrained_weights(model, PRETRAINED_URLS["deit_base_patch16_224"], patch_size=16, key="model")
        return model

    ns = dict(Mlp=Mlp, Attention=Attention, Block=Block, PatchEmbed=PatchEmbed, VisionTransformer=VisionTransformer,
              vit_base_patch16_224=vit_base_patch16_224, vit_large_patch16_224=vit_large_patch16_224,
              deit_base_patch16_224=deit_base_patch16_224)
    return ns


_ns = make_vit_module(R_ours)
Mlp, Attention, Block, PatchEmbed = _ns["Mlp"], _ns["Attention"], _ns["Block"], _ns["PatchEmbed"]
VisionTransformer = _ns["VisionTransformer"]
vit_base_patch16_224 = _ns["vit_base_patch16_224"]
vit_large_patch16_224 = _ns["vit_large_patch16_224"]
deit_base_patch16_224 = _ns["deit_base_patch16_224"]
```

Before: 1031.

## Propagate class-token-only gradient rows through last block backward and relprop

Adds a gate after the final norm so that the backward gradient, which is nonzero only in the class-token row, is carried as a single broadcast row through LayerNorm, GELU, Linear and attention backward. It also adds live_rows variants of the attention relprop and backward kernels, which restrict the query rows processed to the live ones. The last block's relprop passes live_rows=1. This avoids dense work on rows that are all zeros, at the cost of extra code paths, dense fallbacks, and a global registry of row tensors keyed by pointer.

```diff
diff --git a/include/te_relprop.h b/include/te_relprop.h
--- a/include/te_relprop.h
+++ b/include/te_relprop.h
@@ -101,6 +101,22 @@
                              float* cam_k, int64_t ck_sb, int64_t ck_sh, int64_t ck_sn,
                              int64_t B, int64_t H, int64_t N, int64_t D, float out_scale, int variant,
                              void* ws, size_t ws_bytes, te_stream_t stream);
+int te_matmul_relprop_av_fwdz_rows_f32(const float* R, int64_t r_sb, int64_t r_sh, int64_t r_sn,
+                                       const float* attn,
+                                       const float* v, int64_t v_sb, int64_t v_sh, int64_t v_sn,
+                                       const float* Z, int64_t z_sb, int64_t z_sh, int64_t z_sn,
+                                       float* cam_attn,
+                                       float* cam_v, int64_t cv_sb, int64_t cv_sh, int64_t cv_sn,
+                                       int64_t B, int64_t H, int64_t N, int64_t D, int64_t live_rows, float out_scale,
+                                       int variant, void* ws, size_t ws_bytes, te_stream_t stream);
+int te_matmul_relprop_qk_fwd_scaled_rows_f32(const float* R_nn, const float* r_scale, int64_t r_scale_stride,
+                                             const float* q, int64_t q_sb, int64_t q_sh, int64_t q_sn,
+                                             const float* k, int64_t k_sb, int64_t k_sh, int64_t k_sn,
+                                             const float* Z,
+                                             float* cam_q, int64_t cq_sb, int64_t cq_sh, int64_t cq_sn,
+                                             float* cam_k, int64_t ck_sb, int64_t ck_sh, int64_t ck_sn,
+                                             int64_t B, int64_t H, int64_t N, int64_t D, int64_t live_rows, float out_scale,
+                                             int variant, void* ws, size_t ws_bytes, te_stream_t stream);
 
 size_t te_add_relprop_workspace_bytes(int64_t B, int64_t n);
 int te_add_relprop_f32(const float* R, const float* X0, const float* X1, float* out0, float* out1,
@@ -205,6 +221,9 @@
 int te_attention_backward_out_f32(const float* d_out, const float* out, const float* qkv, const float* attn, float* d_attn,
                                   float* d_qkv, int64_t B, int64_t H, int64_t N, int64_t D, float scale, int need_qk,
                                   te_stream_t stream);
+int te_attention_backward_out_rows_f32(const float* d_out, const float* out, const float* qkv, const float* attn, float* d_attn,
+                                       float* d_qkv, int64_t B, int64_t H, int64_t N, int64_t D, int64_t live_rows, float scale,
+                                       int need_qk, te_stream_t stream);
 
 int te_attention_strided_supported(int64_t N, int64_t D);
 size_t te_attention_backward_strided_workspace_bytes(int64_t B, int64_t H, int64_t N);
diff --git a/transformer-explainability_amd/csrc/te_attn.hip b/transformer-explainability_amd/csrc/te_attn.hip
--- a/transformer-explainability_amd/csrc/te_attn.hip
+++ b/transformer-explainability_amd/csrc/te_attn.hip
@@ -128,13 +128,16 @@
                                        cam_v, cv_sb, cv_sh, cv_sn, B, H, N, D, out_scale, variant, ws, ws_bytes, stream_);
 }
 
-extern "C" int te_matmul_relprop_av_fwdz_f32(const float* R, int64_t r_sb, int64_t r_sh, int64_t r_sn,
-                                             const float* attn, const float* v, int64_t v_sb, int64_t v_sh,
-                                             int64_t v_sn, const float* Z, int64_t z_sb, int64_t z_sh, int64_t z_sn,
-                                             float* cam_attn, float* cam_v, int64_t cv_sb, int64_t cv_sh,
-                                             int64_t cv_sn, int64_t B, int64_t H, int64_t N, int64_t D,
-                                             float out_scale, int variant, void* ws, size_t ws_bytes,
-                                             te_stream_t stream_) {
+static int rows_check(int64_t B, int64_t H, int64_t N, int64_t D, int64_t live_rows, int variant) {
+  if (B <= 0 || H <= 0 || N <= 0 || D <= 0 || live_rows < 1 || live_rows > N) return TE_ERR_INVALID_ARG;
+  if ((variant & TE_IMPL_SIMPLE) || !te_attn_rc::supported(B, H, N, D) || !te_attn_kb::supported(B, H, N, D)) return TE_ERR_UNSUPPORTED;
+  return TE_OK;
+}
+
+static int av_rule(const float* R, int64_t r_sb, int64_t r_sh, int64_t r_sn, const float* attn, const float* v, int64_t v_sb,
+                   int64_t v_sh, int64_t v_sn, const float* Z, int64_t z_sb, int64_t z_sh, int64_t z_sn, float* cam_attn, float* cam_v,
+                   int64_t cv_sb, int64_t cv_sh, int64_t cv_sn, int64_t B, int64_t H, int64_t N, int64_t D, int64_t live_rows,
+                   float out_scale, int variant, void* ws, size_t ws_bytes, te_stream_t stream_) {
   if (!R || !attn || !v || !cam_attn || !cam_v || B <= 0 || H <= 0 || N <= 0 || D <= 0)
     return TE_ERR_INVALID_ARG;
   const Strided rs{r_sb, r_sh, r_sn}, vs{v_sb, v_sh, v_sn}, cs{cv_sb, cv_sh, cv_sn}, contig{H * N * D, N * D, D};
@@ -163,8 +166,32 @@
     Z = Zws;
   }
   if (te_attn_kb::supported(B, H, N, D))
-    return finish(te_attn_kb::av_launch(TE_ATTN_RULE, R, rs, attn, v, vs, Z, zs, cam_attn, cam_v, cs, B, H, N, out_scale, stream));
+    return finish(te_attn_kb::av_launch(TE_ATTN_RULE, R, rs, attn, v, vs, Z, zs, cam_attn, cam_v, cs, B, H, N, out_scale, stream, live_rows));
   return finish(te_attn_mfma::av_launch(R, rs, attn, v, vs, Z, zs, cam_attn, cam_v, cs, B, H, N, out_scale, S, stream));
+}
+
+extern "C" int te_matmul_relprop_av_fwdz_f32(const float* R, int64_t r_sb, int64_t r_sh, int64_t r_sn,
+                                             const float* attn, const float* v, int64_t v_sb, int64_t v_sh,
+                                             int64_t v_sn, const float* Z, int64_t z_sb, int64_t z_sh, int64_t z_sn,
+                                             float* cam_attn, float* cam_v, int64_t cv_sb, int64_t cv_sh,
+                                             int64_t cv_sn, int64_t B, int64_t H, int64_t N, int64_t D,
+                                             float out_scale, int variant, void* ws, size_t ws_bytes,
+                                             te_stream_t stream_) {
+  return av_rule(R, r_sb, r_sh, r_sn, attn, v, v_sb, v_sh, v_sn, Z, z_sb, z_sh, z_sn, cam_attn, cam_v, cv_sb, cv_sh, cv_sn, B, H, N, D,
+                 N, out_scale, variant, ws, ws_bytes, stream_);
+}
+
+extern "C" int te_matmul_relprop_av_fwdz_rows_f32(const float* R, int64_t r_sb, int64_t r_sh, int64_t r_sn,
+                                                  const float* attn, const float* v, int64_t v_sb, int64_t v_sh,
+                                                  int64_t v_sn, const float* Z, int64_t z_sb, int64_t z_sh, int64_t z_sn,
+                                                  float* cam_attn, float* cam_v, int64_t cv_sb, int64_t cv_sh,
+                                                  int64_t cv_sn, int64_t B, int64_t H, int64_t N, int64_t D,
+                                                  int64_t live_rows, float out_scale, int variant, void* ws,
+                                                  size_t ws_bytes, te_stream_t stream_) {
+  const int rc = rows_check(B, H, N, D, live_rows, variant);
+  if (rc != TE_OK) return rc;
+  return av_rule(R, r_sb, r_sh, r_sn, attn, v, v_sb, v_sh, v_sn, Z, z_sb, z_sh, z_sn, cam_attn, cam_v, cv_sb, cv_sh, cv_sn, B, H, N, D,
+                 live_rows, out_scale, variant, ws, ws_bytes, stream_);
 }
 
 extern "C" size_t te_matmul_relprop_qk_workspace_bytes(int64_t B, int64_t H, int64_t N, int64_t D) {
@@ -195,14 +222,11 @@
                                              ws_bytes, stream_);
 }
 
-extern "C" int te_matmul_relprop_qk_fwd_scaled_f32(const float* R_nn, const float* r_scale, int64_t r_scale_stride,
-                                                   const float* q, int64_t q_sb, int64_t q_sh, int64_t q_sn,
-                                                   const float* k, int64_t k_sb, int64_t k_sh, int64_t k_sn,
-                                                   const float* Z, float* cam_q, int64_t cq_sb, int64_t cq_sh,
-                                                   int64_t cq_sn, float* cam_k, int64_t ck_sb, int64_t ck_sh,
-                                                   int64_t ck_sn, int64_t B, int64_t H, int64_t N, int64_t D,
-                                                   float out_scale, int variant, void* ws, size_t ws_bytes,
-                                                   te_stream_t stream_) {
+static int qk_rule(const float* R_nn, const float* r_scale, int64_t r_scale_stride, const float* q, int64_t q_sb, int64_t q_sh,
+                   int64_t q_sn, const float* k, int64_t k_sb, int64_t k_sh, int64_t k_sn, const float* Z, float* cam_q, int64_t cq_sb,
+                   int64_t cq_sh, int64_t cq_sn, float* cam_k, int64_t ck_sb, int64_t ck_sh, int64_t ck_sn, int64_t B, int64_t H,
+                   int64_t N, int64_t D, int64_t live_rows, float out_scale, int variant, void* ws, size_t ws_bytes,
+                   te_stream_t stream_) {
   if (!R_nn || !q || !k || !cam_q || !cam_k || B <= 0 || H <= 0 || N <= 0 || D <= 0) return TE_ERR_INVALID_ARG;
   const Strided qs{q_sb, q_sh, q_sn}, ks{k_sb, k_sh, k_sn}, cqs{cq_sb, cq_sh, cq_sn}, cks{ck_sb, ck_sh, ck_sn};
   if (!view_ok(qs) || !view_ok(ks) || !view_ok(cqs) || !view_ok(cks)) return TE_ERR_INVALID_ARG;
@@ -231,12 +255,38 @@
   if (te_attn_rules::supported(B, H, N, D) && q_sn > 65536) return TE_ERR_UNSUPPORTED;
   if (te_attn_rc::supported(B, H, N, D))
     return finish(te_attn_rc::qk_launch(TE_ATTN_RULE, R_nn, q, qs, k, ks, Z, cam_q, cqs, cam_k, cks, B, H, N, out_scale, r_scale, r_scale_stride,
-                                        stream));
+                                        stream, nullptr, nullptr, Strided(), live_rows));
   if (te_attn_rules::supported(B, H, N, D))
     return finish(te_attn_rules::qk_launch(TE_ATTN_RULE, R_nn, q, qs, k, ks, Z, cam_q, cqs, cam_k, cks, B, H, N, out_scale, S, r_scale,
                                            r_scale_stride, stream));
   if (r_scale) return TE_ERR_UNSUPPORTED;
   return finish(te_attn_mfma::qk_launch(R_nn, q, qs, k, ks, Z, cam_q, cqs, cam_k, cks, B, H, N, out_scale, S, stream));
+}
+
+extern "C" int te_matmul_relprop_qk_fwd_scaled_f32(const float* R_nn, const float* r_scale, int64_t r_scale_stride,
+                                                   const float* q, int64_t q_sb, int64_t q_sh, int64_t q_sn,
+                                                   const float* k, int64_t k_sb, int64_t k_sh, int64_t k_sn,
+                                                   const float* Z, float* cam_q, int64_t cq_sb, int64_t cq_sh,
+                                                   int64_t cq_sn, float* cam_k, int64_t ck_sb, int64_t ck_sh,
+                                                   int64_t ck_sn, int64_t B, int64_t H, int64_t N, int64_t D,
+                                                   float out_scale, int variant, void* ws, size_t ws_bytes,
+                                                   te_stream_t stream_) {
+  return qk_rule(R_nn, r_scale, r_scale_stride, q, q_sb, q_sh, q_sn, k, k_sb, k_sh, k_sn, Z, cam_q, cq_sb, cq_sh, cq_sn, cam_k, ck_sb,
+                 ck_sh, ck_sn, B, H, N, D, N, out_scale, variant, ws, ws_bytes, stream_);
+}
+
+extern "C" int te_matmul_relprop_qk_fwd_scaled_rows_f32(const float* R_nn, const float* r_scale, int64_t r_scale_stride,
+                                                        const float* q, int64_t q_sb, int64_t q_sh, int64_t q_sn,
+                                                        const float* k, int64_t k_sb, int64_t k_sh, int64_t k_sn,
+                                                        const float* Z, float* cam_q, int64_t cq_sb, int64_t cq_sh,
+                                                        int64_t cq_sn, float* cam_k, int64_t ck_sb, int64_t ck_sh,
+                                                        int64_t ck_sn, int64_t B, int64_t H, int64_t N, int64_t D,
+                                                        int64_t live_rows, float out_scale, int variant, void* ws,
+                                                        size_t ws_bytes, te_stream_t stream_) {
+  const int rc = rows_check(B, H, N, D, live_rows, variant);
+  if (rc != TE_OK) return rc;
+  return qk_rule(R_nn, r_scale, r_scale_stride, q, q_sb, q_sh, q_sn, k, k_sb, k_sh, k_sn, Z, cam_q, cq_sb, cq_sh, cq_sn, cam_k, ck_sb,
+                 ck_sh, ck_sn, B, H, N, D, live_rows, out_scale, variant, ws, ws_bytes, stream_);
 }
 
 extern "C" int te_attention_forward_supported(int64_t N, int64_t D) { return te_attn_fwd6::supported(1, 1, N, D) ? 1 : 0; }
@@ -260,8 +310,10 @@
 }
 
 static int attention_backward(const float* d_out, const float* out, const float* qkv, const float* attn, float* d_attn, float* d_qkv,
-                              int64_t B, int64_t H, int64_t N, int64_t D, float scale, int need_qk, te_stream_t stream_) {
+                              int64_t B, int64_t H, int64_t N, int64_t D, float scale, int need_qk, int64_t live_rows,
+                              te_stream_t stream_) {
   if (!d_out || !qkv || !attn || !d_attn || !d_qkv || B <= 0 || H <= 0 || N <= 0) return TE_ERR_INVALID_ARG;
+  if (live_rows < 1 || live_rows > N) return TE_ERR_INVALID_ARG;
   if (!te_attn_fwd6::supported(B, H, N, D)) return TE_ERR_UNSUPPORTED;
   hipStream_t stream = (hipStream_t)stream_;
   const int64_t C = H * 64;
@@ -269,11 +321,12 @@
   const Strided fused{N * 3 * C, 64, 3 * C};
   const float *q = qkv, *k = qkv + C, *v = qkv + 2 * C;
   float *d_q = d_qkv, *d_k = d_qkv + C, *d_v = d_qkv + 2 * C;
-  const int rc = te_attn_kb::av_launch(TE_ATTN_BWD, d_out, heads, attn, v, fused, nullptr, Strided(), d_attn, d_v, fused, B, H, N, 1.0f, stream);
+  const int rc = te_attn_kb::av_launch(TE_ATTN_BWD, d_out, heads, attn, v, fused, nullptr, Strided(), d_attn, d_v, fused, B, H, N, 1.0f, stream,
+                                       live_rows);
   if (rc != TE_OK || !need_qk) return finish(rc);
   if ((N <= 160 || out) && te_attn_rc::supported(B, H, N, D))
     return finish(te_attn_rc::qk_launch(TE_ATTN_BWD, d_attn, q, fused, k, fused, attn, d_q, fused, d_k, fused, B, H, N, scale, nullptr, 0, stream,
-                                        out ? d_out : nullptr, out, heads));
+                                        out ? d_out : nullptr, out, heads, live_rows));
   return finish(te_attn_rules::qk_launch(TE_ATTN_BWD, d_attn, q, fused, k, fused, attn, d_q, fused, d_k, fused, B, H, N, scale, nullptr, nullptr, 0,
                                          stream));
 }
@@ -281,14 +334,23 @@
 extern "C" int te_attention_backward_f32(const float* d_out, const float* qkv, const float* attn, float* d_attn,
                                          float* d_qkv, int64_t B, int64_t H, int64_t N, int64_t D, float scale,
                                          int need_qk, te_stream_t stream_) {
-  return attention_backward(d_out, nullptr, qkv, attn, d_attn, d_qkv, B, H, N, D, scale, need_qk, stream_);
+  return attention_backward(d_out, nullptr, qkv, attn, d_attn, d_qkv, B, H, N, D, scale, need_qk, N, stream_);
 }
 
 extern "C" int te_attention_backward_out_f32(const float* d_out, const float* out, const float* qkv, const float* attn,
                                              float* d_attn, float* d_qkv, int64_t B, int64_t H, int64_t N, int64_t D,
                                              float scale, int need_qk, te_stream_t stream_) {
   if (!out) return TE_ERR_INVALID_ARG;
-  return attention_backward(d_out, out, qkv, attn, d_attn, d_qkv, B, H, N, D, scale, need_qk, stream_);
+  return attention_backward(d_out, out, qkv, attn, d_attn, d_qkv, B, H, N, D, scale, need_qk, N, stream_);
+}
+
+extern "C" int te_attention_backward_out_rows_f32(const float* d_out, const float* out, const float* qkv, const float* attn,
+                                                  float* d_attn, float* d_qkv, int64_t B, int64_t H, int64_t N, int64_t D,
+                                                  int64_t live_rows, float scale, int need_qk, te_stream_t stream_) {
+  if (!out) return TE_ERR_INVALID_ARG;
+  const int rc = rows_check(B, H, N, D, live_rows, 0);
+  if (rc != TE_OK) return rc;
+  return attention_backward(d_out, out, qkv, attn, d_attn, d_qkv, B, H, N, D, scale, need_qk, live_rows, stream_);
 }
 
 extern "C" int te_attention_strided_supported(int64_t N, int64_t D) { return te_attn_long::supported(1, 1, N, D) ? 1 : 0; }
diff --git a/transformer-explainability_amd/csrc/te_attn_kb.hip b/transformer-explainability_amd/csrc/te_attn_kb.hip
--- a/transformer-explainability_amd/csrc/te_attn_kb.hip
+++ b/transformer-explainability_amd/csrc/te_attn_kb.hip
@@ -27,7 +27,7 @@
 __global__ __launch_bounds__(kT) void av6_kb_kernel(
     const float* __restrict__ R, Strided rs, const float* __restrict__ Z, Strided zs, const float* __restrict__ attn,
     const float* __restrict__ v, Strided vs, float* __restrict__ cam_attn, float* __restrict__ cam_v, Strided cs, int H,
-    int N, int BH, int KBG, float scale) {
+    int N, int BH, int KBG, float scale, int ntiles) {
   __shared__ __attribute__((aligned(16))) unsigned char Sb[3][kSBuf];
   __shared__ __attribute__((aligned(16))) float Xw[kWaves][TI * XLD];
   __shared__ unsigned arrived;
@@ -39,7 +39,6 @@
   const int nkb = (N + 31) >> 5, kb = g * KBG + wave;
   const bool has_blk = wave < KBG && kb < nkb;
   const int j = kb * 32 + lr;
-  const int ntiles = (N + TI - 1) / TI;
   const int srow = threadIdx.x >> 4, sc = threadIdx.x & 15;
   const int spos = (srow & 0x13) | ((srow & 4) << 1) | ((srow & 8) >> 1);
 
@@ -247,6 +246,18 @@
   }
 }
 
+__global__ __launch_bounds__(256) void zero_rows_kernel(float* __restrict__ a, int64_t per, int64_t first, int64_t cnt) {
+  float* const p = a + (int64_t)blockIdx.x * per + first;
+  const int64_t t = (int64_t)blockIdx.y * 256 + threadIdx.x, nt = (int64_t)gridDim.y * 256;
+  const int64_t mis = (int64_t)((4u - (unsigned)((reinterpret_cast<uintptr_t>(p) >> 2) & 3u)) & 3u);
+  const int64_t head = mis < cnt ? mis : cnt;
+  const int64_t n4 = (cnt - head) >> 2, tail0 = head + 4 * n4;
+  if (t < head) p[t] = 0.0f;
+  f32x4* const p4 = reinterpret_cast<f32x4*>(p + head);
+  for (int64_t i = t; i < n4; i += nt) p4[i] = f32x4{0.0f, 0.0f, 0.0f, 0.0f};
+  if (t < cnt - tail0) p[tail0 + t] = 0.0f;
+}
+
 inline void groups_for(int64_t N, int& ng, int& kbg) {
   const int nkb = (int)((N + 31) / 32);
   ng = (nkb + kWaves - 1) / kWaves;
@@ -262,18 +273,28 @@
 }
 
 int av_launch(int mode, const float* R, Strided rs, const float* attn, const float* v, Strided vs, const float* Z, Strided zs,
-              float* cam_attn, float* cam_v, Strided cs, int64_t B, int64_t H, int64_t N, float scale, hipStream_t stream) {
+              float* cam_attn, float* cam_v, Strided cs, int64_t B, int64_t H, int64_t N, float scale, hipStream_t stream,
+              int64_t live_rows) {
+  if (live_rows < 1 || live_rows > N) return TE_ERR_INVALID_ARG;
   int ng, kbg;
   groups_for(N, ng, kbg);
   const int BH = (int)(B * H);
   auto stride_ok = [](int64_t sn) { return sn >= 64 && sn <= 65536; };
   if (!stride_ok(rs.sn) || !stride_ok(vs.sn) || !stride_ok(cs.sn) || (mode == 0 && !stride_ok(zs.sn))) return TE_ERR_UNSUPPORTED;
   const dim3 grid((unsigned)(BH * ng)), blk(kT);
+  const int ntiles = (int)((live_rows + TI - 1) / TI);
+  const int64_t done = (int64_t)ntiles * TI;
+  if (done < N) {
+    const int64_t cnt = (N - done) * N, per_chunk = cnt / 4096;
+    const unsigned chunks = (unsigned)(per_chunk < 1 ? 1 : per_chunk > 64 ? 64 : per_chunk);
+    zero_rows_kernel<<<dim3((unsigned)BH, chunks), dim3(256), 0, stream>>>(cam_attn, N * N, done * N, cnt);
+  }
   if (mode == 0)
-    av6_kb_kernel<RULE><<<grid, blk, 0, stream>>>(R, rs, Z, zs, attn, v, vs, cam_attn, cam_v, cs, (int)H, (int)N, BH, kbg, scale);
+    av6_kb_kernel<RULE><<<grid, blk, 0, stream>>>(R, rs, Z, zs, attn, v, vs, cam_attn, cam_v, cs, (int)H, (int)N, BH, kbg, scale,
+                                                  ntiles);
   else
     av6_kb_kernel<BWD><<<grid, blk, 0, stream>>>(R, rs, nullptr, Strided{0, 0, 0}, attn, v, vs, cam_attn, cam_v, cs, (int)H,
-                                                 (int)N, BH, kbg, 1.0f);
+                                                 (int)N, BH, kbg, 1.0f, ntiles);
   return TE_OK;
 }
 
diff --git a/transformer-explainability_amd/csrc/te_attn_rc.hip b/transformer-explainability_amd/csrc/te_attn_rc.hip
--- a/transformer-explainability_amd/csrc/te_attn_rc.hip
+++ b/transformer-explainability_amd/csrc/te_attn_rc.hip
@@ -335,9 +335,11 @@
                                                    Strided ks, float* __restrict__ cam_q, Strided cqs,
                                                    float* __restrict__ cam_k, Strided cks, int H, int N, float scale,
                                                    const float* __restrict__ r_scale, int64_t r_scale_stride, int both,
-                                                   const float* __restrict__ dO, const float* __restrict__ O, Strided os) {
+                                                   const float* __restrict__ dO, const float* __restrict__ O, Strided os,
+                                                   int live) {
   extern __shared__ __attribute__((aligned(16))) unsigned char smem[];
   const int NS = (N + 15) >> 4, NB = (N + 31) >> 5;
+  const int LNS = (live + 15) >> 4, LNB = (live + 31) >> 5;
   const size_t plane = (size_t)NS * 2 * kFrag;
   unsigned char* const Pk = smem;
   unsigned char* const Pq = both ? smem + 3 * plane : smem;
@@ -362,7 +364,7 @@
       for (int r0 = 0; r0 < 32 * NB; r0 += kT / 4) {
         const int i = r0 + (threadIdx.x >> 2), c = threadIdx.x & 3;
         float part = 0.0f;
-        if (i < N) {
+        if (i < live) {
           const float* a = dO_bh + (int64_t)i * os.sn + 16 * c;
           const float* o = O_bh + (int64_t)i * os.sn + 16 * c;
           f32x4 av[4], ov[4];
@@ -377,7 +379,7 @@
         part = part + __shfl_xor(part, 2, 64);
         if (c == 0 && i < 32 * NB) rdv[i] = part;
       }
-    } else if (owner) {
+    } else if (wave < LNB) {
       row_dots(rdv, r_rs, z_rs, N, NB, wave);
     }
   }
@@ -389,7 +391,7 @@
     for (int mb = 0; mb < 2; ++mb)
 #pragma unroll
       for (int e = 0; e < 16; ++e) acc[mb][e] = 0.0f;
-    phase_rows<MODE>(acc, Pk, plane, r_rs, z_rs, N, NB, wave, f, has_f, scale, rdv);
+    if (wave < LNB) phase_rows<MODE>(acc, Pk, plane, r_rs, z_rs, N, NB, wave, f, has_f, scale, rdv);
     const int i = wave * 32 + n;
     if (i < N) {
       const float* qrow = q_bh + (int64_t)i * qs.sn + 4 * hh;
@@ -427,7 +429,7 @@
     for (int mb = 0; mb < 2; ++mb)
 #pragma unroll
       for (int e = 0; e < 16; ++e) acc[mb][e] = 0.0f;
-    phase<MODE, COLS>(acc, Pq, plane, r_rs, z_rs, N, NS, wave, f, has_f, scale, rd_own, rdv);
+    phase<MODE, COLS>(acc, Pq, plane, r_rs, z_rs, N, LNS, wave, f, has_f, scale, rd_own, rdv);
     const int j = wave * 32 + n;
     if (j < N) {
       const float* krow = k_bh + (int64_t)j * ks.sn + 4 * hh;
@@ -469,20 +471,22 @@
 
 int qk_launch(int mode, const float* Rnn, const float* q, Strided qs, const float* k, Strided ks, const float* Z, float* cam_q,
               Strided cqs, float* cam_k, Strided cks, int64_t B, int64_t H, int64_t N, float scale, const float* r_scale,
-              int64_t r_scale_stride, hipStream_t stream, const float* d_out, const float* out, Strided os) {
+              int64_t r_scale_stride, hipStream_t stream, const float* d_out, const float* out, Strided os, int64_t live_rows) {
   if (!supported(B, H, N, 64)) return TE_ERR_UNSUPPORTED;
+  if (live_rows < 0 || live_rows > N) return TE_ERR_INVALID_ARG;
+  const int live = (int)(live_rows ? live_rows : N);
   const int both = lds_bytes(N, true) <= kLdsMax ? 1 : 0;
   const size_t lds = lds_bytes(N, both != 0);
   const dim3 grid((unsigned)(B * H));
   if (mode == RULE) {
     (void)hipFuncSetAttribute(reinterpret_cast<const void*>(qk_rc_kernel<RULE>), hipFuncAttributeMaxDynamicSharedMemorySize, (int)kLdsMax);
     qk_rc_kernel<RULE><<<grid, dim3(kT), lds, stream>>>(Rnn, Z, q, qs, k, ks, cam_q, cqs, cam_k, cks, (int)H, (int)N, scale, r_scale,
-                                                       r_scale_stride, both, nullptr, nullptr, Strided{0, 0, 0});
+                                                       r_scale_stride, both, nullptr, nullptr, Strided{0, 0, 0}, live);
   } else {
     (void)hipFuncSetAttribute(reinterpret_cast<const void*>(qk_rc_kernel<BWD>), hipFuncAttributeMaxDynamicSharedMemorySize, (int)kLdsMax);
     const bool from_out = d_out != nullptr && out != nullptr;
     qk_rc_kernel<BWD><<<grid, dim3(kT), lds, stream>>>(Rnn, Z, q, qs, k, ks, cam_q, cqs, cam_k, cks, (int)H, (int)N, scale, nullptr, 0,
-                                                      both, from_out ? d_out : nullptr, from_out ? out : nullptr, os);
+                                                      both, from_out ? d_out : nullptr, from_out ? out : nullptr, os, live);
   }
   return TE_OK;
 }
diff --git a/transformer-explainability_amd/csrc/te_internal.h b/transformer-explainability_amd/csrc/te_internal.h
--- a/transformer-explainability_amd/csrc/te_internal.h
+++ b/transformer-explainability_amd/csrc/te_internal.h
@@ -28,14 +28,16 @@
 namespace te_attn_kb {
 bool supported(int64_t B, int64_t H, int64_t N, int64_t D);
 int av_launch(int mode, const float* R, Strided rs, const float* attn, const float* v, Strided vs, const float* Z, Strided zs,
-              float* cam_attn, float* cam_v, Strided cs, int64_t B, int64_t H, int64_t N, float scale, hipStream_t stream);
+              float* cam_attn, float* cam_v, Strided cs, int64_t B, int64_t H, int64_t N, float scale, hipStream_t stream,
+              int64_t live_rows);
 }
 
 namespace te_attn_rc {
 bool supported(int64_t B, int64_t H, int64_t N, int64_t D);
 int qk_launch(int mode, const float* Rnn, const float* q, Strided qs, const float* k, Strided ks, const float* Z, float* cam_q,
               Strided cqs, float* cam_k, Strided cks, int64_t B, int64_t H, int64_t N, float scale, const float* r_scale,
-              int64_t r_scale_stride, hipStream_t stream, const float* d_out = nullptr, const float* out = nullptr, Strided os = Strided());
+              int64_t r_scale_stride, hipStream_t stream, const float* d_out = nullptr, const float* out = nullptr, Strided os = Strided(),
+              int64_t live_rows = 0);
 }
 
 namespace te_attn_fwd6 {
diff --git a/transformer-explainability_amd/generators.py b/transformer-explainability_amd/generators.py
--- a/transformer-explainability_amd/generators.py
+++ b/transformer-explainability_amd/generators.py
@@ -7,7 +7,7 @@
 import torch
 
 from . import methods as M
-from . import ops
+from . import ops, producers
 from .rules import StopRelprop, stop_after_attn_cam
 from .vit import relprop_tail
 
@@ -37,15 +37,27 @@
     return torch.stack([a.mean(dim=1) for a in attns], 0)
 
 
-def _attention_gradients(loss, attn_modules, retain_graph=False):
+def _class_row_attention(model):
+    if not getattr(model, "exploit_cls_sparsity", False) or not hasattr(model, "_cls_index"):
+        return None
+    blocks = getattr(model, "blocks", None)
+    return blocks[-1].attn if blocks else None
+
+
+def _attention_gradients(loss, attn_modules, retain_graph=False, class_row=None):
     anchors = [getattr(m, "_fused_anchor", None) for m in attn_modules]
     if anchors and all(a is not None for a in anchors):
         lowest = attn_modules[0]
         lowest._fused_stop_backward = True
+        if class_row is not None and any(m is class_row for m in attn_modules):
+            class_row._fused_live_rows = 1
         try:
-            torch.autograd.grad(loss, [anchors[0]], retain_graph=retain_graph, allow_unused=True)
+            with (producers.class_row_backward() if class_row is not None else ops._NULL):
+                torch.autograd.grad(loss, [anchors[0]], retain_graph=retain_graph, allow_unused=True)
         finally:
             lowest._fused_stop_backward = False
+            if class_row is not None:
+                class_row._fused_live_rows = None
         return
     if any(a is not None for a in anchors):
         raise ops._lib.TeError("attention gradients: some of the listed blocks ran on the producer kernels and some on "
@@ -217,7 +229,7 @@
     def _gradients_and_chain(self, loss, attn_modules, chain, tail_owner=None, retain_graph=False):
         if chain is None or not (self.overlap_backward and loss.is_cuda):
             if attn_modules:
-                _attention_gradients(loss, attn_modules, retain_graph)
+                _attention_gradients(loss, attn_modules, retain_graph, _class_row_attention(self.model))
             return None if chain is None else chain()
         dev = loss.device
         main = torch.cuda.current_stream(dev)
@@ -226,7 +238,7 @@
         side = self._relprop_stream
         side.wait_stream(main)
         if attn_modules:
-            _attention_gradients(loss, attn_modules, retain_graph)
+            _attention_gradients(loss, attn_modules, retain_graph, _class_row_attention(self.model))
         if tail_owner is not None:
             grads_ready = main.record_event()
             tail_owner._before_tail = lambda: torch.cuda.current_stream(dev).wait_event(grads_ready)
diff --git a/transformer-explainability_amd/ops.py b/transformer-explainability_amd/ops.py
--- a/transformer-explainability_amd/ops.py
+++ b/transformer-explainability_amd/ops.py
@@ -571,6 +571,23 @@
     return _c(z.detach())
 
 
+_LIVE_QUERY_ROWS: Optional[int] = None
+
+
+class live_query_rows:
+
+    def __init__(self, n: Optional[int]):
+        self.n = n
+
+    def __enter__(self):
+        global _LIVE_QUERY_ROWS
+        self.was, _LIVE_QUERY_ROWS = _LIVE_QUERY_ROWS, self.n
+
+    def __exit__(self, *exc):
+        global _LIVE_QUERY_ROWS
+        _LIVE_QUERY_ROWS = self.was
+
+
 def matmul_relprop_av(R: Tensor, attn: Tensor, v: Tensor, out_scale: float = 1.0,
                       cam_v_out: Optional[Tensor] = None, variant="ours", z: Optional[Tensor] = None
                       ) -> Tuple[Tensor, Tensor]:
@@ -600,8 +617,15 @@
         ws = _ws(lib.te_matmul_relprop_av_workspace_bytes(B, H, N, D), attn)
         args = (_ptr(cam_attn), _ptr(cam_v), cv_sb, cv_sh, cv_sn, B, H, N, D, float(out_scale), _variant(variant),
                 _ptr(ws), ws.numel(), _stream(attn))
-        rc = lib.te_matmul_relprop_av_fwdz_f32(_ptr(R), r_sb, r_sh, r_sn, _ptr(attn), _ptr(v), v_sb, v_sh, v_sn,
-                                               _ptr(zc), z_str[0], z_str[1], z_str[2], *args)
+        rc = _lib.TE_ERR_UNSUPPORTED
+        live_rows = _LIVE_QUERY_ROWS
+        if live_rows is not None and 1 <= live_rows < N and not FORCE_SIMPLE:
+            rc = lib.te_matmul_relprop_av_fwdz_rows_f32(_ptr(R), r_sb, r_sh, r_sn, _ptr(attn), _ptr(v), v_sb, v_sh, v_sn,
+                                                        _ptr(zc), z_str[0], z_str[1], z_str[2], *args[:9], int(live_rows),
+                                                        *args[9:])
+        if rc == _lib.TE_ERR_UNSUPPORTED:
+            rc = lib.te_matmul_relprop_av_fwdz_f32(_ptr(R), r_sb, r_sh, r_sn, _ptr(attn), _ptr(v), v_sb, v_sh, v_sn,
+                                                   _ptr(zc), z_str[0], z_str[1], z_str[2], *args)
         if rc == _lib.TE_ERR_UNSUPPORTED and zc is not None and not zc.is_contiguous():
             zc = zc.contiguous()
             rc = lib.te_matmul_relprop_av_fwd_f32(_ptr(R), r_sb, r_sh, r_sn, _ptr(attn), _ptr(v), v_sb, v_sh, v_sn,
@@ -635,8 +659,14 @@
         tail = (_ptr(q), q_sb, q_sh, q_sn, _ptr(k), k_sb, k_sh, k_sn, _ptr(zc), _ptr(cam_q), cq[0], cq[1], cq[2],
                 _ptr(cam_k), ck[0], ck[1], ck[2], B, H, N, D, float(out_scale), _variant(variant), _ptr(ws), ws.numel(),
                 _stream(R))
-        rc = lib.te_matmul_relprop_qk_fwd_scaled_f32(_ptr(R), _ptr(r_scale), 0 if r_scale is None else r_scale.stride(0),
-                                                     *tail)
+        rc = _lib.TE_ERR_UNSUPPORTED
+        live_rows = _LIVE_QUERY_ROWS
+        if live_rows is not None and 1 <= live_rows < N and not FORCE_SIMPLE:
+            rc = lib.te_matmul_relprop_qk_fwd_scaled_rows_f32(_ptr(R), _ptr(r_scale), 0 if r_scale is None else r_scale.stride(0),
+                                                              *tail[:21], int(live_rows), *tail[21:])
+        if rc == _lib.TE_ERR_UNSUPPORTED:
+            rc = lib.te_matmul_relprop_qk_fwd_scaled_f32(_ptr(R), _ptr(r_scale), 0 if r_scale is None else r_scale.stride(0),
+                                                         *tail)
         if rc == _lib.TE_ERR_UNSUPPORTED and r_scale is not None:
             R = _c(Deferred(R, r_scale).materialise())
             rc = lib.te_matmul_relprop_qk_fwd_scaled_f32(_ptr(R), None, 0, *tail)
@@ -811,7 +841,8 @@
 
 
 def attention_backward(d_out: Tensor, qkv: Tensor, attn: Tensor, num_heads: int, scale: float,
-                       need_qk: bool = True, out: Optional[Tensor] = None) -> Tuple[Tensor, Optional[Tensor]]:
+                       need_qk: bool = True, out: Optional[Tensor] = None, live_rows: Optional[int] = None
+                       ) -> Tuple[Tensor, Optional[Tensor]]:
     if _is_bf16(d_out) or _is_bf16(qkv) or _is_bf16(attn):
         qkv = _c16(qkv)
         C = qkv.shape[-1] // 3
@@ -833,7 +864,14 @@
     d_attn = torch.empty_like(attn)
     with _on_device(qkv) as lib, _timed("attention_backward", (8.0 if need_qk else 4.0) * B * H * N * N * D,
                                         4.0 * B * ((4 if need_qk else 2) * H * N * N + 8 * N * C)):
-        if out is not None and need_qk and tuple(out.shape) == tuple(d_out.shape) and out.is_contiguous() and out.dtype == d_out.dtype:
+        with_out = out is not None and tuple(out.shape) == tuple(d_out.shape) and out.is_contiguous() and out.dtype == d_out.dtype
+        rc = _lib.TE_ERR_UNSUPPORTED
+        if with_out and live_rows is not None and 1 <= live_rows < N:
+            rc = lib.te_attention_backward_out_rows_f32(_ptr(d_out), _ptr(out), _ptr(qkv), _ptr(attn), _ptr(d_attn), _ptr(d_qkv),
+                                                        B, H, N, D, int(live_rows), float(scale), int(bool(need_qk)), _stream(qkv))
+        if rc != _lib.TE_ERR_UNSUPPORTED:
+            _lib.check(rc, "te_attention_backward_out_rows_f32")
+        elif with_out and need_qk:
             _lib.check(lib.te_attention_backward_out_f32(_ptr(d_out), _ptr(out), _ptr(qkv), _ptr(attn), _ptr(d_attn), _ptr(d_qkv),
                                                          B, H, N, D, float(scale), 1, _stream(qkv)),
                        "te_attention_backward_out_f32")
diff --git a/transformer-explainability_amd/producers.py b/transformer-explainability_amd/producers.py
--- a/transformer-explainability_amd/producers.py
+++ b/transformer-explainability_amd/producers.py
@@ -17,6 +17,65 @@
 def norm_usable(x: torch.Tensor, norm) -> bool:
     return (usable(x) and not norm.training and getattr(norm, "weight", None) is not None
             and tuple(norm.normalized_shape) == (x.shape[-1],))
+
+
+_ROWS = None
+
+
+class class_row_backward:
+
+    def __enter__(self):
+        global _ROWS
+        self.was, _ROWS = _ROWS, {}
+
+    def __exit__(self, *exc):
+        global _ROWS
+        _ROWS = self.was
+
+
+def _as_rows(row, like_shape):
+    row = row.contiguous()
+    _ROWS[row.data_ptr()] = row
+    return row.expand(like_shape)
+
+
+def row_of(dy):
+    if (_ROWS is None or dy is None or dy.dim() != 3 or dy.shape[1] < 2 or dy.stride(1) != 0 or dy.stride(2) != 1
+            or dy.data_ptr() not in _ROWS):
+        return None
+    return dy[:, :1]
+
+
+def dense_of(dy):
+    row = row_of(dy)
+    if row is None:
+        return dy
+    out = torch.zeros(dy.shape, dtype=dy.dtype, device=dy.device)
+    out[:, 0] = row[:, 0]
+    return out
+
+
+class _ClassRowGate(torch.autograd.Function):
+
+    @staticmethod
+    def forward(ctx, x):
+        return x.view_as(x)
+
+    @staticmethod
+    def backward(ctx, dy):
+        if _ROWS is None or dy.dim() != 3 or dy.shape[1] < 2:
+            return dy
+        return _as_rows(dy[:, :1], dy.shape)
+
+
+def class_row_gate(x):
+    return _ClassRowGate.apply(x)
+
+
+def _ln_rows(row, x, weight, mean, rstd, add=None):
+    B, N = x.shape[0], x.shape[1]
+    return ops.layernorm_backward(row, x[:, :1], weight, mean.view(B, N)[:, :1].contiguous(), rstd.view(B, N)[:, :1].contiguous(),
+                                  add=add)
 
 
 class _LayerNorm(torch.autograd.Function):
@@ -29,7 +88,10 @@
     @staticmethod
     def backward(ctx, dy):
         x, weight, mean, rstd = ctx.saved_tensors
-        return ops.layernorm_backward(dy, x, weight, mean, rstd), None, None, None
+        row = row_of(dy)
+        if row is not None and x.dim() == 3:
+            return _as_rows(_ln_rows(row, x, weight, mean, rstd), x.shape), None, None, None
+        return ops.layernorm_backward(dense_of(dy), x, weight, mean, rstd), None, None, None
 
 
 class _ResidualLayerNorm(torch.autograd.Function):
@@ -44,8 +106,11 @@
     def backward(ctx, d_bypass, dy):
         x, weight, mean, rstd = ctx.saved_tensors
         if dy is None:
-            return d_bypass, None, None, None
-        return ops.layernorm_backward(dy, x, weight, mean, rstd, add=d_bypass), None, None, None
+            return dense_of(d_bypass), None, None, None
+        row, row_bypass = row_of(dy), row_of(d_bypass)
+        if row is not None and row_bypass is not None and x.dim() == 3:
+            return _as_rows(_ln_rows(row, x, weight, mean, rstd, add=row_bypass), x.shape), None, None, None
+        return ops.layernorm_backward(dense_of(dy), x, weight, mean, rstd, add=dense_of(d_bypass)), None, None, None
 
 
 class _Gelu(torch.autograd.Function):
@@ -63,6 +128,9 @@
     @staticmethod
     def backward(ctx, dy):
         (x,) = ctx.saved_tensors
+        row = row_of(dy)
+        if row is not None:
+            return _as_rows(ops.gelu_backward(row, x[:, :1]), x.shape), None, None
         if ctx.source is not None:
             return ops.post_dy_planes(ctx.source, ops.gelu_backward_planes(dy, x), x), None, None
         return ops.gelu_backward(dy, x), None, None
@@ -81,6 +149,12 @@
     @staticmethod
     def backward(ctx, dy):
         w = ctx.weight
+        row = row_of(dy)
+        if row is not None:
+            if ctx.bwd_x6 and ops.gemm_x6_supported(row.shape[0], w.shape[0], w.shape[1]):
+                dx = ops.gemm_x6(row, ops.x6_matrix_planes(w, True, ctx.cache), None, w.shape[1], "linear_backward_x6")
+                return _as_rows(dx, dy.shape[:-1] + (w.shape[1],)), None, None, None, None, None
+            dy = dense_of(dy)
         if ctx.bwd_x6:
             dx = ops.gemm_x6(dy, ops.x6_matrix_planes(w, True, ctx.cache), None, w.shape[1], "linear_backward_x6",
                              x_planes=ops.take_dy_planes(ctx.cache, dy))
diff --git a/transformer-explainability_amd/vit.py b/transformer-explainability_amd/vit.py
--- a/transformer-explainability_amd/vit.py
+++ b/transformer-explainability_amd/vit.py
@@ -116,7 +116,11 @@
         if d_out is None:
             return None, None, None, None, None
         stop = bool(getattr(ctx.module, "_fused_stop_backward", False))
-        d_attn, d_qkv = ops.attention_backward(d_out, qkv, attn, ctx.num_heads, ctx.scale, need_qk=not stop, out=out)
+        live = getattr(ctx.module, "_fused_live_rows", None)
+        if producers.row_of(d_out) is not None:
+            d_out, live = producers.dense_of(d_out), 1
+        d_attn, d_qkv = ops.attention_backward(d_out, qkv, attn, ctx.num_heads, ctx.scale, need_qk=not stop, out=out,
+                                               live_rows=live)
         ctx.module.save_attn_gradients(d_attn)
         return (None if stop else d_qkv), None, None, None, None
 
@@ -247,7 +251,9 @@
         def relprop(self, cam, **kwargs):
             return self.relprop_after_proj(self.proj.relprop(cam, **kwargs), **kwargs)
 
-        def relprop_after_proj(self, cam, **kwargs):
+        def relprop_after_proj(self, cam, live_rows=None, **kwargs):
+            if self.head_mask is not None:
+                live_rows = None
             B, N, C = cam.shape
             H = self.num_heads
             D = C // H
@@ -259,16 +265,18 @@
             cam_qkv = torch.empty((B, N, 3 * C), dtype=cam.dtype, device=cam.device)
             slots = cam_qkv.view(B, N, 3, H, D).permute(2, 0, 3, 1, 4)
             var = self.matmul2.variant
-            cam1, cam_v = ops.matmul_relprop_av(r_heads, attn, v, out_scale=0.5, cam_v_out=slots[2], variant=var,
-                                                z=R_ours._cached_y(self.matmul2))
+            with ops.live_query_rows(live_rows):
+                cam1, cam_v = ops.matmul_relprop_av(r_heads, attn, v, out_scale=0.5, cam_v_out=slots[2], variant=var,
+                                                    z=R_ours._cached_y(self.matmul2))
             self.save_v_cam(cam_v)
             if self.head_mask is not None:
                 cam1, _ = self.mul.relprop(cam1, **kwargs)
             self.save_attn_cam(cam1)
             if getattr(self, "_stop_after_attn_cam", False):
                 raise L.StopRelprop()
-            ops.matmul_relprop_qk(cam1, q, k, out_scale=0.5, cam_q_out=slots[0], cam_k_out=slots[1], variant=var,
-                                  z=R_ours._cached_y(self.matmul1))
+            with ops.live_query_rows(live_rows):
+                ops.matmul_relprop_qk(cam1, q, k, out_scale=0.5, cam_q_out=slots[0], cam_k_out=slots[1], variant=var,
+                                      z=R_ours._cached_y(self.matmul1))
             return self.qkv.relprop(cam_qkv, **kwargs)
 
     class Block(nn.Module):
@@ -324,7 +332,7 @@
             dense = torch.zeros((2, B, N, C), dtype=c2.dtype, device=c2.device)
             dense[0, :, 0] = c1[:, 0]
             dense[1, :, 0] = c2[:, 0]
-            cam2 = self.attn.relprop_after_proj(dense[1], **kwargs)
+            cam2 = self.attn.relprop_after_proj(dense[1], live_rows=1, **kwargs)
             return self.clone1.relprop((dense[0], cam2), **kwargs)
 
     class PatchEmbed(nn.Module):
@@ -408,8 +416,30 @@
                 for blk, hm in zip(self.blocks, head_mask):
                     x = blk(x) if hm is None else blk(x, hm)
                 x = self.norm(x)
+                if self._class_row_tail(x):
+                    x = producers.class_row_gate(x)
                 x = self.pool(x, dim=1, indices=self._cls_index).squeeze(1)
                 return self.head(x)
+
+        def _class_row_tail(self, x):
+            if not (self.exploit_cls_sparsity and ops.USE_FUSED_PRODUCERS and not self.training and x.dim() == 3
+                    and x.shape[1] > 1 and x.is_cuda and x.dtype == torch.float32 and x.requires_grad and len(self.blocks)):
+                return False
+            blk = self.blocks[-1]
+            T = x.shape[0] * x.shape[1]
+
+            def on_producers(lin):
+                if not isinstance(lin, R_ours.Linear) or ops.X6_GEMM == "off":
+                    return False
+                out_f, in_f = lin.weight.shape
+                return ops.gemm_x6_wanted(T, in_f, out_f) or ops.gemm_x6_wanted(T, out_f, in_f)
+            act = blk.mlp.act
+            return bool(getattr(blk.attn, "_fused_anchor", None) is not None and blk.attn.head_mask is None
+                        and isinstance(self.norm, R_ours.LayerNorm)
+                        and all(producers.norm_usable(x, n) for n in (self.norm, blk.norm1, blk.norm2))
+                        and all(on_producers(lin) for lin in (blk.attn.proj, blk.mlp.fc1, blk.mlp.fc2))
+                        and isinstance(act, R_ours.GELU) and getattr(act, "approximate", "none") == "none"
+                        and (T * blk.mlp.fc1.weight.shape[0]) % 4 == 0)
 
         def relprop(self, cam=None, method=None, is_ablation=False, start_layer=0, **kwargs):
             if method is None:
```

After: 1042 (median of 6 runs). About the same (+1.0%).
